# linchaobao/EPPM

Hardware: AMD Instinct MI355X
Metric: Mflow-vectors/sec (higher is better)
Workload: dtype f32; 1 GPU; single 1024x436 Sintel-shape synthetic pair per step, full 3-level pyramid, patch_r=9, default defs.h parameters; 1 rank(s), independent pairs; inputs: RGBA planes resident in HBM before the timed region; outputs: interleaved float2 flow left in HBM (the PCIe-inclusive window of the reference API -- host RGB in, host u/v out -- is `host_boundary`, with --full); inputs=device-resident RGBA, outputs=device-resident float2 flow, pairs_in_flight_per_gpu=24, pairs_per_launch=8, contexts_in_flight=3, width=1024, height=436

## Files before the change

### eppm_amd/_lib.py

```python
import ctypes as C
import os

from .build import lib_path


class EppmError(RuntimeError):
    pass


class CParams(C.Structure):
    _fields_ = [("patch_r", C.c_int), ("num_iter", C.c_int), ("search_range", C.c_int), ("num_guess", C.c_int),
                ("seg_len", C.c_int), ("wmf_iters", C.c_int), ("seed", C.c_ulonglong), ("propagation", C.c_int),
                ("levels", C.c_int)]


class CTrackParams(C.Structure):
    _fields_ = [("spacing", C.c_int), ("min_eig", C.c_int64), ("fb_alpha", C.c_float), ("fb_beta", C.c_float), ("mb_alpha", C.c_float),
                ("mb_beta", C.c_float), ("capacity", C.c_int)]


class CTFilterParams(C.Structure):
    _fields_ = [("thresh", C.c_float), ("n_max", C.c_int)]


class CStabParams(C.Structure):
    _fields_ = [("tau", C.c_float), ("iters", C.c_int), ("smooth", C.c_float)]


class CGMotionModel(C.Structure):
    _fields_ = [("p", C.c_double * 6), ("n_valid", C.c_int64), ("n_inliers", C.c_int64), ("valid", C.c_int), ("passes", C.c_int)]

    def as_dict(self):
        import numpy as np
        return dict(p=np.array(self.p[:], np.float64), n_valid=int(self.n_valid), n_inliers=int(self.n_inliers), valid=int(self.valid),
                    passes=int(self.passes))


class CCutParams(C.Structure):
    _fields_ = [("lost_permille", C.c_int), ("residual_max", C.c_float)]


class CCutStats(C.Structure):
    _fields_ = [("n", C.c_int64), ("c1", C.c_int64 * 4), ("c2", C.c_int64 * 4), ("n_tracked", C.c_int64), ("sad", C.c_int64), ("cut", C.c_int32),
                ("stepped", C.c_int32)]

    def as_dict(self):
        return dict(n=int(self.n), c1=[int(x) for x in self.c1], c2=[int(x) for x in self.c2], n_tracked=int(self.n_tracked), sad=int(self.sad),
                    cut=int(self.cut), stepped=int(self.stepped))


class CTrackCounts(C.Structure):
    _fields_ = [("live", C.c_int), ("ended", C.c_int), ("seeded", C.c_int), ("dropped", C.c_int), ("frame", C.c_int), ("next_id", C.c_int)]

    def as_dict(self):
        return {k: int(getattr(self, k)) for k, _ in self._fields_}


_lib = None

SYMBOLS = [
    "eppm_default_params", "eppm_create", "eppm_create_batch", "eppm_batch_size", "eppm_batch_set_images", "eppm_batch_set_images_device",
    "eppm_batch_compute", "eppm_batch_compute_device", "eppm_batch_compute_end", "eppm_batch_get_plane", "eppm_destroy", "eppm_set_stream", "eppm_set_images", "eppm_set_images_device",
    "eppm_compute", "eppm_compute_begin", "eppm_compute_end", "eppm_compute_device", "eppm_synchronize", "eppm_num_levels", "eppm_level_dims", "eppm_get_plane",
    "eppm_stage_times", "eppm_clear_stage_times", "eppm_enable_stage_timing", "eppm_last_error", "eppm_version",
    "eppm_device_count", "eppm_set_device", "eppm_malloc_device", "eppm_malloc_pitched", "eppm_free_device",
    "eppm_memcpy_h2d", "eppm_memcpy_d2h", "eppm_memcpy2d_h2d", "eppm_memcpy2d_d2h", "eppm_memset_device",
    "eppm_device_synchronize", "eppm_device_mem_info", "eppm_device_pci_bus_id", "eppm_bind_thread_to_device", "eppm_release_cached_memory", "eppm_set_launcher_stream", "eppm_set_launcher_params", "eppm_launcher_status",
    "baoCudaPatchMatchMultiscalePrepare", "baoCudaCensusTransform", "baoCudaPatchMatch", "baoCudaLeftRightCheck",
    "baoCudaOutlierRemoval", "baoCudaWeightedMedianFilter", "baoCudaFillHole", "baoCudaNNF2Flow", "baoCudaBLF_C2F",
    "baoCudaBLFCostFilterRefine", "baoCudaFlowSmoothing", "eppm_flow_to_color", "eppm_compute_color",
    "eppm_pm_rng_create", "eppm_pm_rng_reset", "eppm_pm_rng_destroy", "eppm_pm_rng_block_states", "eppm_pm_gen_rand_field",
    "eppm_pm_cost_field", "eppm_pm_seg_propagate", "eppm_pm_jump_propagate", "eppm_pm_parallel_propagate", "eppm_pm_random_search", "eppm_gauss_filter_rgba", "eppm_resize_rgba",
    "eppm_resize_flow",
    "eppm_host_register", "eppm_host_unregister", "eppm_host_is_registered", "eppm_host_alloc", "eppm_host_free",
    "eppm_compute_begin_into", "eppm_batch_compute_begin_into",
    "eppm_load_ppm", "eppm_ppm_size", "eppm_save_flo", "eppm_load_flo", "eppm_flo_size", "eppm_flow_error",
    "eppm_flow_error_border", "eppm_flow_error_percentage", "eppm_flow_cutoff", "eppm_flow_to_color_host",
    "eppm_compute_bidirectional", "eppm_compute_bidirectional_device", "eppm_batch_compute_bidirectional", "eppm_set_occlusion_params",
    "eppm_fb_occlusion", "eppm_fb_occlusion_host",
    "eppm_interpolate", "eppm_interpolate_device", "eppm_batch_interpolate", "eppm_interpolate_frames", "eppm_interpolate_host",
    "eppm_track_default_params", "eppm_track_capacity", "eppm_tracker_create", "eppm_tracker_destroy", "eppm_track_step",
    "eppm_track_step_frames", "eppm_tracker_get", "eppm_tracker_get_ended", "eppm_tracker_set", "eppm_track_step_host", "eppm_track_seeds_host",
    "eppm_push_image", "eppm_push_image_device", "eppm_set_temporal", "eppm_temporal_reset", "eppm_temporal_valid", "eppm_temporal_prior_host",
    "eppm_temporal_prior",
    "eppm_batch_set_temporal", "eppm_batch_push_images", "eppm_batch_push_images_device", "eppm_batch_temporal_valid", "eppm_batch_temporal_reset",
    "eppm_temporal_prior_batch",
    "eppm_set_stop_level", "eppm_stop_level", "eppm_flow_upsample",
    "eppm_tfilter_default_params", "eppm_tfilter_create", "eppm_tfilter_create_size", "eppm_tfilter_destroy", "eppm_tfilter_reset", "eppm_tfilter_step",
    "eppm_tfilter_step_frames", "eppm_tfilter_get", "eppm_tfilter_get_device", "eppm_tfilter_get_state", "eppm_tfilter_set_state",
    "eppm_tfilter_seed_host", "eppm_tfilter_step_host",
    "eppm_stab_default_params", "eppm_stab_create", "eppm_stab_create_size", "eppm_stab_destroy", "eppm_stab_reset", "eppm_stab_step",
    "eppm_stab_step_frames", "eppm_stab_get", "eppm_stab_get_device", "eppm_stab_get_mask", "eppm_stab_get_model", "eppm_stab_get_path",
    "eppm_stab_set_path", "eppm_gmotion_fit_host", "eppm_stab_update_host", "eppm_stab_warp_host",
    "eppm_cutdet_default_params", "eppm_cutdet_create", "eppm_cutdet_create_size", "eppm_cutdet_destroy", "eppm_cutdet_step",
    "eppm_cutdet_step_frames", "eppm_cutdet_get", "eppm_cutdet_cuts", "eppm_cutdet_host",
]


TEST_SYMBOLS = ["eppm_test_set_option", "eppm_test_c2f_refine_batch", "eppm_probe_c2f_window", "eppm_probe_dispatch", "eppm_probe_fast_exp", "eppm_probe_div_const", "eppm_probe_delta_table",
                "eppm_probe_unpack_texel", "eppm_probe_pm_parity", "eppm_probe_ctx_rng_states"]

_variant = None


def select_library(variant):
    global _variant
    if _lib is not None and variant != _variant:
        raise EppmError("select_library: a library is loaded already")
    _variant = variant


def lib():
    global _lib
    if _lib is None:
        path = lib_path(_variant)
        if not os.path.exists(path):
            raise EppmError(f"{path} is missing: run eppm_amd.build() (hipcc --offload-arch=gfx950); there is no CPU fallback")
        L = C.CDLL(path)
        L.eppm_last_error.restype = C.c_char_p
        L.eppm_version.restype = C.c_char_p
        _lib = L
    return _lib


def check(status, what=""):
    if status != 0:
        raise EppmError(f"{what}: status {status}: {lib().eppm_last_error().decode()}")


def check_launcher(what=""):
    check(lib().eppm_launcher_status(), what)


def probe_dispatch(stage, *args, nout=1):
    a = (C.c_int * len(args))(*[int(v) for v in args])
    out = (C.c_int * nout)()
    check(lib().eppm_probe_dispatch(stage.encode(), a, len(args), out, nout), f"eppm_probe_dispatch {stage}")
    return tuple(out)
```

### eppm_amd/csrc/api_internal.h

```cpp
#pragma once

#include <ctype.h>
#include <math.h>
#include <sched.h>
#include <stdarg.h>
#include <stdio.h>
#include <stdlib.h>
#include <string.h>

#include <atomic>
#include <chrono>
#include <condition_variable>
#include <map>
#include <mutex>
#include <string>
#include <tuple>
#include <vector>

#include "eppm_internal.h"
#include "host_registry.h"

#define EPPM_HIDDEN __attribute__((visibility("hidden")))

EPPM_HIDDEN int set_err(int code, const char* fmt, ...) __attribute__((format(printf, 2, 3)));
#define HIPCHK(expr)                                                                                         \
    do {                                                                                                     \
        hipError_t e_ = (expr);                                                                              \
        if (e_ != hipSuccess) {                                                                              \
            (void)hipGetLastError();                                                                         \
            return set_err(EPPM_ERR_HIP, "%s failed: %s (%s:%d)", #expr, hipGetErrorString(e_), __FILE__, __LINE__); \
        }                                                                                                    \
    } while (0)
#define CHK(expr)                     \
    do {                              \
        int r_ = (expr);              \
        if (r_ != EPPM_OK) return r_; \
    } while (0)

EPPM_HIDDEN int check_params(const eppm_params& p);
EPPM_HIDDEN void host_pm_lut(int R, std::vector<float>& v);
EPPM_HIDDEN void host_wmf_lut(std::vector<float>& v);
EPPM_HIDDEN void host_blf_lut(std::vector<float>& v);
EPPM_HIDDEN int pyr_init_dim(int* arrH, int* arrW, int h, int w, int maxDepth, double ratio);
EPPM_HIDDEN int upload_lut(float** dst, const std::vector<float>& v);
struct DeltaIndex { int32_t t1[256]; std::vector<float> dval; };
EPPM_HIDDEN const DeltaIndex& delta_index();
EPPM_HIDDEN int upload_lut_delta(float** dst, const std::vector<float>& head, int which);
EPPM_HIDDEN int upload_pm_lut(float** dst, int R);
EPPM_HIDDEN int upload_wmf_lut(float** dst);
EPPM_HIDDEN int upload_blf_lut(float** dst);

#ifdef EPPM_TEST_HOOKS
EPPM_HIDDEN extern std::atomic<int> g_opt_rand_table;
EPPM_HIDDEN extern std::atomic<int> g_opt_sweep_spec;
EPPM_HIDDEN extern std::atomic<int> g_opt_no_split;
EPPM_HIDDEN extern std::atomic<int> g_opt_force_split;
static inline int opt_rand_table() { return g_opt_rand_table.load(); }
static inline int opt_sweep_spec() { return g_opt_sweep_spec.load(); }
static inline int opt_no_split() { return g_opt_no_split.load(); }
static inline int opt_force_split() { return g_opt_force_split.load(); }
#else
static constexpr int opt_rand_table() { return 1; }
static constexpr int opt_sweep_spec() { return -1; }
static constexpr int opt_no_split() { return 0; }
static constexpr int opt_force_split() { return 0; }
#endif


namespace eppm { struct RngTables; }
struct eppm_pm_rng {
    eppm::RngTables* tables = nullptr;
    const int16_t* rand_tab = nullptr;
    size_t rand_stride = 0;
    int device = 0, w = 0, h = 0, gx = 0, gy = 0, G = 0, per_lane = 0;
    unsigned long long seed = 0;
    uint32_t* init_tab = nullptr;
    uint32_t* iter_tab = nullptr;
    uint32_t* work[2][2] = {{nullptr, nullptr}, {nullptr, nullptr}};
    bool own_work = true;
    int cur[2] = {0, 0};
    uint32_t* skip_mat = nullptr;
    uint32_t skip_weyl = 0;
    eppm::PmRngDev dev() const
    {
        eppm::PmRngDev d;
        d.init_tab = init_tab; d.iter_tab = iter_tab; d.skip_mat = skip_mat;
        d.skip_weyl = skip_weyl; d.per_lane = per_lane; d.gx = gx; d.gy = gy;
        return d;
    }
};
EPPM_HIDDEN int rng_create(eppm_pm_rng** out, int w, int h, const eppm_params& p, bool alloc_work = true);
EPPM_HIDDEN void rng_free(eppm_pm_rng* r);
EPPM_HIDDEN void rngtab_release_idle();

EPPM_HIDDEN hipError_t cache_alloc(void** p, size_t bytes, bool pinned, int device);
EPPM_HIDDEN void cache_free(void* p, size_t bytes, bool pinned, int device);
EPPM_HIDDEN hipError_t pooled_stream_create(hipStream_t* out, int device);
EPPM_HIDDEN void pooled_stream_destroy(hipStream_t s, int device);

EPPM_HIDDEN eppm::PmProblem mk_problem(const eppm::PlanesH& P, float* cost, int16_t* nnf, int16_t* nnf_alt, eppm_pm_rng* rng, int k, float* spec = nullptr,
                                       int32_t* scand = nullptr, uint32_t* wl = nullptr, int16_t* seed = nullptr);
EPPM_HIDDEN void search(eppm::PmBatch& b, eppm_pm_rng* rng, const float* lut, const eppm_params& prm, hipStream_t s, int launch_no = -1);
EPPM_HIDDEN bool sweep_list_on(int mode);
EPPM_HIDDEN void sweep(eppm::PmBatch& b, const float* lut, const eppm_params& prm, int dir, hipStream_t s, bool speculative = false);
EPPM_HIDDEN void jump(eppm::PmBatch& b, const float* lut, const eppm_params& prm, hipStream_t s);
EPPM_HIDDEN void neighbor(eppm::PmBatch& b, const float* lut, const eppm_params& prm, int launches, hipStream_t s);
EPPM_HIDDEN void run_patchmatch(eppm::PmBatch& b, eppm_pm_rng* rng, const float* lut, const eppm_params& prm, hipStream_t s, int spec_mode);
EPPM_HIDDEN void pm_start(eppm::PmBatch& b, eppm_pm_rng* rng, const float* lut, const eppm_params& prm, hipStream_t s);
EPPM_HIDDEN void pm_iterate(eppm::PmBatch& b, eppm_pm_rng* rng, const float* lut, const eppm_params& prm, hipStream_t s, int spec_mode);
#ifndef EPPM_SWEEP_CACHE
#define EPPM_SWEEP_CACHE 1
#endif

EPPM_HIDDEN int launcher_finish();

EPPM_HIDDEN int ctx_track_inputs(eppm_ctx* c, int pair, int h, int w, int device, const char* what, eppm::TrackIn* in, hipStream_t* s);
EPPM_HIDDEN int ctx_device(const eppm_ctx* c, int* h, int* w);
EPPM_HIDDEN void ctx_stage_begin(eppm_ctx* c, const char* name);
EPPM_HIDDEN void ctx_stage_end(eppm_ctx* c);
EPPM_HIDDEN int tracker_step_on(eppm_tracker* t, const eppm::TrackIn& in, hipStream_t s, eppm_ctx* timing);
EPPM_HIDDEN int tracker_device(const eppm_tracker* t, int* h, int* w);

EPPM_HIDDEN int ctx_tfilter_inputs(eppm_ctx* c, int h, int w, int device, int nslots, const char* what, eppm::TFilterArgs* in, hipStream_t* s);
EPPM_HIDDEN int tfilter_step_on(eppm_tfilter* f, eppm::TFilterArgs& in, int slot0, const uint8_t* cut, hipStream_t s, eppm_ctx* timing);
EPPM_HIDDEN int tfilter_device(const eppm_tfilter* f, int* h, int* w, int* nslots);

EPPM_HIDDEN int ctx_stab_inputs(eppm_ctx* c, int h, int w, int device, int nslots, const char* what, eppm::StabArgs* in, hipStream_t* s);
EPPM_HIDDEN int stab_step_on(eppm_stab* f, eppm::StabArgs& in, int slot0, const uint8_t* cut, hipStream_t s, eppm_ctx* timing);
EPPM_HIDDEN int stab_device(const eppm_stab* f, int* h, int* w, int* nslots);

EPPM_HIDDEN int ctx_cutdet_inputs(eppm_ctx* c, int h, int w, int device, int nslots, const char* what, eppm::CutArgs* in, hipStream_t* s);
EPPM_HIDDEN int cutdet_step_on(eppm_cutdet* f, eppm::CutArgs& in, int slot0, hipStream_t s, eppm_ctx* timing);
EPPM_HIDDEN int cutdet_device(const eppm_cutdet* f, int* h, int* w, int* nslots);
```

### eppm_amd/csrc/context.cpp

```cpp
#include "context.h"

using namespace eppm;

extern "C" int eppm_destroy(eppm_ctx* c)
{
    if (!c) return EPPM_OK;
    (void)hipSetDevice(c->device);
    if (c->stream) (void)hipStreamSynchronize(c->stream);
    c->out_hold.release();
    clear_events(c, c->ev);
    clear_events(c, c->ev_prep);
    for (hipEvent_t e : c->ev_pool) (void)hipEventDestroy(e);
    cache_free(c->slab, c->slab_bytes, false, c->device);
    if (c->h_color) (void)hipHostFree(c->h_color);
    for (int q = 0; q < 2; q++) {
        cache_free(c->h_rgb[q], c->h_rgb_bytes, true, c->device);
        if (c->ev_rgb[q]) (void)hipEventDestroy(c->ev_rgb[q]);
    }
    if (c->ev_h2d) (void)hipEventDestroy(c->ev_h2d);
    cache_free(c->h_flow, c->h_flow_bytes, true, c->device);
    cache_free(c->bwd, c->bwd_bytes, false, c->device);
    cache_free(c->h_bwd, c->h_bwd_bytes, true, c->device);
    cache_free(c->itp, c->itp_bytes, false, c->device);
    cache_free(c->h_itp, c->h_itp_bytes, true, c->device);
    cache_free(c->tmp, c->tmp_bytes, false, c->device);
    rng_free(c->rng);
    if (c->own_stream && c->stream) pooled_stream_destroy(c->stream, c->device);
    delete c;
    return EPPM_OK;
}

static int shared_luts(int device, int R, float** pm, float** wmf, float** blf)
{
    struct Entry { int device, R; float *pm, *wmf, *blf; };
    static std::mutex mu;
    static std::vector<Entry> tab;
    std::lock_guard<std::mutex> lk(mu);
    for (const Entry& e : tab)
        if (e.device == device && e.R == R) { *pm = e.pm; *wmf = e.wmf; *blf = e.blf; return EPPM_OK; }
    Entry e{device, R, nullptr, nullptr, nullptr};
    CHK(upload_pm_lut(&e.pm, R));
    CHK(upload_wmf_lut(&e.wmf));
    CHK(upload_blf_lut(&e.blf));
    tab.push_back(e);
    *pm = e.pm; *wmf = e.wmf; *blf = e.blf;
    return EPPM_OK;
}

static int ctx_alloc(eppm_ctx* c)
{
    const int h = c->h, w = c->w;
    Carve cv;
    auto pitch_of = [](size_t row_bytes) { return (row_bytes + 255) & ~(size_t)255; };
    c->raw_pitch = pitch_of((size_t)w * 4);
    for (uint32_t** p : {&c->raw1, &c->raw2}) cv.plane(p, c->raw_pitch * h);
    for (int i = 0; i < c->nl; i++) {
        c->ipitch[i] = pitch_of((size_t)c->W[i] * 4);
        c->cpitch[i] = pitch_of((size_t)c->W[i]);
        const size_t n = (size_t)c->W[i] * c->H[i];
        for (uint32_t** p : {&c->img1[i], &c->img2[i], &c->tmpu[i]}) cv.plane(p, c->ipitch[i] * c->H[i]);
        for (void** p : {&c->pk1[i], &c->pk2[i]}) cv.plane(p, n * 16);
        for (uint32_t** p : {&c->pc1[i], &c->pc2[i]}) cv.plane(p, n * 4);
        for (uint8_t** p : {&c->cen1[i], &c->cen2[i]}) cv.plane(p, c->cpitch[i] * c->H[i]);
        for (float** p : {&c->flow[i], &c->flow_tmp[i]}) cv.plane(p, n * 8);
        if (i < c->nl - 1 && c2f_refine_wants_split(c->W[i], c->H[i], c->prm.patch_r, 1, c->opt_no_split != 0)) cv.plane(&c->c2f_cost9[i], n * 36 * 4);
    }
    const int L = c->nl - 1;
    const size_t n2 = (size_t)c->W[L] * c->H[L];
#ifndef EPPM_TOL
    if (c->prm.patch_r == 9)
#endif
    {
        c->pp_pad = (c->prm.patch_r + 2) & ~1;
        c->pp_pitch = parity_pitch(c->W[L], c->pp_pad);
        for (uint32_t** p : {&c->pp1, &c->pp2}) cv.plane(p, (size_t)2 * c->H[L] * c->pp_pitch * 4);
    }
    for (int16_t** p : {&c->nnf1, &c->nnf2, &c->nnf_tmp, &c->nnf_tmp2}) cv.plane(p, n2 * 4);
    for (float** p : {&c->cost1, &c->cost2}) cv.plane(p, n2 * 4);
    for (float** p : {&c->spec1, &c->spec2}) cv.plane(p, n2 * 4 * 4);
    for (int32_t** p : {&c->scand1, &c->scand2}) cv.plane(p, n2 * 4 * 4);
    for (uint32_t** p : {&c->wl1, &c->wl2}) cv.plane(p, pm_worklist_words(c->W[L], c->H[L], c->prm.seg_len) * 4);
    for (int16_t** p : {&c->seed1, &c->seed2}) cv.plane(p, n2 * 4 * 4);
    cv.plane(&c->wmf_ws, wmf_workspace_words(c->W[L], c->H[L], c->prm.wmf_iters) * 4);
    cv.plane(&c->d_rgb, (size_t)h * w * 3 * 2);
    cv.plane(&c->d_color, (size_t)h * w * 4);
    cv.plane(&c->d_uv, (size_t)h * w * 8);
    CHK(rng_create(&c->rng, c->W[L], c->H[L], c->prm, false));
    const size_t rng_bytes = (size_t)c->rng->gx * c->rng->gy * 64 * 6 * 4;
    for (int k = 0; k < 2; k++)
        for (int q = 0; q < 2; q++) cv.plane(&c->rng->work[k][q], rng_bytes);
    c->stride = (cv.off + 4095) & ~(size_t)4095;
    CHK(cv.alloc(&c->slab, &c->slab_bytes, c->stride * c->npairs, c->device, (std::to_string(c->npairs) + " slab(s)").c_str()));
    CHK(shared_luts(c->device, c->prm.patch_r, &c->lut_pm, &c->lut_wmf, &c->lut_blf));
    c->out_u.assign(c->npairs, nullptr);
    c->out_v.assign(c->npairs, nullptr);
    for (auto* v : {&c->tmp_snap, &c->tmp_valid, &c->tmp_seeded, &c->tmp_cut}) v->assign(c->npairs, 0);
    return EPPM_OK;
}

extern "C" int eppm_create_batch(eppm_ctx** out, int h, int w, int device, const eppm_params* params, int npairs)
{
    if (!out) return set_err(EPPM_ERR_ARG, "eppm_create: NULL out");
    *out = nullptr;
    if (npairs < 1 || npairs > 4096) return set_err(EPPM_ERR_ARG, "eppm_create_batch: npairs %d out of range [1,4096]", npairs);
    if (h < 4 || w < 4 || h > 32767 || w > 32767) return set_err(EPPM_ERR_ARG, "eppm_create: size %dx%d out of range (NNF coordinates are int16)", w, h);
    if ((unsigned long long)h * (unsigned long long)w * 16ULL >= (1ULL << 32))
        return set_err(EPPM_ERR_ARG, "eppm_create: size %dx%d out of range (texel planes are addressed with 32-bit byte offsets)", w, h);
    eppm_params p;
    eppm_default_params(&p);
    if (params) p = *params;
    CHK(check_params(p));
    HIPCHK(hipSetDevice(device));
    eppm_ctx* c = new eppm_ctx();
    c->device = device; c->prm = p; c->h = h; c->w = w; c->npairs = npairs; c->n_active = 1;
    c->opt_sweep_spec = opt_sweep_spec(); c->opt_no_split = opt_no_split();
    c->nl = pyr_init_dim(c->H, c->W, h, w, p.levels, 0.5f);
    const int L = c->nl - 1;
    if (c->H[L] < 1 || c->W[L] < 1 || (c->W[L] + p.seg_len - 1) / p.seg_len > 1024 || (c->H[L] + p.seg_len - 1) / p.seg_len > 1024) {
        delete c;
        return set_err(EPPM_ERR_ARG, "eppm_create: unsupported size %dx%d", w, h);
    }
    const hipError_t e = pooled_stream_create(&c->stream, c->device);
    if (e != hipSuccess) { delete c; return set_err(EPPM_ERR_HIP, "hipStreamCreate: %s", hipGetErrorString(e)); }
    c->own_stream = true;
    int r = ctx_alloc(c);
    if (r != EPPM_OK) { eppm_destroy(c); return r; }
    *out = c;
    return EPPM_OK;
}

extern "C" int eppm_create(eppm_ctx** out, int h, int w, int device, const eppm_params* params)
{
    return eppm_create_batch(out, h, w, device, params, 1);
}

extern "C" int eppm_batch_size(const eppm_ctx* c) { return c ? c->npairs : 0; }

extern "C" int eppm_set_stream(eppm_ctx* c, void* s)
{
    if (!c) return set_err(EPPM_ERR_ARG, "NULL ctx");
    if (c->own_stream && c->stream) { (void)hipStreamSynchronize(c->stream); pooled_stream_destroy(c->stream, c->device); }
    c->stream = (hipStream_t)s;
    c->own_stream = false;
    return EPPM_OK;
}

extern "C" int eppm_num_levels(const eppm_ctx* c) { return c ? c->nl : 0; }
extern "C" int eppm_level_dims(const eppm_ctx* c, int level, int* h, int* w)
{
    if (!c || level < 0 || level >= c->nl) return set_err(EPPM_ERR_ARG, "bad level");
    if (h) *h = c->H[level];
    if (w) *w = c->W[level];
    return EPPM_OK;
}
extern "C" int eppm_enable_stage_timing(eppm_ctx* c, int on)
{
    if (!c) return set_err(EPPM_ERR_ARG, "NULL ctx");
    c->timing = (on == 2) ? 2 : (on != 0);
    return EPPM_OK;
}

int ctx_device(const eppm_ctx* c, int* h, int* w)
{
    *h = c->h;
    *w = c->w;
    return c->device;
}

void ctx_stage_begin(eppm_ctx* c, const char* name) { stage_begin(c, c->ev, name); }
void ctx_stage_end(eppm_ctx* c) { stage_end(c, c->ev); }

extern "C" int eppm_synchronize(eppm_ctx* c)
{
    if (!c) return set_err(EPPM_ERR_ARG, "NULL ctx");
    HIPCHK(hipStreamSynchronize(c->stream));
    return EPPM_OK;
}

extern "C" int eppm_stage_times(eppm_ctx* c, const char** names, float* ms, int max)
{
    if (!c) return 0;
    (void)hipStreamSynchronize(c->stream);
    int n = 0;
    for (auto* v : {&c->ev_prep, &c->ev})
        for (auto& e : *v) {
            if (n >= max) return n;
            float t = 0;
            if (hipEventElapsedTime(&t, e.a, e.b) != hipSuccess) t = -1;
            names[n] = e.name; ms[n] = t; n++;
        }
    return n;
}

extern "C" int eppm_clear_stage_times(eppm_ctx* c)
{
    if (!c) return set_err(EPPM_ERR_ARG, "NULL ctx");
    (void)hipStreamSynchronize(c->stream);
    clear_events(c, c->ev);
    clear_events(c, c->ev_prep);
    return EPPM_OK;
}

extern "C" int eppm_batch_get_plane(eppm_ctx* c, int pair, const char* name, int level, void* dst, size_t dst_bytes)
{
    if (!c || !name || !dst) return set_err(EPPM_ERR_ARG, "eppm_get_plane: NULL argument");
    if (level < 0 || level >= c->nl) return set_err(EPPM_ERR_ARG, "eppm_get_plane: bad level %d", level);
    if (pair < 0 || pair >= c->npairs) return set_err(EPPM_ERR_ARG, "eppm_get_plane: bad pair %d", pair);
    HIPCHK(hipSetDevice(c->device));
    HIPCHK(hipStreamSynchronize(c->stream));
    const int w = c->W[level], h = c->H[level], L = c->nl - 1;
    const void* src = nullptr;
    size_t esz = 0, pitch = 0, pstride = c->stride;
    std::string n(name);
    if (n == "img1" || n == "img2") { src = (n == "img1") ? c->img1[level] : c->img2[level]; esz = 4; pitch = c->ipitch[level]; }
    else if (n == "census1" || n == "census2") { src = (n == "census1") ? c->cen1[level] : c->cen2[level]; esz = 1; pitch = c->cpitch[level]; }
    else if (n == "flow") { src = c->flow[level]; esz = 8; pitch = (size_t)w * 8; }
    else if (level == L && (n == "nnf1" || n == "nnf2")) { src = (n == "nnf1") ? c->nnf1 : c->nnf2; esz = 4; pitch = (size_t)w * 4; }
    else if (level == L && (n == "cost1" || n == "cost2")) { src = (n == "cost1") ? c->cost1 : c->cost2; esz = 4; pitch = (size_t)w * 4; }
    else if (n == "flow_bwd" || (level == 0 && (n == "occ1" || n == "occ2"))) {
        if (!c->have_bwd) return set_err(EPPM_ERR_STATE, "eppm_get_plane: '%s' needs a bidirectional call first", name);
        if (n == "flow_bwd") { src = c->bflow[level]; esz = 8; }
        else { src = (n == "occ1") ? c->occ1 : c->occ2; esz = 1; }
        pitch = (size_t)w * esz;
        pstride = c->bwd_stride;
    }
    else if (level == L && (n == "prior1" || n == "prior2" || n == "nnf_init1" || n == "nnf_init2" || n == "cost_init1" || n == "cost_init2")) {
        if (!c->tmp_seeded[pair]) return set_err(EPPM_ERR_STATE, "eppm_get_plane: '%s' needs a compute that started from a temporal prior", name);
        src = n == "prior1" ? (void*)c->prior1 : n == "prior2" ? (void*)c->prior2 : n == "nnf_init1" ? (void*)c->nnf_init1 : n == "nnf_init2" ? (void*)c->nnf_init2
            : n == "cost_init1" ? (void*)c->cost_init1 : (void*)c->cost_init2;
        esz = 4; pitch = (size_t)w * 4;
        pstride = c->tmp_stride;
    }
    else return set_err(EPPM_ERR_ARG, "eppm_get_plane: unknown plane '%s' at level %d", name, level);
    if (dst_bytes < (size_t)w * h * esz) return set_err(EPPM_ERR_ARG, "eppm_get_plane: dst too small");
    HIPCHK(hipMemcpy2D(dst, (size_t)w * esz, (const char*)src + (size_t)pair * pstride, pitch, (size_t)w * esz, h, hipMemcpyDeviceToHost));
    return EPPM_OK;
}

extern "C" int eppm_get_plane(eppm_ctx* c, const char* name, int level, void* dst, size_t dst_bytes)
{
    return eppm_batch_get_plane(c, 0, name, level, dst, dst_bytes);
}

extern "C" int eppm_compute_color(eppm_ctx* c, uint8_t* rgb, size_t row_stride, float max_disp_x, float max_disp_y)
{
    if (!c || !rgb) return set_err(EPPM_ERR_ARG, "eppm_compute_color: NULL argument");
    if (!c->have_flow) return set_err(EPPM_ERR_STATE, "eppm_compute_color: no flow computed yet");
    if (row_stride < (size_t)c->w * 3) return set_err(EPPM_ERR_ARG, "eppm_compute_color: row_stride %zu < 3*w", row_stride);
    HIPCHK(hipSetDevice(c->device));
    const size_t n = (size_t)c->h * c->w;
    if (!c->h_color) HIPCHK(hipHostMalloc((void**)&c->h_color, n * 4, hipHostMallocDefault));
    launch_flow_to_color(c->d_color, c->flow[0], c->h, c->w, max_disp_x, max_disp_y, c->stream);
    HIPCHK(hipMemcpyAsync(c->h_color, c->d_color, n * 4, hipMemcpyDeviceToHost, c->stream));
    HIPCHK(hipStreamSynchronize(c->stream));
    for (int y = 0; y < c->h; y++)
        for (int x = 0; x < c->w; x++) {
            const uint32_t p = c->h_color[(size_t)y * c->w + x];
            uint8_t* o = rgb + (size_t)y * row_stride + (size_t)x * 3;
            o[0] = (uint8_t)(p & 0xff); o[1] = (uint8_t)((p >> 8) & 0xff); o[2] = (uint8_t)((p >> 16) & 0xff);
        }
    return EPPM_OK;
}

#ifdef EPPM_TEST_HOOKS
extern "C" int eppm_probe_pm_parity(const eppm_ctx* c, int* pitch, int* pad, int* kernels)
{
    if (!c || !pitch || !pad || !kernels) return set_err(EPPM_ERR_ARG, "eppm_probe_pm_parity: NULL argument");
    *pitch = c->pp1 ? c->pp_pitch : 0;
    *pad = c->pp1 ? c->pp_pad : 0;
    *kernels = c->pp1 ? pm_parity_kernels(c->prm.patch_r) : 0;
    return EPPM_OK;
}
extern "C" int eppm_probe_ctx_rng_states(eppm_ctx* c, uint32_t* dst, size_t dst_words)
{
    if (!c || !dst) return set_err(EPPM_ERR_ARG, "eppm_probe_ctx_rng_states: NULL argument");
    const int nb = c->rng->gx * c->rng->gy;
    if (dst_words < (size_t)nb * 6) return set_err(EPPM_ERR_ARG, "eppm_probe_ctx_rng_states: dst too small");
    HIPCHK(hipSetDevice(c->device));
    HIPCHK(hipStreamSynchronize(c->stream));
    HIPCHK(hipMemcpy2D(dst, 24, c->rng->work[0][c->rng->cur[0]], 64 * 24, 24, nb, hipMemcpyDeviceToHost));
    return EPPM_OK;
}
#endif
```

### eppm_amd/csrc/context.h

```cpp
#pragma once

#include <algorithm>

#include "api_internal.h"

struct StageEv { const char* name; hipEvent_t a, b; };

struct eppm_ctx {
    int device = 0;
    hipStream_t stream = nullptr;
    bool own_stream = false;
    int opt_sweep_spec = -1, opt_no_split = 0;
    eppm_params prm;
    int h = 0, w = 0, nl = 0;
    int stop_level = 0;
    int npairs = 1, n_active = 1;
    char* slab = nullptr;
    size_t stride = 0;
    int H[eppm::kMaxLevels], W[eppm::kMaxLevels];
    size_t ipitch[eppm::kMaxLevels], cpitch[eppm::kMaxLevels];
    uint32_t *raw1 = nullptr, *raw2 = nullptr;
    size_t raw_pitch = 0;
    uint32_t *img1[eppm::kMaxLevels] = {}, *img2[eppm::kMaxLevels] = {}, *tmpu[eppm::kMaxLevels] = {};
    uint8_t *cen1[eppm::kMaxLevels] = {}, *cen2[eppm::kMaxLevels] = {};
    void *pk1[eppm::kMaxLevels] = {}, *pk2[eppm::kMaxLevels] = {};
    uint32_t *pc1[eppm::kMaxLevels] = {}, *pc2[eppm::kMaxLevels] = {};
    uint32_t *pp1 = nullptr, *pp2 = nullptr;
    int pp_pitch = 0, pp_pad = 0;
    int16_t *nnf1 = nullptr, *nnf2 = nullptr, *nnf_tmp = nullptr, *nnf_tmp2 = nullptr;
    float *cost1 = nullptr, *cost2 = nullptr;
    float *spec1 = nullptr, *spec2 = nullptr;
    int32_t *scand1 = nullptr, *scand2 = nullptr;
    uint32_t *wl1 = nullptr, *wl2 = nullptr;
    int16_t *seed1 = nullptr, *seed2 = nullptr;
    uint32_t* wmf_ws = nullptr;
    bool flow_pending = false;
    float *flow[eppm::kMaxLevels] = {}, *flow_tmp[eppm::kMaxLevels] = {};
    float* c2f_cost9[eppm::kMaxLevels] = {};
    float *lut_pm = nullptr, *lut_wmf = nullptr, *lut_blf = nullptr;
    eppm_pm_rng* rng = nullptr;
    float* d_uv = nullptr;
    uint32_t* d_color = nullptr;
    uint32_t* h_color = nullptr;
    uint8_t* d_rgb = nullptr;
    size_t slab_bytes = 0, h_rgb_bytes = 0, h_flow_bytes = 0;
    uint8_t* h_rgb[2] = {nullptr, nullptr};
    hipEvent_t ev_rgb[2] = {nullptr, nullptr};
    hipEvent_t ev_h2d = nullptr;
    int rgb_cur = 0;
    float* h_flow = nullptr;
    std::vector<float*> out_u, out_v;
    eppm::HostHold out_hold;
    bool have_images = false, have_flow = false;
    char* bwd = nullptr;
    size_t bwd_stride = 0, bwd_bytes = 0, h_bwd_bytes = 0;
    float* bflow[eppm::kMaxLevels] = {};
    float* d_buv = nullptr;
    uint8_t *occ1 = nullptr, *occ2 = nullptr;
    uint8_t* h_bwd = nullptr;
    float occ_alpha = 0.01f, occ_beta = 0.5f;
    bool have_bwd = false;
    bool bwd_images = false;
    char* itp = nullptr;
    size_t itp_bytes = 0, itp_plane = 0, h_itp_bytes = 0;
    uint64_t* itp_keys = nullptr;
    int32_t *itp_fill1 = nullptr, *itp_fill2 = nullptr;
    uint8_t* itp_rgb = nullptr;
    uint8_t* h_itp = nullptr;
    bool temporal = false;
    std::vector<uint8_t> tmp_snap;
    std::vector<uint8_t> tmp_valid;
    std::vector<uint8_t> tmp_seeded;
    std::vector<uint8_t> tmp_cut;
    char* tmp = nullptr;
    size_t tmp_bytes = 0, tmp_stride = 0;
    int16_t *prev_fwd = nullptr, *prev_bwd = nullptr, *prior1 = nullptr, *prior2 = nullptr, *nnf_init1 = nullptr, *nnf_init2 = nullptr;
    float *cost_init1 = nullptr, *cost_init2 = nullptr;
    int32_t* tmp_keys = nullptr;
    void tmp_drop() { std::fill(tmp_valid.begin(), tmp_valid.end(), 0); std::fill(tmp_snap.begin(), tmp_snap.end(), 0); std::fill(tmp_cut.begin(), tmp_cut.end(), 0); }
    int timing = 0;
    std::vector<StageEv> ev;
    std::vector<StageEv> ev_prep;
    std::vector<hipEvent_t> ev_pool;
    eppm::Batch bt() const { return eppm::Batch{n_active, stride}; }
    template <class T> T* of_pair(T* p, int k) const { return (T*)((char*)p + (size_t)k * stride); }
    template <class T> T* of_bwd_pair(T* p, int k) const { return (T*)((char*)p + (size_t)k * bwd_stride); }
};

static inline eppm::PlanesH planes(const eppm_ctx* c, int l, bool swap)
{
    eppm::PlanesH p;
    p.pk1 = swap ? c->pk2[l] : c->pk1[l];
    p.pk2 = swap ? c->pk1[l] : c->pk2[l];
    p.w = c->W[l]; p.h = c->H[l];
    p.pitch = c->W[l];
    p.pc1 = swap ? c->pc2[l] : c->pc1[l];
    p.pc2 = swap ? c->pc1[l] : c->pc2[l];
    if (l == c->nl - 1 && c->pp1) {
        p.pp1 = swap ? c->pp2 : c->pp1;
        p.pp2 = swap ? c->pp1 : c->pp2;
        p.pp_pitch = c->pp_pitch; p.pp_pad = c->pp_pad;
    }
    return p;
}

static inline hipEvent_t pool_event(eppm_ctx* c)
{
    hipEvent_t e = nullptr;
    if (!c->ev_pool.empty()) { e = c->ev_pool.back(); c->ev_pool.pop_back(); }
    else (void)hipEventCreate(&e);
    return e;
}
static inline bool stage_on(const eppm_ctx* c, bool dominant) { return c->timing == 1 || (c->timing == 2 && dominant); }
static inline void stage_begin(eppm_ctx* c, std::vector<StageEv>& v, const char* name, bool dominant = false)
{
    if (!stage_on(c, dominant)) return;
    StageEv e;
    e.name = name;
    e.a = pool_event(c);
    e.b = pool_event(c);
    (void)hipEventRecord(e.a, c->stream);
    v.push_back(e);
}
static inline void stage_end(eppm_ctx* c, std::vector<StageEv>& v, bool dominant = false)
{
    if (!stage_on(c, dominant)) return;
    (void)hipEventRecord(v.back().b, c->stream);
}
static inline void stage_end_at(eppm_ctx* c, std::vector<StageEv>& v, size_t idx)
{
    if (!stage_on(c, false)) return;
    (void)hipEventRecord(v[idx].b, c->stream);
}
static inline void clear_events(eppm_ctx* c, std::vector<StageEv>& v)
{
    for (auto& e : v) { c->ev_pool.push_back(e.a); c->ev_pool.push_back(e.b); }
    v.clear();
}

struct EPPM_HIDDEN Carve {
    struct Fix { void** dst; size_t off; };
    std::vector<Fix> fix;
    size_t off = 0;
    template <class T> void plane(T** dst, size_t bytes) { fix.push_back(Fix{(void**)dst, off}); off = (off + bytes + 255) & ~(size_t)255; }
    int alloc(char** base, size_t* held, size_t bytes, int device, const char* what) const
    {
        const hipError_t e = cache_alloc((void**)base, bytes, false, device);
        if (e != hipSuccess) {
            (void)hipGetLastError();
            *base = nullptr;
            return set_err(EPPM_ERR_HIP, "hipMalloc of %zu bytes (%s) failed: %s", bytes, what, hipGetErrorString(e));
        }
        *held = bytes;
        for (const Fix& f : fix) *f.dst = *base + f.off;
        return EPPM_OK;
    }
};

template <class T> static inline hipError_t pinned_lazy(T** p, size_t* held, size_t bytes, int device)
{
    if (*p) return hipSuccess;
    *held = bytes;
    return cache_alloc((void**)p, bytes, true, device);
}

static inline void copy_rows(uint8_t* dst, size_t dst_stride, const uint8_t* src, size_t src_stride, size_t row, int h)
{
    if (dst_stride == row && src_stride == row) { memcpy(dst, src, row * h); return; }
    for (int y = 0; y < h; y++) memcpy(dst + (size_t)y * dst_stride, src + (size_t)y * src_stride, row);
}
```

### eppm_amd/csrc/ctx_compute.cpp

```cpp
#include "context.h"
#include "temporal.h"

using namespace eppm;

static int tmp_alloc(eppm_ctx* c)
{
    if (c->tmp) return EPPM_OK;
    const int L = c->nl - 1;
    const size_t n2 = (size_t)c->W[L] * c->H[L];
    Carve cv;
    for (int16_t** p : {&c->prev_fwd, &c->prev_bwd, &c->prior1, &c->prior2, &c->nnf_init1, &c->nnf_init2}) cv.plane(p, n2 * 4);
    for (float** p : {&c->cost_init1, &c->cost_init2}) cv.plane(p, n2 * 4);
    cv.plane(&c->tmp_keys, n2 * 4 * 2);
    c->tmp_stride = cv.off;
    CHK(cv.alloc(&c->tmp, &c->tmp_bytes, c->tmp_stride * c->npairs, c->device, "temporal planes"));
    for (int k = 0; k < c->npairs; k++) launch_temporal_keys_init((int32_t*)((char*)c->tmp_keys + (size_t)k * c->tmp_stride), (int)(2 * n2), c->stream);
    HIPCHK(hipGetLastError());
    return EPPM_OK;
}

static int set_temporal(eppm_ctx* c, int on)
{
    c->temporal = on != 0;
    if (!on) c->tmp_drop();
    return EPPM_OK;
}
extern "C" int eppm_set_temporal(eppm_ctx* c, int on)
{
    if (!c) return set_err(EPPM_ERR_ARG, "eppm_set_temporal: NULL ctx");
    if (on && c->npairs != 1) return set_err(EPPM_ERR_ARG, "eppm_set_temporal: a batch context streams through eppm_batch_set_temporal (one clip per slot)");
    return set_temporal(c, on);
}
extern "C" int eppm_temporal_reset(eppm_ctx* c)
{
    if (!c) return set_err(EPPM_ERR_ARG, "eppm_temporal_reset: NULL ctx");
    return eppm_batch_temporal_reset(c, 0);
}
extern "C" int eppm_temporal_valid(const eppm_ctx* c) { return eppm_batch_temporal_valid(c, 0); }

extern "C" int eppm_batch_set_temporal(eppm_ctx* c, int on)
{
    if (!c) return set_err(EPPM_ERR_ARG, "eppm_batch_set_temporal: NULL ctx");
    return set_temporal(c, on);
}
extern "C" int eppm_batch_temporal_reset(eppm_ctx* c, int pair)
{
    if (!c) return set_err(EPPM_ERR_ARG, "eppm_batch_temporal_reset: NULL ctx");
    if (pair >= c->npairs) return set_err(EPPM_ERR_ARG, "eppm_batch_temporal_reset: pair %d, context holds %d", pair, c->npairs);
    for (int k = pair < 0 ? 0 : pair; k < (pair < 0 ? c->npairs : pair + 1); k++) c->tmp_valid[k] = c->tmp_snap[k] = 0;
    return EPPM_OK;
}
extern "C" int eppm_batch_temporal_valid(const eppm_ctx* c, int pair)
{
    return c && pair >= 0 && pair < c->npairs && c->temporal && c->tmp_valid[pair] ? 1 : 0;
}

struct Branch {
    int16_t *&nnf, *&nnf_alt;
    float* cost;
    uint32_t* const* guide;
    bool swap, bwd, dominant;
    int16_t* snapshot;
    float *a[kMaxLevels], *b[kMaxLevels];
};

enum { kStageUp, kStageRefine, kStageBlf, kStageJbu };
static const struct EPPM_HIDDEN LevelStageNames {
    char s[4][2][kMaxLevels][24];
    LevelStageNames()
    {
        const char* base[4] = {"upsample", "c2f_refine", "flow_blf", "flow_jbu"};
        for (int k = 0; k < 4; k++)
            for (int b = 0; b < 2; b++)
                for (int l = 0; l < kMaxLevels; l++) snprintf(s[k][b][l], sizeof s[k][b][l], "%s%s_L%d", base[k], b ? "_bwd" : "", l);
    }
} level_stage;

static void branch_nnf2flow(eppm_ctx* c, Branch& d)
{
    hipStream_t s = c->stream;
    const Batch bt = c->bt();
    const int L = c->nl - 1, lw = c->W[L], lh = c->H[L], gp = (int)(c->ipitch[L] / 4);
    launch_outlier(d.nnf_alt, d.cost, d.nnf, lw, lh, lw, lw, s, bt);
    std::swap(d.nnf, d.nnf_alt);
    if (launch_wmf(d.nnf, d.nnf_alt, d.guide[L], gp, lw, lh, lw, c->lut_wmf, c->prm.wmf_iters, 1, c->wmf_ws, s, bt) != d.nnf)
        std::swap(d.nnf, d.nnf_alt);
    launch_fill_holes(d.nnf_alt, d.nnf, d.guide[L], gp, lw, lh, lw, s, bt);
    std::swap(d.nnf, d.nnf_alt);
    if (d.snapshot) launch_nnf2flow_snapshot(d.a[L], lw, d.snapshot, c->tmp_stride, d.nnf, lw, lw, lh, s, bt);
    else launch_nnf2flow(d.a[L], lw, d.nnf, lw, lw, lh, s, bt);
}

static int branch_c2f(eppm_ctx* c, Branch& d, int (*keep)(eppm_ctx*, int, float*))
{
    hipStream_t s = c->stream;
    const Batch bt = c->bt();
    const int L = c->nl - 1;
    auto blf = [&](float* dst, const float* src, int l) { launch_flow_blf(dst, src, d.guide[l], (int)(c->ipitch[l] / 4), c->W[l], c->H[l], c->W[l], c->lut_blf, s, bt); };
    const int stop = c->stop_level;
    float* r = d.a[L];
    for (int l = L - 1; l >= 0; l--) {
        if (l < stop) {
            stage_begin(c, c->ev, level_stage.s[kStageJbu][d.bwd][l]);
            float* out = (r == d.b[l]) ? d.a[l] : d.b[l];
            launch_flow_jbu(out, r, d.guide[l], (int)(c->ipitch[l] / 4), c->W[l], c->H[l], c->W[l + 1], c->H[l + 1], c->lut_blf, s, bt);
            r = out;
            CHK(keep(c, l, r));
            stage_end(c, c->ev);
            continue;
        }
        stage_begin(c, c->ev, level_stage.s[kStageUp][d.bwd][l]);
        launch_resize_flow(d.a[l], c->H[l], c->W[l], r, c->H[l + 1], c->W[l + 1], 2.0f, 2.0f, s, bt);
        stage_end(c, c->ev);
        stage_begin(c, c->ev, level_stage.s[kStageRefine][d.bwd][l], d.dominant);
        launch_c2f_refine(planes(c, l, d.swap), d.a[l], c->lut_pm, c->prm.patch_r, c->c2f_cost9[l], s, bt, c->opt_no_split != 0);
        stage_end(c, c->ev, d.dominant);
        stage_begin(c, c->ev, level_stage.s[kStageBlf][d.bwd][l]);
        blf(d.b[l], d.a[l], l);
        r = d.b[l];
        if (l > 0) CHK(keep(c, l, r));
        stage_end(c, c->ev);
    }
    if (stop > 0) return EPPM_OK;
    stage_begin(c, c->ev, d.bwd ? "flow_blf_bwd_final" : "flow_blf_final");
    float* out = (r == d.b[0]) ? d.a[0] : d.b[0];
    blf(out, r, 0);
    CHK(keep(c, 0, out));
    stage_end(c, c->ev);
    return EPPM_OK;
}

static int keep_fwd(eppm_ctx* c, int l, float* r)
{
    if (r != c->flow[l]) std::swap(c->flow[l], c->flow_tmp[l]);
    return EPPM_OK;
}

static int compute_all(eppm_ctx* c)
{
    if (!c->have_images) return set_err(EPPM_ERR_STATE, "eppm_compute: no images set");
    HIPCHK(hipSetDevice(c->device));
    c->have_bwd = false;
    hipStream_t s = c->stream;
    const Batch bt = c->bt();
    const int L = c->nl - 1, lw = c->W[L], lh = c->H[L];

    const bool tmode = c->temporal;
    bool seeded = false;
    std::fill(c->tmp_seeded.begin(), c->tmp_seeded.end(), 0);
    if (tmode) {
        CHK(tmp_alloc(c));
        TemporalArgs a{};
        for (int k = 0; k < bt.n; k++)
            if (c->tmp_valid[k]) { a.armed[k >> 5] |= 1u << (k & 31); seeded = true; }
        if (seeded) {
            a.prev[0] = c->prev_fwd; a.prior[0] = c->prior1; a.keys[0] = c->tmp_keys; a.step[0] = 1;
            a.prev[1] = c->prev_bwd; a.prior[1] = c->prior2; a.keys[1] = c->tmp_keys + (size_t)lw * lh; a.step[1] = -1;
            a.w = lw; a.h = lh; a.ndir = 2; a.nslots = bt.n; a.stride = c->tmp_stride;
            stage_begin(c, c->ev, "temporal_advect");
            launch_temporal_splat(a, s);
            launch_temporal_gather(a, s);
            stage_end(c, c->ev);
        }
    }
    std::fill(c->tmp_snap.begin(), c->tmp_snap.end(), 0);

    const size_t pm_entry = c->ev.size();
    stage_begin(c, c->ev, "patchmatch");
    {
        PmBatch b;
        b.n = 2; b.cpitch = lw; b.npitch = lw; b.npairs = bt.n; b.stride = bt.stride;
        b.cache_plane = (size_t)lw * lh;
        b.seed_plane = (size_t)lw * lh * 2;
        b.wl_units = pm_worklist_units(lw, lh, c->prm.seg_len);
        b.p[0] = mk_problem(planes(c, L, false), c->cost1, c->nnf1, c->nnf_tmp, c->rng, 0, c->spec1, EPPM_SWEEP_CACHE ? c->scand1 : nullptr, sweep_list_on(c->opt_sweep_spec) ? c->wl1 : nullptr, c->seed1);
        b.p[1] = mk_problem(planes(c, L, true), c->cost2, c->nnf2, c->nnf_tmp2, c->rng, 1, c->spec2, EPPM_SWEEP_CACHE ? c->scand2 : nullptr, sweep_list_on(c->opt_sweep_spec) ? c->wl2 : nullptr, c->seed2);
        if (!seeded) run_patchmatch(b, c->rng, c->lut_pm, c->prm, s, c->opt_sweep_spec);
        else {
            pm_start(b, c->rng, c->lut_pm, c->prm, s);
            PmSeed sd;
            sd.prior[0] = c->prior1; sd.nnf_init[0] = c->nnf_init1; sd.cost_init[0] = c->cost_init1;
            sd.prior[1] = c->prior2; sd.nnf_init[1] = c->nnf_init2; sd.cost_init[1] = c->cost_init2;
            sd.stride = c->tmp_stride;
            stage_begin(c, c->ev, "temporal_select");
            launch_pm_cost_select(b, sd, c->lut_pm, c->prm.patch_r, s);
            stage_end(c, c->ev);
            pm_iterate(b, c->rng, c->lut_pm, c->prm, s, c->opt_sweep_spec);
        }
    }
    stage_end_at(c, c->ev, pm_entry);
    if (tmode) launch_temporal_snapshot(c->prev_bwd, c->tmp_stride, c->nnf2, lw, lw, lh, s, bt);

    stage_begin(c, c->ev, "l2_post");
    launch_lr_check(c->nnf1, c->cost1, c->nnf2, lw, lh, lw, lw, s, bt);
    launch_lr_check(c->nnf2, c->cost2, c->nnf1, lw, lh, lw, lw, s, bt);
    Branch d{c->nnf1, c->nnf_tmp, c->cost1, c->img1, false, false, true, tmode ? c->prev_fwd : nullptr};
    for (int l = 0; l <= L; l++) { d.a[l] = c->flow[l]; d.b[l] = c->flow_tmp[l]; }
    branch_nnf2flow(c, d);
    stage_end(c, c->ev);
    CHK(branch_c2f(c, d, keep_fwd));
    HIPCHK(hipGetLastError());
    c->have_flow = true;
    for (int k = 0; k < bt.n; k++) {
        c->tmp_snap[k] = tmode && !c->tmp_cut[k];
        c->tmp_seeded[k] = tmode && c->tmp_valid[k];
    }
    std::fill(c->tmp_valid.begin(), c->tmp_valid.end(), 0);
    return EPPM_OK;
}


static int bwd_alloc(eppm_ctx* c)
{
    if (c->bwd) return EPPM_OK;
    Carve cv;
    for (int l = 0; l < c->nl; l++) cv.plane(&c->bflow[l], (size_t)c->W[l] * c->H[l] * 8);
    const size_t n = (size_t)c->h * c->w;
    cv.plane(&c->d_buv, n * 10);
    c->bwd_stride = (cv.off + 4095) & ~(size_t)4095;
    CHK(cv.alloc(&c->bwd, &c->bwd_bytes, c->bwd_stride * c->npairs, c->device, "backward planes"));
    c->occ1 = (uint8_t*)c->d_buv + n * 8;
    c->occ2 = c->occ1 + n;
    return EPPM_OK;
}

static int keep_bwd(eppm_ctx* c, int l, float* src)
{
    const size_t bytes = (size_t)c->W[l] * c->H[l] * 8;
    for (int k = 0; k < c->n_active; k++)
        HIPCHK(hipMemcpyAsync(c->of_bwd_pair(c->bflow[l], k), c->of_pair(src, k), bytes, hipMemcpyDeviceToDevice, c->stream));
    return EPPM_OK;
}

static int backward_all(eppm_ctx* c)
{
    const int L = c->nl - 1;
    Branch d{c->nnf2, c->nnf_tmp2, c->cost2, c->img2, true, true, false, nullptr};
    for (int l = 0; l <= L; l++) { d.a[l] = c->flow_tmp[l]; d.b[l] = c->d_uv; }
    stage_begin(c, c->ev, "l2_post_bwd");
    branch_nnf2flow(c, d);
    if (L > 0) CHK(keep_bwd(c, L, d.a[L]));
    stage_end(c, c->ev);
    CHK(branch_c2f(c, d, keep_bwd));

    stage_begin(c, c->ev, "fb_occlusion");
    launch_fb_occlusion(c->occ1, c->occ2, c->flow[0], c->stride, c->bflow[0], c->bwd_stride, c->h, c->w, c->occ_alpha, c->occ_beta, c->n_active, 2, c->stream);
    stage_end(c, c->ev);
    HIPCHK(hipGetLastError());
    c->have_bwd = true;
    c->bwd_images = true;
    return EPPM_OK;
}

static int compute_bidir_all(eppm_ctx* c)
{
    if (!c->have_images) return set_err(EPPM_ERR_STATE, "eppm_compute_bidirectional: no images set");
    HIPCHK(hipSetDevice(c->device));
    CHK(bwd_alloc(c));
    CHK(compute_all(c));
    return backward_all(c);
}

extern "C" int eppm_compute_device(eppm_ctx* c, void* d_flow)
{
    if (!c) return set_err(EPPM_ERR_ARG, "NULL ctx");
    CHK(compute_all(c));
    if (d_flow) HIPCHK(hipMemcpyAsync(d_flow, c->flow[0], (size_t)c->h * c->w * 8, hipMemcpyDeviceToDevice, c->stream));
    return EPPM_OK;
}

extern "C" int eppm_batch_compute_device(eppm_ctx* c, void* const* d_flows)
{
    if (!c) return set_err(EPPM_ERR_ARG, "NULL ctx");
    CHK(compute_all(c));
    if (d_flows)
        for (int k = 0; k < c->n_active; k++)
            if (d_flows[k]) HIPCHK(hipMemcpyAsync(d_flows[k], c->of_pair(c->flow[0], k), (size_t)c->h * c->w * 8, hipMemcpyDeviceToDevice, c->stream));
    return EPPM_OK;
}

static int compute_begin_impl(eppm_ctx* c, int n_out, float* const* u, float* const* v, bool bidir)
{
    CHK(bidir ? compute_bidir_all(c) : compute_all(c));
    const size_t n = (size_t)c->h * c->w;
    launch_split_flow(c->d_uv, c->flow[0], (int)n, c->stream, c->bt());
    if (bidir) {
        launch_split_flow(c->d_buv, c->bflow[0], (int)n, c->stream, Batch{c->n_active, c->bwd_stride});
        HIPCHK(pinned_lazy(&c->h_bwd, &c->h_bwd_bytes, n * 10 * c->npairs, c->device));
        for (int k = 0; k < c->n_active; k++)
            HIPCHK(hipMemcpyAsync(c->h_bwd + (size_t)k * n * 10, c->of_bwd_pair(c->d_buv, k), n * 10, hipMemcpyDeviceToHost, c->stream));
    }
    for (int k = 0; k < c->n_active; k++) {
        float* du = (u && k < n_out) ? u[k] : nullptr;
        float* dv = (v && k < n_out) ? v[k] : nullptr;
        const float* src = c->of_pair(c->d_uv, k);
        if (du && dv && c->out_hold.add2(du, dv, n * 4)) {
            HIPCHK(hipMemcpyAsync(du, src, n * 4, hipMemcpyDeviceToHost, c->stream));
            HIPCHK(hipMemcpyAsync(dv, src + n, n * 4, hipMemcpyDeviceToHost, c->stream));
            c->out_u[k] = du; c->out_v[k] = dv;
            continue;
        }
        HIPCHK(pinned_lazy(&c->h_flow, &c->h_flow_bytes, n * 8 * c->npairs, c->device));
        HIPCHK(hipMemcpyAsync(c->h_flow + (size_t)k * n * 2, src, n * 8, hipMemcpyDeviceToHost, c->stream));
        c->out_u[k] = c->out_v[k] = nullptr;
    }
    c->flow_pending = true;
    return EPPM_OK;
}
static int compute_begin(eppm_ctx* c, int n_out, float* const* u, float* const* v, bool bidir = false)
{
    const int r = compute_begin_impl(c, n_out, u, v, bidir);
    if (r != EPPM_OK && !c->out_hold.v.empty()) {
        (void)hipStreamSynchronize(c->stream);
        c->out_hold.release();
    }
    return r;
}

extern "C" int eppm_compute_begin(eppm_ctx* c)
{
    if (!c) return set_err(EPPM_ERR_ARG, "eppm_compute_begin: NULL ctx");
    return compute_begin(c, 0, nullptr, nullptr);
}

extern "C" int eppm_compute_begin_into(eppm_ctx* c, float* u, float* v)
{
    if (!c || !u || !v) return set_err(EPPM_ERR_ARG, "eppm_compute_begin_into: NULL argument");
    return compute_begin(c, 1, &u, &v);
}

extern "C" int eppm_batch_compute_begin_into(eppm_ctx* c, float* const* u, float* const* v)
{
    if (!c || !u || !v) return set_err(EPPM_ERR_ARG, "eppm_batch_compute_begin_into: NULL argument");
    return compute_begin(c, c->n_active, u, v);
}

static int compute_end(eppm_ctx* c, int n_out, float* const* u, float* const* v)
{
    if (!c->flow_pending) return set_err(EPPM_ERR_STATE, "eppm_compute_end without eppm_compute_begin");
    HIPCHK(hipSetDevice(c->device));
    const hipError_t es = hipStreamSynchronize(c->stream);
    c->out_hold.release();
    HIPCHK(es);
    c->flow_pending = false;
    const size_t n = (size_t)c->h * c->w;
    for (int k = 0; k < n_out && k < c->n_active; k++) {
        if (!u[k] || !v[k]) continue;
        const float* fu = c->out_u[k] ? c->out_u[k] : c->h_flow + (size_t)k * n * 2;
        const float* fv = c->out_v[k] ? c->out_v[k] : c->h_flow + (size_t)k * n * 2 + n;
        if (u[k] != fu) memcpy(u[k], fu, n * sizeof(float));
        if (v[k] != fv) memcpy(v[k], fv, n * sizeof(float));
    }
    return EPPM_OK;
}

extern "C" int eppm_compute_end(eppm_ctx* c, float* u, float* v)
{
    if (!c || !u || !v) return set_err(EPPM_ERR_ARG, "eppm_compute_end: NULL argument");
    return compute_end(c, 1, &u, &v);
}

extern "C" int eppm_batch_compute_end(eppm_ctx* c, float* const* u, float* const* v)
{
    if (!c || !u || !v) return set_err(EPPM_ERR_ARG, "eppm_batch_compute_end: NULL argument");
    return compute_end(c, c->n_active, u, v);
}

extern "C" int eppm_compute(eppm_ctx* c, float* u, float* v)
{
    if (!c || !u || !v) return set_err(EPPM_ERR_ARG, "eppm_compute: NULL argument");
    CHK(compute_begin(c, 1, &u, &v));
    return compute_end(c, 1, &u, &v);
}

extern "C" int eppm_batch_compute(eppm_ctx* c, float* const* u, float* const* v)
{
    if (!c || !u || !v) return set_err(EPPM_ERR_ARG, "eppm_batch_compute: NULL argument");
    CHK(compute_begin(c, c->n_active, u, v));
    return compute_end(c, c->n_active, u, v);
}

static void bwd_copy_out(eppm_ctx* c, int n_out, float* const* bu, float* const* bv, uint8_t* const* o1, uint8_t* const* o2)
{
    const size_t n = (size_t)c->h * c->w;
    for (int k = 0; k < n_out && k < c->n_active; k++) {
        const uint8_t* src = c->h_bwd + (size_t)k * n * 10;
        if (bu && bu[k]) memcpy(bu[k], src, n * 4);
        if (bv && bv[k]) memcpy(bv[k], src + n * 4, n * 4);
        if (o1 && o1[k]) memcpy(o1[k], src + n * 8, n);
        if (o2 && o2[k]) memcpy(o2[k], src + n * 9, n);
    }
}

static int compute_bidir(eppm_ctx* c, int n_out, float* const* u, float* const* v, float* const* bu, float* const* bv, uint8_t* const* o1,
                         uint8_t* const* o2)
{
    if (c->flow_pending) return set_err(EPPM_ERR_STATE, "eppm_compute_bidirectional: an eppm_compute_begin is pending");
    CHK(compute_begin(c, n_out, u, v, true));
    CHK(compute_end(c, n_out, u, v));
    bwd_copy_out(c, n_out, bu, bv, o1, o2);
    return EPPM_OK;
}

extern "C" int eppm_compute_bidirectional(eppm_ctx* c, float* u, float* v, float* bu, float* bv, uint8_t* occ1, uint8_t* occ2)
{
    if (!c || !u || !v) return set_err(EPPM_ERR_ARG, "eppm_compute_bidirectional: NULL argument");
    return compute_bidir(c, 1, &u, &v, &bu, &bv, &occ1, &occ2);
}

extern "C" int eppm_batch_compute_bidirectional(eppm_ctx* c, float* const* u, float* const* v, float* const* bu, float* const* bv,
                                                uint8_t* const* occ1, uint8_t* const* occ2)
{
    if (!c || !u || !v) return set_err(EPPM_ERR_ARG, "eppm_batch_compute_bidirectional: NULL argument");
    return compute_bidir(c, c->n_active, u, v, bu, bv, occ1, occ2);
}

extern "C" int eppm_compute_bidirectional_device(eppm_ctx* c, void* d_flow, void* d_flow_bwd, void* d_occ1, void* d_occ2)
{
    if (!c) return set_err(EPPM_ERR_ARG, "eppm_compute_bidirectional_device: NULL ctx");
    CHK(compute_bidir_all(c));
    const size_t n = (size_t)c->h * c->w;
    if (d_flow) HIPCHK(hipMemcpyAsync(d_flow, c->flow[0], n * 8, hipMemcpyDeviceToDevice, c->stream));
    if (d_flow_bwd) HIPCHK(hipMemcpyAsync(d_flow_bwd, c->bflow[0], n * 8, hipMemcpyDeviceToDevice, c->stream));
    if (d_occ1) HIPCHK(hipMemcpyAsync(d_occ1, c->occ1, n, hipMemcpyDeviceToDevice, c->stream));
    if (d_occ2) HIPCHK(hipMemcpyAsync(d_occ2, c->occ2, n, hipMemcpyDeviceToDevice, c->stream));
    return EPPM_OK;
}

extern "C" int eppm_set_stop_level(eppm_ctx* c, int level)
{
    if (!c) return set_err(EPPM_ERR_ARG, "eppm_set_stop_level: NULL ctx");
    if (level < 0 || level > c->nl - 1) return set_err(EPPM_ERR_ARG, "eppm_set_stop_level: level %d outside 0 .. %d", level, c->nl - 1);
    if (c->flow_pending) return set_err(EPPM_ERR_STATE, "eppm_set_stop_level: an eppm_compute_begin is pending");
    c->stop_level = level;
    c->have_flow = c->have_bwd = false;
    return EPPM_OK;
}
extern "C" int eppm_stop_level(const eppm_ctx* c) { return c ? c->stop_level : -1; }

extern "C" int eppm_set_occlusion_params(eppm_ctx* c, float alpha, float beta)
{
    if (!c) return set_err(EPPM_ERR_ARG, "eppm_set_occlusion_params: NULL ctx");
    if (!(alpha >= 0 && isfinite(alpha)) || !(beta >= 0 && isfinite(beta)))
        return set_err(EPPM_ERR_ARG, "eppm_set_occlusion_params: alpha %g, beta %g must be finite and >= 0", alpha, beta);
    c->occ_alpha = alpha;
    c->occ_beta = beta;
    return EPPM_OK;
}
```

### eppm_amd/csrc/eppm_internal.h

```cpp
#pragma once

#include <hip/hip_runtime.h>
#include <stddef.h>
#include <stdint.h>

#include "../../include/eppm.h"

namespace eppm {

constexpr int kMaxLevels = 8;
constexpr int kNumLevels = 3;
constexpr int kBlock = 16;
constexpr int kMaxS = 32;
constexpr int kWmfRadius = 4;
constexpr int kBlfRadius = 10;
constexpr int kDeltaSlots = 800;

struct Batch {
    int n;
    size_t stride;
};
constexpr Batch kOnePair = {1, 0};

#define EPPM_DECISION __attribute__((visibility("hidden")))

struct PlanesH {
    const void* pk1;
    const void* pk2;
    int w, h, pitch;
    const uint32_t* pc1 = nullptr;
    const uint32_t* pc2 = nullptr;
    const uint32_t* pp1 = nullptr;
    const uint32_t* pp2 = nullptr;
    int pp_pitch = 0, pp_pad = 0;
};
inline int parity_pitch(int w, int pad) { return (w + 2 * pad + 1) / 2 + 1; }
void launch_parity_planes(uint32_t* pp, int pp_pitch, int pad, const uint32_t* pc, int pc_pitch, int w, int h, hipStream_t s, Batch bt = kOnePair);

void launch_gauss_rgba(uint32_t* out, const uint32_t* in, int pitch_px, int h, int w, float sigma, int radius, hipStream_t s, Batch bt = kOnePair);
bool gauss_decimate2_ok(int outH, int outW, int h, int w, float ratio, int radius);
void launch_gauss_decimate2(uint32_t* out0, const uint32_t* in0, uint32_t* out1, const uint32_t* in1, int nimg, int out_pitch_px, int outH,
                            int outW, int pitch_px, int h, int w, float sigma, int radius, hipStream_t s, Batch bt = kOnePair);
void launch_gauss_rgba2(uint32_t* out0, const uint32_t* in0, uint32_t* out1, const uint32_t* in1, int pitch_px, int h, int w, float sigma,
                        int radius, hipStream_t s, Batch bt = kOnePair);
struct CensusJob { uint8_t* census; int cpitch; void* texels; int tpitch; const uint32_t* img; int ipitch; int w, h; int first_block;
                   uint32_t* packed = nullptr; };
struct CensusBatch { int n; CensusJob job[2 * kMaxLevels]; };
void launch_census_batch(CensusBatch& B, hipStream_t s, Batch bt = kOnePair);
void launch_resize_rgba(uint32_t* out, int out_pitch_px, int outH, int outW, const uint32_t* in, int in_pitch_px, int h, int w,
                        float ratio, hipStream_t s, Batch bt = kOnePair);
void launch_census(uint8_t* census, int cpitch, void* texels, int tpitch, const uint32_t* img, int ipitch, int w, int h, hipStream_t s);
void launch_pack(void* texels, int tpitch, const uint32_t* img, int ipitch, const uint8_t* census, int cpitch, int w, int h, hipStream_t s);
void launch_delta_values(float* t2, int n, int which, hipStream_t s);
void launch_rgb_to_rgba(uint32_t* out, int pitch_px, const uint8_t* rgb, int h, int w, hipStream_t s, Batch bt = kOnePair);

struct PmProblem {
    PlanesH P;
    float* cost;
    int16_t* nnf;
    int16_t* nnf_alt;
    float* spec = nullptr;
    int32_t* scand = nullptr;
    uint32_t* wl = nullptr;
    int16_t* seed = nullptr;
    uint32_t* rng_work;
    uint32_t* rng_work_next;
};
struct PmBatch {
    PmProblem p[2];
    int n;
    int cpitch, npitch;
    int npairs = 1;
    size_t stride = 0;
    size_t cache_plane = 0;
    int wl_units = 0;
    int sweep_seq = 0;
    size_t seed_plane = 0;
    int merged_it = 0;
    int seg_len = 0, nseg_row = 0, nseg_col = 0;
};
int pm_worklist_units(int w, int h, int seg_len);
inline size_t pm_worklist_words(int w, int h, int seg_len) { return 16 + 10 * (size_t)pm_worklist_units(w, h, seg_len); }
struct PmRngDev {
    const uint32_t* init_tab;
    const uint32_t* iter_tab;
    const uint32_t* skip_mat;
    uint32_t skip_weyl;
    int per_lane;
    int gx, gy;
    const int16_t* rand_tab = nullptr;
};
void launch_pm_rand_table(const PmRngDev& rng, uint32_t* work, int16_t* tab, int G, hipStream_t s);
void launch_pm_init_field(const PmBatch& b, const PmRngDev& rng, hipStream_t s);
void launch_pm_cost_field(const PmBatch& b, const float* lut, int R, hipStream_t s);
int pm_parity_kernels(int R);
bool launch_pm_sweep(PmBatch& b, const float* lut, int R, int seg_len, int dir, hipStream_t s, bool speculative = false);
bool launch_pm_sweeps_merged(PmBatch& b, const float* lut, int R, int seg_len, int iteration, hipStream_t s);
void launch_pm_jump(const PmBatch& b, const float* lut, int R, int step, hipStream_t s);
void launch_pm_neighbor(const PmBatch& b, const float* lut, int R, hipStream_t s);
void launch_pm_random_search(const PmBatch& b, const PmRngDev& rng, const float* lut, int R, int search_range, int num_guess,
                             hipStream_t s);
EPPM_DECISION int pm_search_rows(int w, int h, int R, int problems, int npairs, bool table);
struct SweepForm { int lpc; bool small, pre, tile; };
EPPM_DECISION SweepForm pm_sweep_form(int w, int h, int R, int seg_len, int dir, int problems, int npairs);

struct PmSeed {
    const int16_t* prior[2];
    int16_t* nnf_init[2];
    float* cost_init[2];
    size_t stride = 0;
};
void launch_pm_cost_select(const PmBatch& b, const PmSeed& seed, const float* lut, int R, hipStream_t s);

constexpr int kTemporalMaxSlots = 4096;
struct TemporalArgs {
    const int16_t* prev[2];
    int16_t* prior[2];
    int32_t* keys[2];
    int step[2];
    int w, h, ndir;
    int nslots;
    size_t stride;
    uint32_t armed[kTemporalMaxSlots / 32];
};
void launch_temporal_keys_init(int32_t* keys, int n, hipStream_t s);
void launch_temporal_splat(const TemporalArgs& a, hipStream_t s);
void launch_temporal_gather(const TemporalArgs& a, hipStream_t s);
void launch_temporal_snapshot(int16_t* prev, size_t prev_stride, const int16_t* nnf, int nnf_pitch, int w, int h, hipStream_t s, Batch bt = kOnePair);
void launch_nnf2flow_snapshot(float* flow, int flow_pitch, int16_t* prev, size_t prev_stride, const int16_t* nnf, int nnf_pitch, int w, int h,
                              hipStream_t s, Batch bt = kOnePair);

void launch_lr_check(int16_t* nnf1, float* cost1, const int16_t* nnf2, int w, int h, int cost_pitch, int nnf_pitch, hipStream_t s, Batch bt = kOnePair);
void launch_outlier(int16_t* nnf_out, float* cost, const int16_t* nnf_in, int w, int h, int cost_pitch, int nnf_pitch, hipStream_t s, Batch bt = kOnePair);
size_t wmf_workspace_words(int w, int h, int num_iter);
int16_t* launch_wmf(int16_t* buf_a, int16_t* buf_b, const uint32_t* img, int ipitch, int w, int h, int nnf_pitch,
                    const float* wmf_lut, int num_iter, int only_occlusion, uint32_t* ws, hipStream_t s, Batch bt = kOnePair);
void launch_fill_holes(int16_t* nnf_out, const int16_t* nnf_in, const uint32_t* img, int ipitch, int w, int h, int nnf_pitch,
                       hipStream_t s, Batch bt = kOnePair);
void launch_nnf2flow(float* flow, int flow_pitch, const int16_t* nnf, int nnf_pitch, int w, int h, hipStream_t s, Batch bt = kOnePair);

void launch_resize_flow(float* out, int outH, int outW, const float* in, int h, int w, float ratio, float post_scale, hipStream_t s, Batch bt = kOnePair);
void launch_mul_scalar(float* flow, float scale, int h, int w, hipStream_t s);
EPPM_DECISION int c2f_refine_split_factor(int w, int h, int R, int npairs = 1, bool no_split = false);
bool c2f_refine_wants_split(int w, int h, int R, int npairs = 1, bool no_split = false);
bool c2f_window_span(int R, int* span_x, int* span_y);
void launch_c2f_refine(const PlanesH& P, float* flow, const float* lut, int R, float* cost9, hipStream_t s, Batch bt = kOnePair, bool no_split = false);
void launch_flow_blf(float* out, const float* in, const uint32_t* img, int ipitch, int w, int h, int flow_pitch,
                     const float* blf_lut, hipStream_t s, Batch bt = kOnePair);
EPPM_DECISION int flow_blf_pixels_per_lane(int w, int h, int npairs = 1);
void launch_flow_jbu(float* out, const float* in_coarse, const uint32_t* img, int ipitch, int w, int h, int wc, int hc, const float* blf_lut,
                     hipStream_t s, Batch bt = kOnePair);

void launch_split_flow(float* uv, const float* flow, int n, hipStream_t s, Batch bt = kOnePair);

void launch_fb_occlusion(uint8_t* occ1, uint8_t* occ2, const float* fwd, size_t fwd_stride, const float* bwd, size_t bwd_stride, int h, int w,
                         float alpha, float beta, int npairs, int ndir, hipStream_t s);

constexpr int kInterpChunk = 4;
struct InterpArgs {
    const uint8_t* img1;
    const uint8_t* img2;
    size_t img_pitch, img_stride;
    const float* flow;
    size_t flow_stride;
    const uint8_t* occ1;
    const uint8_t* occ2;
    size_t occ_stride;
    uint64_t* keys;
    int32_t* fill1;
    int32_t* fill2;
    size_t plane;
    uint8_t* rgb;
    uint8_t* rgba[kInterpChunk];
    size_t rgba_pitch;
    int h, w, nt;
    float t[kInterpChunk];
};
void launch_interp_splat(const InterpArgs& a, int npairs, hipStream_t s);
void launch_interp_fill(const InterpArgs& a, int npairs, hipStream_t s);
void launch_interp_blend(const InterpArgs& a, int npairs, hipStream_t s);

enum {
    kTrackCntLive, kTrackCntNextId, kTrackCntFrame, kTrackCntDropped, kTrackCntEnded, kTrackCntSeeded,
    kTrackCntIdBase, kTrackCntSurv, kTrackCntPrevLive, kTrackCntSeeded0, kTrackCntDropped0, kTrackCntN = 16
};
struct TrackRec;
struct TrackDev {
    struct {
        int spacing;
        long long min_eig;
        float fb_alpha, fb_beta, mb_alpha, mb_beta;
    } p;
    int cap, ncells, ncx;
    float* npos;
    uint8_t* stat;
    TrackRec* ended;
    int32_t* ended_reason;
    uint8_t* cov;
    uint8_t* flags;
    int32_t *blk_s, *blk_e;
    int32_t* blk_c;
    int32_t* cnt;
};
struct TrackIn {
    const uint8_t* img1;
    const uint8_t* img2;
    size_t pitch;
    const float* fwd;
    const float* bwd;
    int h, w;
};
void launch_track_seed0(const TrackDev& d, const TrackIn& in, TrackRec* cur, hipStream_t s);
void launch_track_advance(const TrackDev& d, const TrackIn& in, const TrackRec* cur, hipStream_t s);
void launch_track_seed(const TrackDev& d, const TrackIn& in, hipStream_t s);
void launch_track_compact(const TrackDev& d, const TrackIn& in, const TrackRec* cur, TrackRec* next, hipStream_t s);

struct TFilterArgs {
    const uint8_t* img1;
    const uint8_t* img2;
    size_t img_pitch, img_stride;
    const float* bwd;
    size_t bwd_stride;
    const uint8_t* occ2;
    size_t occ_stride;
    float* st0;
    float* st1;
    uint32_t* out;
    size_t slot_stride;
    int h, w, n, slot0;
    float thresh;
    int n_max;
    uint32_t cur[kTemporalMaxSlots / 32], empty[kTemporalMaxSlots / 32], cut[kTemporalMaxSlots / 32];
};
void launch_tfilter_step(const TFilterArgs& a, hipStream_t s);

constexpr int kGmTileW = 64, kGmTileH = 16, kGmSlabBytes = 128;
struct StabArgs {
    const uint8_t* img2;
    size_t img_pitch, img_stride;
    const float* fwd;
    size_t fwd_stride;
    const uint8_t* occ1;
    size_t occ_stride;
    char* mem;
    size_t slot_stride, off_model, off_out, off_mask;
    int h, w, n, slot0, tiles_x, tiles_y, iters, pass;
    float tau2, smooth;
    uint32_t empty[kTemporalMaxSlots / 32], cut[kTemporalMaxSlots / 32];
};
void launch_gmotion_accumulate(const StabArgs& a, hipStream_t s);
void launch_gmotion_solve(const StabArgs& a, hipStream_t s);
void launch_stab_warp(const StabArgs& a, hipStream_t s);

constexpr int kCutTileW = 64, kCutTileH = 16, kCutSlabBytes = 64;
struct CutArgs {
    const uint8_t* img1;
    const uint8_t* img2;
    size_t img_pitch, img_stride;
    const float* bwd;
    size_t bwd_stride;
    const uint8_t* occ1;
    const uint8_t* occ2;
    size_t occ_stride;
    char* mem;
    size_t off_slabs, slab_stride;
    int h, w, n, slot0, tiles_x, tiles_y;
    int lost_permille;
    long long r16;
};
void launch_cutdet_accumulate(const CutArgs& a, hipStream_t s);
void launch_cutdet_finish(const CutArgs& a, hipStream_t s);

void launch_flow_to_color(uint32_t* rgba, const float* flow, int h, int w, float max_disp_x, float max_disp_y, hipStream_t s, Batch bt = kOnePair);

void launch_probe_delta(const float* x, float* y, int n, const float* delta_tab, hipStream_t s);
void launch_probe(const float* x, float* y, int n, int which, hipStream_t s);
void launch_probe_unpack(const uint32_t* w, float* y, int n, hipStream_t s);

struct XorwowState { uint32_t v[5]; uint32_t d; };
void xorwow_init(XorwowState* s, unsigned long long seed, unsigned long long subsequence);
uint32_t xorwow_next(XorwowState* s);
void xorwow_skip_matrix(unsigned long long n, uint32_t* out);

}
```

### eppm_amd/csrc/k_pm_search.hip

```cpp
#include "pm_device.cuh"

namespace eppm {

__device__ __forceinline__ void xorwow_skip(Xorwow& st, const uint32_t* __restrict__ skip_mat, uint32_t skip_weyl)
{
    const uint32_t v[5] = {st.v0, st.v1, st.v2, st.v3, st.v4};
    uint32_t a0 = 0, a1 = 0, a2 = 0, a3 = 0, a4 = 0;
#pragma unroll
    for (int wd = 0; wd < 5; wd++) {
        const uint32_t vw = v[wd];
#pragma unroll 8
        for (int b = 0; b < 32; b++) {
            const uint32_t* row = skip_mat + (wd * 32 + b) * 5;
            const uint32_t m = 0u - ((vw >> b) & 1u);
            a0 ^= m & row[0]; a1 ^= m & row[1]; a2 ^= m & row[2]; a3 ^= m & row[3]; a4 ^= m & row[4];
        }
    }
    st.v0 = a0; st.v1 = a1; st.v2 = a2; st.v3 = a3; st.v4 = a4;
    st.d += skip_weyl;
}

__global__ __launch_bounds__(64) void k_pm_rand_table(PmRngDev rng, uint32_t* __restrict__ work, int16_t* __restrict__ tab, int G)
{
    const int block_id = blockIdx.x, lane = threadIdx.x;
    const size_t so = ((size_t)block_id * 64 + lane) * 6;
    Xorwow st = load_state(work + so);
    int16_t* __restrict__ out = tab + (size_t)block_id * 512 * G + rng.per_lane * lane;
    for (int q = 0; q < rng.per_lane; q++) out[q] = (int16_t)xorwow_next(st);
    xorwow_skip(st, rng.skip_mat, rng.skip_weyl);
    store_state(work + so, st);
}
void launch_pm_rand_table(const PmRngDev& rng, uint32_t* work, int16_t* tab, int G, hipStream_t s)
{
    hipLaunchKernelGGL(k_pm_rand_table, dim3(rng.gx * rng.gy), dim3(64), 0, s, rng, work, tab, G);
}

template <int RT, int PK = 0, bool TAB = false, int ROWS = 4>
__global__ __launch_bounds__(576) EPPM_SEARCH_OCC void k_pm_random_search(PmBatch B, PmRngDev rng, const float* __restrict__ lut, int R,
                                                          int search_range, int G)
{
    static_assert(ROWS == 4 || (ROWS == 2 && TAB && RT != 0), "eighth-block workgroups read their numbers from the table");
    using LUT = typename SearchLut<RT>::type;
    constexpr int PIXW = 16 * ROWS, NSUB = kBlock / ROWS;
    constexpr int TW = (RT == 0) ? 1 : kBlock + 2 * RT, TH = (RT == 0) ? 1 : ROWS + 2 * RT;
    __shared__ float4 s_src[TW * TH];
    __shared__ EPPM_LUT_ALIGN LUT L;
    __shared__ int16_t s_rand[TAB ? 2 : 8 * 512];
    __shared__ float s_cost[8][64];
    __shared__ int s_guess[8][64];
    __shared__ uint32_t s_state[TAB ? 2 : 64 * 6];
    const unsigned nprob = B.n * B.npairs, bq = blockIdx.x % nprob, brest = blockIdx.x / nprob;
    const int bxx = brest % rng.gx, byy = brest / rng.gx;
    const PmProblem pr = pm_problem(B, bq);
    const int tid = threadIdx.x;
    const int tile_y = byy / NSUB, quarter = byy % NSUB;
    const int block_id = tile_y * rng.gx + bxx;
    load_patch_lut(L, lut, R, tid, blockDim.x);
    if (!TAB && tid < 64) {
        const size_t so = ((size_t)block_id * 64 + tid) * 6;
        Xorwow st = load_state(pr.rng_work + so);
        const int base = rng.per_lane * tid;
        for (int q = 0; q < rng.per_lane; q++) s_rand[base + q] = (int16_t)xorwow_next(st);
        if (quarter == 0) store_state(s_state + tid * 6, st);
    }
    const Planes P = to_dev(pr.P);
    if (RT != 0) {
        const int x0 = bxx * kBlock - RT, y0 = tile_y * kBlock + quarter * ROWS - RT;
        for (int t = tid; t < TW * TH; t += blockDim.x) {
            const int sy = iclamp(y0 + t / TW, 0, P.h - 1), sx = iclamp(x0 + t % TW, 0, P.w - 1);
            s_src[t] = P.pk1[(unsigned)(sy * P.pitch + sx)];
        }
    }
    __syncthreads();
    const int lane = tid % PIXW, k = tid / PIXW;
    if (!TAB && k == G) {
        if (quarter == 0) {
            const size_t so = ((size_t)block_id * 64 + lane) * 6;
            Xorwow st = load_state(s_state + lane * 6);
            xorwow_skip(st, rng.skip_mat, rng.skip_weyl);
            store_state(pr.rng_work_next + so, st);
        }
    }
    const int pix = quarter * PIXW + lane;
    const int x = bxx * kBlock + (pix & 15), y = tile_y * kBlock + (pix >> 4);
    const bool inimg = (k < G) && (x < P.w && y < P.h);
    const int nidx = y * B.npitch + x, cidx = y * B.cpitch + x;
    int bx = 0, by = 0;
    int mag = search_range;
    for (int q = 0; q < k; q++) if (mag / 2 >= 1) mag /= 2;
    if (inimg) { bx = pr.nnf[nidx * 2]; by = pr.nnf[nidx * 2 + 1]; }
    int gx = 0, gy = 0;
    bool evaluate = false;
    if (inimg) {
        uint32_t rdn1, rdn2;
        if (TAB) {
            const uint32_t two = *reinterpret_cast<const uint32_t*>(rng.rand_tab + ((size_t)block_id * G + k) * 512 + 2 * pix);
            rdn1 = (uint32_t)(int32_t)(int16_t)(two & 0xffffu);
            rdn2 = (uint32_t)(int32_t)(int16_t)(two >> 16);
        } else {
            rdn1 = (uint32_t)(int32_t)s_rand[512 * k + 2 * pix];
            rdn2 = (uint32_t)(int32_t)s_rand[512 * k + 2 * pix + 1];
        }
        const int xmin = max(bx - mag, 0), xmax = min(bx + mag + 1, P.w + 1);
        const int ymin = max(by - mag, 0), ymax = min(by + mag + 1, P.h + 1);
        gx = (int)(int16_t)((uint32_t)xmin + rdn1 % (uint32_t)(xmax - xmin));
        gy = (int)(int16_t)((uint32_t)ymin + rdn2 % (uint32_t)(ymax - ymin));
        evaluate = !(EPPM_SEARCH_SKIP_SAME && gx == bx && gy == by);
        s_guess[k][lane] = (gx & 0xffff) | (gy << 16);
    }
    if (inimg) {
        float cv = INFINITY;
        if (evaluate) {
            cv = search_patch_dist<RT, PK>(P, L, R, s_src, TW, lane & 15, lane >> 4, x, y, gx, gy, pr.P);
        }
        s_cost[k][lane] = cv;
    }
    __syncthreads();
    if (k == 0 && inimg) {
        float best_cost = pr.cost[cidx];
        for (int g = 0; g < G; g++) {
            const float cv = s_cost[g][lane];
            if (cv < best_cost) {
                const int e = s_guess[g][lane];
                bx = (int)(int16_t)(e & 0xffff); by = e >> 16; best_cost = cv;
            }
        }
        pr.nnf[nidx * 2] = (int16_t)bx;
        pr.nnf[nidx * 2 + 1] = (int16_t)by;
        pr.cost[cidx] = best_cost;
    }
}

int pm_search_rows(int w, int h, int R, int problems, int npairs, bool table)
{
    const int quarter_wgs = ((w + kBlock - 1) / kBlock) * ((h + kBlock - 1) / kBlock) * 4 * problems * npairs;
    return (table && R == 9 && quarter_wgs < EPPM_SEARCH_HALF_BELOW_WGS) ? 2 : 4;
}

void launch_pm_random_search(const PmBatch& b, const PmRngDev& rng, const float* lut, int R, int search_range, int num_guess,
                             hipStream_t s)
{
    dim3 grid(rng.gx * rng.gy * 4 * b.n * b.npairs), block(64 * (num_guess + 1));
    const bool have_pc = b.p[0].P.pc2 && (b.n < 2 || b.p[1].P.pc2);
    if (rng.rand_tab && (R == 9 || R == 17)) {
        dim3 blockt(64 * num_guess);
        const bool half = pm_search_rows(b.p[0].P.w, b.p[0].P.h, R, b.n, b.npairs, true) == 2;
        if (pm_has_parity(b, R, EPPM_PARITY_SEARCH)) {
            if (half)
                hipLaunchKernelGGL((k_pm_random_search<9, 2, true, 2>), dim3(grid.x * 2), dim3(32 * num_guess), 0, s, b, rng, lut, R, search_range, num_guess);
            else if (R == 9) hipLaunchKernelGGL((k_pm_random_search<9, 2, true>), grid, blockt, 0, s, b, rng, lut, R, search_range, num_guess);
            else hipLaunchKernelGGL((k_pm_random_search<17, 2, true>), grid, blockt, 0, s, b, rng, lut, R, search_range, num_guess);
            return;
        }
        if (half) {
            hipLaunchKernelGGL((k_pm_random_search<9, 0, true, 2>), dim3(grid.x * 2), dim3(32 * num_guess), 0, s, b, rng, lut, R, search_range, num_guess);
            return;
        }
        if (R == 9) hipLaunchKernelGGL((k_pm_random_search<9, 0, true>), grid, blockt, 0, s, b, rng, lut, R, search_range, num_guess);
        else if (have_pc) hipLaunchKernelGGL((k_pm_random_search<17, 1, true>), grid, blockt, 0, s, b, rng, lut, R, search_range, num_guess);
        else hipLaunchKernelGGL((k_pm_random_search<17, 0, true>), grid, blockt, 0, s, b, rng, lut, R, search_range, num_guess);
        return;
    }
    if (R == 17 && have_pc && EPPM_SEARCH_PK17) hipLaunchKernelGGL((k_pm_random_search<17, 1>), grid, block, 0, s, b, rng, lut, R, search_range, num_guess);
    else if (R == 9) hipLaunchKernelGGL(k_pm_random_search<9>, grid, block, 0, s, b, rng, lut, R, search_range, num_guess);
    else if (R == 17) hipLaunchKernelGGL(k_pm_random_search<17>, grid, block, 0, s, b, rng, lut, R, search_range, num_guess);
    else hipLaunchKernelGGL(k_pm_random_search<0>, grid, block, 0, s, b, rng, lut, R, search_range, num_guess);
}

}
```

### eppm_amd/csrc/launchers_ref_abi.cpp

```cpp
#include "api_internal.h"

using namespace eppm;

namespace {
struct DevState {
    float *lut_pm = nullptr, *lut_wmf = nullptr, *lut_blf = nullptr;
    int lut_R = -1;
    void* scratch[9] = {nullptr, nullptr, nullptr, nullptr, nullptr, nullptr, nullptr, nullptr, nullptr};
    size_t scratch_bytes[9] = {0, 0, 0, 0, 0, 0, 0, 0, 0};
    std::map<std::tuple<int, int, int, unsigned long long>, eppm_pm_rng*> rngs;
};
std::mutex g_mu;
std::map<int, DevState> g_dev;
hipStream_t g_stream = nullptr;
eppm_params g_prm = {9, 10, 30, 6, 10, 20, 1234ULL, 0, kNumLevels};
int g_launch_status = EPPM_OK;

int dev_state(DevState** out)
{
    int d = 0;
    HIPCHK(hipGetDevice(&d));
    DevState& s = g_dev[d];
    if (s.lut_R != g_prm.patch_r) {
        (void)hipFree(s.lut_pm); s.lut_pm = nullptr;
        CHK(upload_pm_lut(&s.lut_pm, g_prm.patch_r));
        s.lut_R = g_prm.patch_r;
    }
    if (!s.lut_wmf) CHK(upload_wmf_lut(&s.lut_wmf));
    if (!s.lut_blf) CHK(upload_blf_lut(&s.lut_blf));
    *out = &s;
    return EPPM_OK;
}
int get_scratch(DevState* s, size_t bytes, void** out, int slot = 0)
{
    if (s->scratch_bytes[slot] < bytes) {
        (void)hipStreamSynchronize(g_stream);
        (void)hipFree(s->scratch[slot]);
        s->scratch[slot] = nullptr; s->scratch_bytes[slot] = 0;
        HIPCHK(hipMalloc(&s->scratch[slot], bytes));
        s->scratch_bytes[slot] = bytes;
    }
    *out = s->scratch[slot];
    return EPPM_OK;
}
int get_rng(DevState* s, int w, int h, eppm_pm_rng** out)
{
    auto key = std::make_tuple(w, h, g_prm.num_guess, g_prm.seed);
    auto it = s->rngs.find(key);
    if (it == s->rngs.end()) {
        eppm_pm_rng* r = nullptr;
        CHK(rng_create(&r, w, h, g_prm));
        it = s->rngs.emplace(key, r).first;
    }
    *out = it->second;
    return EPPM_OK;
}
int mk_planes(DevState* ds, PlanesH* out, const void* i1, const void* i2, const void* c1, const void* c2, int w, int h, size_t ip, size_t cp)
{
    void *a = nullptr, *b = nullptr;
    CHK(get_scratch(ds, (size_t)w * h * 16, &a, 2));
    CHK(get_scratch(ds, (size_t)w * h * 16, &b, 3));
    launch_pack(a, w, (const uint32_t*)i1, (int)(ip / 4), (const uint8_t*)c1, (int)cp, w, h, g_stream);
    launch_pack(b, w, (const uint32_t*)i2, (int)(ip / 4), (const uint8_t*)c2, (int)cp, w, h, g_stream);
    out->pk1 = a; out->pk2 = b; out->w = w; out->h = h; out->pitch = w;
    return EPPM_OK;
}
int finish() { HIPCHK(hipGetLastError()); return EPPM_OK; }
int split_scratch(DevState* ds, int w, int h, float** out)
{
    *out = nullptr;
    if (!opt_force_split()) return EPPM_OK;
    void* p = nullptr;
    CHK(get_scratch(ds, (size_t)w * h * 36 * 4, &p, 8));
    *out = (float*)p;
    return EPPM_OK;
}
int copy_d2d(void* dst, const void* src, size_t bytes)
{
    HIPCHK(hipMemcpyAsync(dst, src, bytes, hipMemcpyDeviceToDevice, g_stream));
    return EPPM_OK;
}
}

#define LAUNCHER_BEGIN std::lock_guard<std::mutex> lk_(g_mu); DevState* ds = nullptr; g_launch_status = dev_state(&ds); if (g_launch_status != EPPM_OK) return
#define LAUNCHER_BEGIN_INT std::lock_guard<std::mutex> lk_(g_mu); DevState* ds = nullptr; CHK(dev_state(&ds))

extern "C" int eppm_set_launcher_stream(void* s) { std::lock_guard<std::mutex> lk(g_mu); g_stream = (hipStream_t)s; return EPPM_OK; }
extern "C" int eppm_set_launcher_params(const eppm_params* p)
{
    std::lock_guard<std::mutex> lk(g_mu);
    if (!p) return eppm_default_params(&g_prm);
    CHK(check_params(*p));
    g_prm = *p;
    return EPPM_OK;
}

extern "C" int eppm_pm_rng_create(eppm_pm_rng** out, int w, int h, const eppm_params* p)
{
    if (!out || w < 1 || h < 1) return set_err(EPPM_ERR_ARG, "eppm_pm_rng_create: bad argument");
    eppm_params q;
    eppm_default_params(&q);
    if (p) q = *p;
    CHK(check_params(q));
    return rng_create(out, w, h, q);
}
extern "C" int eppm_pm_rng_reset(eppm_pm_rng* r)
{
    if (!r) return set_err(EPPM_ERR_ARG, "NULL rng");
    const size_t bytes = (size_t)r->gx * r->gy * 64 * 6 * 4;
    HIPCHK(hipMemcpy(r->work[0][r->cur[0]], r->iter_tab, bytes, hipMemcpyDeviceToDevice));
    return EPPM_OK;
}
extern "C" int eppm_pm_rng_destroy(eppm_pm_rng* r) { rng_free(r); return EPPM_OK; }
extern "C" int eppm_pm_rng_block_states(eppm_pm_rng* r, uint32_t* dst, size_t dst_words)
{
    if (!r || !dst) return set_err(EPPM_ERR_ARG, "NULL argument");
    const int nb = r->gx * r->gy;
    if (dst_words < (size_t)nb * 6) return set_err(EPPM_ERR_ARG, "dst too small");
    HIPCHK(hipDeviceSynchronize());
    HIPCHK(hipMemcpy2D(dst, 24, r->work[0][r->cur[0]], 64 * 24, 24, nb, hipMemcpyDeviceToHost));
    return EPPM_OK;
}
extern "C" int eppm_pm_gen_rand_field(eppm_pm_rng* r, eppm_short2* d_nnf, int w, int h, size_t disp_pitch)
{
    if (!r || !d_nnf || w != r->w || h != r->h) return set_err(EPPM_ERR_ARG, "eppm_pm_gen_rand_field: bad argument");
    std::lock_guard<std::mutex> lk(g_mu);
    PmBatch b;
    b.n = 1; b.cpitch = w; b.npitch = (int)(disp_pitch / 4);
    PlanesH P0;
    P0.pk1 = P0.pk2 = nullptr; P0.w = w; P0.h = h; P0.pitch = w;
    b.p[0] = mk_problem(P0, nullptr, (int16_t*)d_nnf, nullptr, r, 0);
    launch_pm_init_field(b, r->dev(), g_stream);
    return finish();
}
extern "C" int eppm_pm_cost_field(float* d_cost, const eppm_short2* d_nnf, const eppm_uchar4* i1, const eppm_uchar4* i2,
                                  const unsigned char* c1, const unsigned char* c2, int w, int h, size_t img_pitch,
                                  size_t cost_pitch, size_t disp_pitch, size_t census_pitch)
{
    LAUNCHER_BEGIN_INT;
    PmBatch b;
    b.n = 1; b.cpitch = (int)(cost_pitch / 4); b.npitch = (int)(disp_pitch / 4);
    PlanesH P;
    CHK(mk_planes(ds, &P, i1, i2, c1, c2, w, h, img_pitch, census_pitch));
    b.p[0] = mk_problem(P, d_cost, (int16_t*)d_nnf, nullptr, nullptr, 0);
    launch_pm_cost_field(b, ds->lut_pm, g_prm.patch_r, g_stream);
    return finish();
}
extern "C" int eppm_pm_seg_propagate(float* d_cost, eppm_short2* d_nnf, const eppm_uchar4* i1, const eppm_uchar4* i2,
                                     const unsigned char* c1, const unsigned char* c2, int w, int h, size_t img_pitch,
                                     size_t cost_pitch, size_t disp_pitch, size_t census_pitch, int dir)
{
    LAUNCHER_BEGIN_INT;
    void* tmp = nullptr;
    CHK(get_scratch(ds, disp_pitch * h, &tmp));
    PmBatch b;
    b.n = 1; b.cpitch = (int)(cost_pitch / 4); b.npitch = (int)(disp_pitch / 4);
    PlanesH P;
    CHK(mk_planes(ds, &P, i1, i2, c1, c2, w, h, img_pitch, census_pitch));
    void* spec = nullptr;
    const bool speculative = opt_sweep_spec() >= 1;
    const size_t plane_bytes = cost_pitch * h;
    CHK(get_scratch(ds, plane_bytes * 8, &spec, 4));
    HIPCHK(hipMemsetAsync((char*)spec + plane_bytes * 4, 0xff, plane_bytes * 4, g_stream));
    b.cache_plane = plane_bytes / 4;
    void* wl = nullptr;
    if (speculative && sweep_list_on(opt_sweep_spec())) {
        b.wl_units = pm_worklist_units(w, h, g_prm.seg_len);
        const size_t wl_bytes = pm_worklist_words(w, h, g_prm.seg_len) * 4;
        CHK(get_scratch(ds, wl_bytes, &wl, 5));
        HIPCHK(hipMemsetAsync(wl, 0, wl_bytes, g_stream));
    }
    b.p[0] = mk_problem(P, d_cost, (int16_t*)d_nnf, (int16_t*)tmp, nullptr, 0, (float*)spec, (int32_t*)((char*)spec + plane_bytes * 4), (uint32_t*)wl);
    for (int d = 0; d < 4; d++)
        if (dir < 0 || dir == d) sweep(b, ds->lut_pm, g_prm, d, g_stream, speculative);
    if (b.p[0].nnf != (int16_t*)d_nnf) HIPCHK(hipMemcpyAsync(d_nnf, b.p[0].nnf, disp_pitch * h, hipMemcpyDeviceToDevice, g_stream));
    return finish();
}
extern "C" int eppm_pm_jump_propagate(float* d_cost, eppm_short2* d_nnf, const eppm_uchar4* i1, const eppm_uchar4* i2,
                                      const unsigned char* c1, const unsigned char* c2, int w, int h, size_t img_pitch,
                                      size_t cost_pitch, size_t disp_pitch, size_t census_pitch)
{
    LAUNCHER_BEGIN_INT;
    void* tmp = nullptr;
    CHK(get_scratch(ds, disp_pitch * h, &tmp));
    PmBatch b;
    b.n = 1; b.cpitch = (int)(cost_pitch / 4); b.npitch = (int)(disp_pitch / 4);
    PlanesH P;
    CHK(mk_planes(ds, &P, i1, i2, c1, c2, w, h, img_pitch, census_pitch));
    b.p[0] = mk_problem(P, d_cost, (int16_t*)d_nnf, (int16_t*)tmp, nullptr, 0);
    jump(b, ds->lut_pm, g_prm, g_stream);
    if (b.p[0].nnf != (int16_t*)d_nnf) HIPCHK(hipMemcpyAsync(d_nnf, b.p[0].nnf, disp_pitch * h, hipMemcpyDeviceToDevice, g_stream));
    return finish();
}
extern "C" int eppm_pm_parallel_propagate(float* d_cost, eppm_short2* d_nnf, const eppm_uchar4* i1, const eppm_uchar4* i2,
                                          const unsigned char* c1, const unsigned char* c2, int w, int h, size_t img_pitch,
                                          size_t cost_pitch, size_t disp_pitch, size_t census_pitch)
{
    LAUNCHER_BEGIN_INT;
    void* tmp = nullptr;
    CHK(get_scratch(ds, disp_pitch * h, &tmp));
    PmBatch b;
    b.n = 1; b.cpitch = (int)(cost_pitch / 4); b.npitch = (int)(disp_pitch / 4);
    PlanesH P;
    CHK(mk_planes(ds, &P, i1, i2, c1, c2, w, h, img_pitch, census_pitch));
    b.p[0] = mk_problem(P, d_cost, (int16_t*)d_nnf, (int16_t*)tmp, nullptr, 0);
    neighbor(b, ds->lut_pm, g_prm, 1, g_stream);
    if (b.p[0].nnf != (int16_t*)d_nnf) HIPCHK(hipMemcpyAsync(d_nnf, b.p[0].nnf, disp_pitch * h, hipMemcpyDeviceToDevice, g_stream));
    return finish();
}
extern "C" int eppm_pm_random_search(eppm_pm_rng* r, float* d_cost, eppm_short2* d_nnf, const eppm_uchar4* i1, const eppm_uchar4* i2,
                                     const unsigned char* c1, const unsigned char* c2, int w, int h, size_t img_pitch,
                                     size_t cost_pitch, size_t disp_pitch, size_t census_pitch)
{
    if (!r || w != r->w || h != r->h) return set_err(EPPM_ERR_ARG, "eppm_pm_random_search: bad rng");
    LAUNCHER_BEGIN_INT;
    if (r->G != g_prm.num_guess) return set_err(EPPM_ERR_ARG, "rng was created for num_guess=%d", r->G);
    PmBatch b;
    b.n = 1; b.cpitch = (int)(cost_pitch / 4); b.npitch = (int)(disp_pitch / 4);
    PlanesH P;
    CHK(mk_planes(ds, &P, i1, i2, c1, c2, w, h, img_pitch, census_pitch));
    b.p[0] = mk_problem(P, d_cost, (int16_t*)d_nnf, nullptr, r, 0);
    if (opt_rand_table() == 2 && (g_prm.patch_r == 9 || g_prm.patch_r == 17)) {
        void* tab = nullptr;
        CHK(get_scratch(ds, (size_t)r->gx * r->gy * 512 * r->G * sizeof(int16_t), &tab, 7));
        PmRngDev d = r->dev();
        launch_pm_rand_table(d, r->work[0][r->cur[0]], (int16_t*)tab, r->G, g_stream);
        d.rand_tab = (const int16_t*)tab;
        launch_pm_random_search(b, d, ds->lut_pm, g_prm.patch_r, g_prm.search_range, g_prm.num_guess, g_stream);
        return finish();
    }
    search(b, r, ds->lut_pm, g_prm, g_stream);
    return finish();
}
extern "C" int eppm_gauss_filter_rgba(eppm_uchar4* d_out, const eppm_uchar4* d_in, size_t pitch, int h, int w, float sigma, int radius)
{
    if (radius < 0 || radius > 6) return set_err(EPPM_ERR_ARG, "radius %d out of range [0,6]", radius);
    std::lock_guard<std::mutex> lk(g_mu);
    launch_gauss_rgba((uint32_t*)d_out, (const uint32_t*)d_in, (int)(pitch / 4), h, w, sigma, radius, g_stream);
    return finish();
}
extern "C" int eppm_resize_rgba(eppm_uchar4* d_out, size_t out_pitch, int outH, int outW, const eppm_uchar4* d_in, size_t in_pitch,
                                int h, int w, float ratio)
{
    std::lock_guard<std::mutex> lk(g_mu);
    launch_resize_rgba((uint32_t*)d_out, (int)(out_pitch / 4), outH, outW, (const uint32_t*)d_in, (int)(in_pitch / 4), h, w, ratio, g_stream);
    return finish();
}
extern "C" int eppm_resize_flow(eppm_float2* d_out, int outH, int outW, const eppm_float2* d_in, int h, int w, float ratio)
{
    std::lock_guard<std::mutex> lk(g_mu);
    launch_resize_flow((float*)d_out, outH, outW, (const float*)d_in, h, w, ratio, 1.0f, g_stream);
    return finish();
}
extern "C" int eppm_flow_upsample(eppm_float2* d_out, int h, int w, const eppm_float2* d_coarse, int hc, int wc, const eppm_uchar4* d_guide,
                                  size_t guide_pitch)
{
    if (!d_out || !d_coarse || !d_guide || h < 1 || w < 1 || hc < 1 || wc < 1) return set_err(EPPM_ERR_ARG, "eppm_flow_upsample: bad argument");
    if (guide_pitch < (size_t)w * 4 || (guide_pitch & 3)) return set_err(EPPM_ERR_ARG, "eppm_flow_upsample: bad pitch %zu", guide_pitch);
    if ((unsigned long long)h * (unsigned long long)guide_pitch >= (1ULL << 32) || (unsigned long long)h * (unsigned long long)w >= (1ULL << 30))
        return set_err(EPPM_ERR_ARG, "eppm_flow_upsample: size %dx%d out of range", w, h);
    LAUNCHER_BEGIN_INT;
    launch_flow_jbu((float*)d_out, (const float*)d_coarse, (const uint32_t*)d_guide, (int)(guide_pitch / 4), w, h, wc, hc, ds->lut_blf, g_stream);
    HIPCHK(hipStreamSynchronize(g_stream));
    return finish();
}

extern "C" void baoCudaCensusTransform(unsigned char* d_census1, unsigned char* d_census2, eppm_uchar4* d_img1, eppm_uchar4* d_img2,
                                       int w, int h, size_t img_pitch, size_t census_pitch)
{
    std::lock_guard<std::mutex> lk(g_mu);
    launch_census(d_census1, (int)census_pitch, nullptr, 0, (const uint32_t*)d_img1, (int)(img_pitch / 4), w, h, g_stream);
    launch_census(d_census2, (int)census_pitch, nullptr, 0, (const uint32_t*)d_img2, (int)(img_pitch / 4), w, h, g_stream);
    g_launch_status = finish();
}

extern "C" void baoCudaPatchMatchMultiscalePrepare(eppm_uchar4** pImgPyr1, eppm_uchar4** pImgPyr2, unsigned char** pCensusPyr1,
        unsigned char** pCensusPyr2, eppm_uchar4** pTempPyr1, eppm_uchar4** pTempPyr2, int* arrH, int* arrW,
        size_t* arrPitchUchar4, size_t* arrPitchUchar1, int nLevels, eppm_uchar4* d_img1, eppm_uchar4* d_img2, int h, int w)
{
    std::lock_guard<std::mutex> lk(g_mu);
    hipStream_t s = g_stream;
    const float ratio = 0.5f;
    const float baseSigma = (1 / ratio - 1);
    const int n = (int)(log(0.25) / (double)logf(ratio));
    const float nSigma = baseSigma * n;
    for (int k = 0; k < 2; k++) {
        uint32_t** pyr = (uint32_t**)(k ? pImgPyr2 : pImgPyr1);
        uint32_t** tmp = (uint32_t**)(k ? pTempPyr2 : pTempPyr1);
        const uint32_t* raw = (const uint32_t*)(k ? d_img2 : d_img1);
        launch_gauss_rgba(pyr[0], raw, (int)(arrPitchUchar4[0] / 4), h, w, .5f, 2, s);
        for (int i = 1; i < nLevels; i++) {
            if (i <= n) {
                const float sigma = baseSigma * i;
                launch_gauss_rgba(tmp[0], pyr[0], (int)(arrPitchUchar4[0] / 4), arrH[0], arrW[0], sigma, (int)(sigma * 3), s);
                launch_resize_rgba(pyr[i], (int)(arrPitchUchar4[i] / 4), arrH[i], arrW[i], tmp[0], (int)(arrPitchUchar4[0] / 4), arrH[0], arrW[0], (float)pow(ratio, i), s);
            } else {
                const int j = i - n;
                launch_gauss_rgba(tmp[j], pyr[j], (int)(arrPitchUchar4[j] / 4), arrH[j], arrW[j], nSigma, (int)(nSigma * 3), s);
                launch_resize_rgba(pyr[i], (int)(arrPitchUchar4[i] / 4), arrH[i], arrW[i], tmp[j], (int)(arrPitchUchar4[j] / 4), arrH[j], arrW[j],
                                   (float)pow(ratio, i) * arrW[0] / arrW[j], s);
            }
        }
    }
    for (int i = 0; i < nLevels; i++) {
        launch_census(pCensusPyr1[i], (int)arrPitchUchar1[i], nullptr, 0, (const uint32_t*)pImgPyr1[i], (int)(arrPitchUchar4[i] / 4), arrW[i], arrH[i], s);
        launch_census(pCensusPyr2[i], (int)arrPitchUchar1[i], nullptr, 0, (const uint32_t*)pImgPyr2[i], (int)(arrPitchUchar4[i] / 4), arrW[i], arrH[i], s);
    }
    g_launch_status = finish();
}

extern "C" void baoCudaPatchMatch(eppm_short2* d_disp_vec, float* d_cost, eppm_uchar4* d_img1, eppm_uchar4* d_img2,
        unsigned char* d_census1, unsigned char* d_census2, int w, int h, size_t img_pitch, size_t cost_pitch,
        size_t disp_pitch, size_t census_pitch)
{
    LAUNCHER_BEGIN;
    eppm_pm_rng* r = nullptr;
    g_launch_status = get_rng(ds, w, h, &r);
    if (g_launch_status != EPPM_OK) return;
    void* tmp = nullptr;
    g_launch_status = get_scratch(ds, disp_pitch * h, &tmp);
    if (g_launch_status != EPPM_OK) return;
    PmBatch b;
    b.n = 1; b.cpitch = (int)(cost_pitch / 4); b.npitch = (int)(disp_pitch / 4);
    PlanesH P;
    g_launch_status = mk_planes(ds, &P, d_img1, d_img2, d_census1, d_census2, w, h, img_pitch, census_pitch);
    if (g_launch_status != EPPM_OK) return;
    void* spec = nullptr;
    const size_t plane_bytes = cost_pitch * h;
    g_launch_status = get_scratch(ds, plane_bytes * 8, &spec, 4);
    if (g_launch_status != EPPM_OK) return;
    b.cache_plane = plane_bytes / 4;
    void* wl = nullptr;
    b.wl_units = pm_worklist_units(w, h, g_prm.seg_len);
    g_launch_status = get_scratch(ds, pm_worklist_words(w, h, g_prm.seg_len) * 4, &wl, 5);
    if (g_launch_status != EPPM_OK) return;
    b.p[0] = mk_problem(P, d_cost, (int16_t*)d_disp_vec, (int16_t*)tmp, r, 0, (float*)spec, (int32_t*)((char*)spec + plane_bytes * 4), sweep_list_on(opt_sweep_spec()) ? (uint32_t*)wl : nullptr);
    run_patchmatch(b, r, ds->lut_pm, g_prm, g_stream, opt_sweep_spec());
    if (b.p[0].nnf != (int16_t*)d_disp_vec && (g_launch_status = copy_d2d(d_disp_vec, b.p[0].nnf, disp_pitch * h)) != EPPM_OK) return;
    g_launch_status = finish();
}

extern "C" void baoCudaLeftRightCheck(eppm_short2* d_disp_vec, float* d_cost, eppm_short2* d_disp_vec2, float* d_cost2,
        int w, int h, size_t cost_pitch, size_t disp_pitch)
{
    std::lock_guard<std::mutex> lk(g_mu);
    launch_lr_check((int16_t*)d_disp_vec, d_cost, (const int16_t*)d_disp_vec2, w, h, (int)(cost_pitch / 4), (int)(disp_pitch / 4), g_stream);
    launch_lr_check((int16_t*)d_disp_vec2, d_cost2, (const int16_t*)d_disp_vec, w, h, (int)(cost_pitch / 4), (int)(disp_pitch / 4), g_stream);
    g_launch_status = finish();
}

extern "C" void baoCudaOutlierRemoval(eppm_short2* d_disp_vec, float* d_cost, int w, int h, size_t cost_pitch, size_t disp_pitch)
{
    LAUNCHER_BEGIN;
    void* tmp = nullptr;
    g_launch_status = get_scratch(ds, disp_pitch * h, &tmp);
    if (g_launch_status != EPPM_OK) return;
    if ((g_launch_status = copy_d2d(tmp, d_disp_vec, disp_pitch * h)) != EPPM_OK) return;
    launch_outlier((int16_t*)d_disp_vec, d_cost, (const int16_t*)tmp, w, h, (int)(cost_pitch / 4), (int)(disp_pitch / 4), g_stream);
    g_launch_status = finish();
}

extern "C" void baoCudaWeightedMedianFilter(eppm_short2* d_disp_vec, float* d_cost, eppm_uchar4* d_img, int w, int h,
        size_t img_pitch, size_t cost_pitch, size_t disp_pitch, int num_iter, bool is_only_occlusion)
{
    (void)d_cost; (void)cost_pitch;
    LAUNCHER_BEGIN;
    void* tmp = nullptr;
    g_launch_status = get_scratch(ds, disp_pitch * h, &tmp);
    if (g_launch_status != EPPM_OK) return;
    void* ws = nullptr;
    g_launch_status = get_scratch(ds, wmf_workspace_words(w, h, num_iter) * 4, &ws, 1);
    if (g_launch_status != EPPM_OK) return;
    int16_t* res = launch_wmf((int16_t*)d_disp_vec, (int16_t*)tmp, (const uint32_t*)d_img, (int)(img_pitch / 4), w, h, (int)(disp_pitch / 4),
                              ds->lut_wmf, num_iter, is_only_occlusion ? 1 : 0, (uint32_t*)ws, g_stream);
    if (res != (int16_t*)d_disp_vec && (g_launch_status = copy_d2d(d_disp_vec, res, disp_pitch * h)) != EPPM_OK) return;
    g_launch_status = finish();
}

extern "C" void baoCudaFillHole(eppm_short2* d_disp_vec, float* d_cost, eppm_uchar4* d_img, int w, int h,
        size_t img_pitch, size_t cost_pitch, size_t disp_pitch)
{
    (void)d_cost; (void)cost_pitch;
    LAUNCHER_BEGIN;
    void* tmp = nullptr;
    g_launch_status = get_scratch(ds, disp_pitch * h, &tmp);
    if (g_launch_status != EPPM_OK) return;
    if ((g_launch_status = copy_d2d(tmp, d_disp_vec, disp_pitch * h)) != EPPM_OK) return;
    launch_fill_holes((int16_t*)d_disp_vec, (const int16_t*)tmp, (const uint32_t*)d_img, (int)(img_pitch / 4), w, h, (int)(disp_pitch / 4), g_stream);
    g_launch_status = finish();
}

extern "C" void baoCudaNNF2Flow(eppm_float2* d_flow, eppm_short2* d_disp_vec, int w, int h, size_t disp_pitch, size_t flow_pitch)
{
    std::lock_guard<std::mutex> lk(g_mu);
    launch_nnf2flow((float*)d_flow, (int)(flow_pitch / 8), (const int16_t*)d_disp_vec, (int)(disp_pitch / 4), w, h, g_stream);
    g_launch_status = finish();
}

extern "C" void baoCudaBLFCostFilterRefine(eppm_float2* d_flow_vec, eppm_uchar4* d_img1, eppm_uchar4* d_img2, unsigned char* d_census1,
        unsigned char* d_census2, int w, int h, size_t img_pitch, size_t census_pitch)
{
    LAUNCHER_BEGIN;
    PlanesH P;
    g_launch_status = mk_planes(ds, &P, d_img1, d_img2, d_census1, d_census2, w, h, img_pitch, census_pitch);
    if (g_launch_status != EPPM_OK) return;
    float* cost9 = nullptr;
    if ((g_launch_status = split_scratch(ds, w, h, &cost9)) != EPPM_OK) return;
    launch_c2f_refine(P, (float*)d_flow_vec, ds->lut_pm, g_prm.patch_r, cost9, g_stream, kOnePair, opt_no_split() != 0);
    g_launch_status = finish();
}

extern "C" void baoCudaBLF_C2F(eppm_float2** pFlowPyr, eppm_uchar4** pImgPyr1, eppm_uchar4** pImgPyr2, unsigned char** pCensusPyr1,
        unsigned char** pCensusPyr2, eppm_float2** pTempPyr1, eppm_float2** pTempPyr2, int* arrH, int* arrW,
        size_t* arrPitchUchar4, size_t* arrPitchUchar1, int nLayerIdx)
{
    (void)pTempPyr1; (void)pTempPyr2;
    LAUNCHER_BEGIN;
    const int l = nLayerIdx;
    launch_resize_flow((float*)pFlowPyr[l], arrH[l], arrW[l], (const float*)pFlowPyr[l + 1], arrH[l + 1], arrW[l + 1], 2.0f, 1.0f, g_stream);
    launch_mul_scalar((float*)pFlowPyr[l], 2.0f, arrH[l], arrW[l], g_stream);
    PlanesH P;
    g_launch_status = mk_planes(ds, &P, pImgPyr1[l], pImgPyr2[l], pCensusPyr1[l], pCensusPyr2[l], arrW[l], arrH[l], arrPitchUchar4[l], arrPitchUchar1[l]);
    if (g_launch_status != EPPM_OK) return;
    float* cost9 = nullptr;
    if ((g_launch_status = split_scratch(ds, arrW[l], arrH[l], &cost9)) != EPPM_OK) return;
    launch_c2f_refine(P, (float*)pFlowPyr[l], ds->lut_pm, g_prm.patch_r, cost9, g_stream, kOnePair, opt_no_split() != 0);
    g_launch_status = finish();
}

#ifdef EPPM_TEST_HOOKS
extern "C" int eppm_test_c2f_refine_batch(float* d_flow, const uint32_t* d_img1, const uint32_t* d_img2, const uint8_t* d_census1,
        const uint8_t* d_census2, int w, int h, int npairs)
{
    if (!d_flow || !d_img1 || !d_img2 || !d_census1 || !d_census2 || w < 1 || h < 1 || npairs < 1)
        return set_err(EPPM_ERR_ARG, "eppm_test_c2f_refine_batch: bad argument");
    LAUNCHER_BEGIN_INT;
    const size_t n = (size_t)w * h, stride = n * 16;
    void *a = nullptr, *b = nullptr, *f = nullptr;
    CHK(get_scratch(ds, stride * npairs, &a, 2));
    CHK(get_scratch(ds, stride * npairs, &b, 3));
    CHK(get_scratch(ds, stride * npairs, &f, 0));
    for (int p = 0; p < npairs; p++) {
        launch_pack((char*)a + p * stride, w, d_img1 + p * n, w, d_census1 + p * n, w, w, h, g_stream);
        launch_pack((char*)b + p * stride, w, d_img2 + p * n, w, d_census2 + p * n, w, w, h, g_stream);
        CHK(copy_d2d((char*)f + p * stride, d_flow + p * n * 2, n * 8));
    }
    PlanesH P;
    P.pk1 = a; P.pk2 = b; P.w = w; P.h = h; P.pitch = w;
    launch_c2f_refine(P, (float*)f, ds->lut_pm, g_prm.patch_r, nullptr, g_stream, Batch{npairs, stride}, opt_no_split() != 0);
    for (int p = 0; p < npairs; p++) CHK(copy_d2d(d_flow + p * n * 2, (char*)f + p * stride, n * 8));
    return finish();
}
#endif

extern "C" void baoCudaFlowSmoothing(eppm_float2* d_flow, eppm_uchar4* d_img, int w, int h, size_t img_pitch, size_t flow_pitch)
{
    LAUNCHER_BEGIN;
    void* tmp = nullptr;
    g_launch_status = get_scratch(ds, flow_pitch * h, &tmp);
    if (g_launch_status != EPPM_OK) return;
    if ((g_launch_status = copy_d2d(tmp, d_flow, flow_pitch * h)) != EPPM_OK) return;
    launch_flow_blf((float*)d_flow, (const float*)tmp, (const uint32_t*)d_img, (int)(img_pitch / 4), w, h, (int)(flow_pitch / 8), ds->lut_blf, g_stream);
    g_launch_status = finish();
}

extern "C" int eppm_flow_to_color(eppm_uchar4* d_rgba, const eppm_float2* d_flow, int h, int w, float max_disp_x, float max_disp_y)
{
    if (!d_rgba || !d_flow || h < 1 || w < 1) return set_err(EPPM_ERR_ARG, "eppm_flow_to_color: bad argument");
    LAUNCHER_BEGIN_INT;
    (void)ds;
    launch_flow_to_color((uint32_t*)d_rgba, (const float*)d_flow, h, w, max_disp_x, max_disp_y, g_stream);
    return finish();
}
extern "C" int eppm_fb_occlusion(uint8_t* d_occ, const eppm_float2* d_flow, const eppm_float2* d_other, int h, int w, float alpha, float beta)
{
    if (!d_occ || !d_flow || !d_other || h < 1 || w < 1) return set_err(EPPM_ERR_ARG, "eppm_fb_occlusion: bad argument");
    if (!(alpha >= 0 && isfinite(alpha)) || !(beta >= 0 && isfinite(beta)))
        return set_err(EPPM_ERR_ARG, "eppm_fb_occlusion: alpha %g, beta %g must be finite and >= 0", alpha, beta);
    LAUNCHER_BEGIN_INT;
    (void)ds;
    launch_fb_occlusion(d_occ, nullptr, (const float*)d_flow, 0, (const float*)d_other, 0, h, w, alpha, beta, 1, 1, g_stream);
    return finish();
}
extern "C" int eppm_temporal_prior(eppm_short2* d_prior, const eppm_short2* d_prev, int h, int w, int backward)
{
    if (!d_prior || !d_prev || h < 1 || w < 1 || h > 32767 || w > 32767) return set_err(EPPM_ERR_ARG, "eppm_temporal_prior: bad argument");
    if ((unsigned long long)h * (unsigned long long)w >= (1ULL << 30)) return set_err(EPPM_ERR_ARG, "eppm_temporal_prior: size %dx%d out of range", w, h);
    LAUNCHER_BEGIN_INT;
    void* keys = nullptr;
    CHK(get_scratch(ds, (size_t)w * h * 4, &keys, 6));
    TemporalArgs a{};
    a.prev[0] = (const int16_t*)d_prev; a.prior[0] = (int16_t*)d_prior; a.keys[0] = (int32_t*)keys; a.step[0] = backward ? -1 : 1;
    a.w = w; a.h = h; a.ndir = 1; a.nslots = 1; a.armed[0] = 1u;
    launch_temporal_keys_init(a.keys[0], w * h, g_stream);
    launch_temporal_splat(a, g_stream);
    launch_temporal_gather(a, g_stream);
    return finish();
}
extern "C" int eppm_temporal_prior_batch(eppm_short2* d_prior, const eppm_short2* d_prev, int h, int w, int backward, int npairs, const uint8_t* armed)
{
    if (!d_prior || !d_prev || h < 1 || w < 1 || h > 32767 || w > 32767 || npairs < 1 || npairs > kTemporalMaxSlots)
        return set_err(EPPM_ERR_ARG, "eppm_temporal_prior_batch: bad argument");
    if ((unsigned long long)h * (unsigned long long)w * (unsigned long long)npairs >= (1ULL << 30))
        return set_err(EPPM_ERR_ARG, "eppm_temporal_prior_batch: %d slots of %dx%d out of range", npairs, w, h);
    LAUNCHER_BEGIN_INT;
    void* keys = nullptr;
    CHK(get_scratch(ds, (size_t)w * h * 4 * npairs, &keys, 6));
    TemporalArgs a{};
    a.prev[0] = (const int16_t*)d_prev; a.prior[0] = (int16_t*)d_prior; a.keys[0] = (int32_t*)keys; a.step[0] = backward ? -1 : 1;
    a.w = w; a.h = h; a.ndir = 1; a.nslots = npairs; a.stride = (size_t)w * h * 4;
    for (int k = 0; k < npairs; k++)
        if (!armed || armed[k]) a.armed[k >> 5] |= 1u << (k & 31);
    launch_temporal_keys_init(a.keys[0], w * h * npairs, g_stream);
    launch_temporal_splat(a, g_stream);
    launch_temporal_gather(a, g_stream);
    return finish();
}
extern "C" int eppm_interpolate_frames(void* d_rgba_out, size_t out_pitch, const void* d_rgba1, const void* d_rgba2, size_t in_pitch,
                                       const eppm_float2* d_flow, const uint8_t* d_occ1, const uint8_t* d_occ2, int h, int w, float t)
{
    if (!d_rgba_out || !d_rgba1 || !d_rgba2 || !d_flow || !d_occ1 || !d_occ2 || h < 1 || w < 1) return set_err(EPPM_ERR_ARG, "eppm_interpolate_frames: bad argument");
    if (!(t >= 0.0f && t <= 1.0f)) return set_err(EPPM_ERR_ARG, "eppm_interpolate_frames: t = %g outside [0, 1]", t);
    if (in_pitch < (size_t)w * 4 || out_pitch < (size_t)w * 4 || (in_pitch & 3) || (out_pitch & 3))
        return set_err(EPPM_ERR_ARG, "eppm_interpolate_frames: bad pitch %zu / %zu", in_pitch, out_pitch);
    if ((unsigned long long)h * (unsigned long long)w >= (1ULL << 31)) return set_err(EPPM_ERR_ARG, "eppm_interpolate_frames: size %dx%d out of range", w, h);
    LAUNCHER_BEGIN_INT;
    const size_t plane = ((size_t)h * w + 63) & ~(size_t)63;
    void* scr = nullptr;
    CHK(get_scratch(ds, plane * 16, &scr, 6));
    InterpArgs a{};
    a.img1 = (const uint8_t*)d_rgba1; a.img2 = (const uint8_t*)d_rgba2; a.img_pitch = in_pitch;
    a.flow = (const float*)d_flow;
    a.occ1 = d_occ1; a.occ2 = d_occ2;
    a.keys = (uint64_t*)scr; a.fill1 = (int32_t*)((char*)scr + plane * 8); a.fill2 = (int32_t*)((char*)scr + plane * 12); a.plane = plane;
    a.rgba[0] = (uint8_t*)d_rgba_out; a.rgba_pitch = out_pitch;
    a.h = h; a.w = w; a.nt = 1; a.t[0] = t;
    launch_interp_splat(a, 1, g_stream);
    launch_interp_fill(a, 1, g_stream);
    launch_interp_blend(a, 1, g_stream);
    return finish();
}
extern "C" int eppm_track_step_frames(eppm_tracker* t, const void* d_rgba1, const void* d_rgba2, size_t pitch, const eppm_float2* d_flow,
                                      const eppm_float2* d_flow_bwd, int h, int w)
{
    if (!t || !d_rgba1 || !d_rgba2 || !d_flow || !d_flow_bwd) return set_err(EPPM_ERR_ARG, "eppm_track_step_frames: NULL argument");
    int th, tw;
    const int device = tracker_device(t, &th, &tw);
    if (h != th || w != tw) return set_err(EPPM_ERR_ARG, "eppm_track_step_frames: %dx%d planes, the tracker is %dx%d", w, h, tw, th);
    if (pitch < (size_t)w * 4 || (pitch & 3)) return set_err(EPPM_ERR_ARG, "eppm_track_step_frames: bad pitch %zu", pitch);
    std::lock_guard<std::mutex> lk(g_mu);
    int d = 0;
    HIPCHK(hipGetDevice(&d));
    if (d != device) return set_err(EPPM_ERR_ARG, "eppm_track_step_frames: the tracker lives on device %d, the current device is %d", device, d);
    TrackIn in{(const uint8_t*)d_rgba1, (const uint8_t*)d_rgba2, pitch, (const float*)d_flow, (const float*)d_flow_bwd, h, w};
    CHK(tracker_step_on(t, in, g_stream, nullptr));
    HIPCHK(hipStreamSynchronize(g_stream));
    return finish();
}
extern "C" int eppm_tfilter_step_frames(eppm_tfilter* f, int slot, const void* d_rgba1, const void* d_rgba2, size_t pitch,
                                        const eppm_float2* d_flow_bwd, const uint8_t* d_occ2, int cut)
{
    if (!f || !d_rgba1 || !d_rgba2 || !d_flow_bwd || !d_occ2) return set_err(EPPM_ERR_ARG, "eppm_tfilter_step_frames: NULL argument");
    int h, w, nslots;
    const int device = tfilter_device(f, &h, &w, &nslots);
    if (slot < 0 || slot >= nslots) return set_err(EPPM_ERR_ARG, "eppm_tfilter_step_frames: slot %d, the filter has %d", slot, nslots);
    if (pitch < (size_t)w * 4 || (pitch & 3)) return set_err(EPPM_ERR_ARG, "eppm_tfilter_step_frames: bad pitch %zu", pitch);
    std::lock_guard<std::mutex> lk(g_mu);
    int d = 0;
    HIPCHK(hipGetDevice(&d));
    if (d != device) return set_err(EPPM_ERR_ARG, "eppm_tfilter_step_frames: the filter lives on device %d, the current device is %d", device, d);
    TFilterArgs in{};
    in.img1 = (const uint8_t*)d_rgba1; in.img2 = (const uint8_t*)d_rgba2; in.img_pitch = pitch;
    in.bwd = (const float*)d_flow_bwd; in.occ2 = d_occ2;
    in.n = 1;
    const uint8_t c = cut != 0;
    CHK(tfilter_step_on(f, in, slot, &c, g_stream, nullptr));
    HIPCHK(hipStreamSynchronize(g_stream));
    return finish();
}
extern "C" int eppm_stab_step_frames(eppm_stab* f, int slot, const void* d_rgba2, size_t pitch, const eppm_float2* d_flow, const uint8_t* d_occ1, int cut)
{
    if (!f || !d_rgba2 || !d_flow || !d_occ1) return set_err(EPPM_ERR_ARG, "eppm_stab_step_frames: NULL argument");
    int h, w, nslots;
    const int device = stab_device(f, &h, &w, &nslots);
    if (slot < 0 || slot >= nslots) return set_err(EPPM_ERR_ARG, "eppm_stab_step_frames: slot %d, the stabiliser has %d", slot, nslots);
    if (pitch < (size_t)w * 4 || (pitch & 3)) return set_err(EPPM_ERR_ARG, "eppm_stab_step_frames: bad pitch %zu", pitch);
    std::lock_guard<std::mutex> lk(g_mu);
    int d = 0;
    HIPCHK(hipGetDevice(&d));
    if (d != device) return set_err(EPPM_ERR_ARG, "eppm_stab_step_frames: the stabiliser lives on device %d, the current device is %d", device, d);
    StabArgs in{};
    in.img2 = (const uint8_t*)d_rgba2; in.img_pitch = pitch;
    in.fwd = (const float*)d_flow; in.occ1 = d_occ1;
    in.n = 1;
    const uint8_t c = cut != 0;
    CHK(stab_step_on(f, in, slot, &c, g_stream, nullptr));
    HIPCHK(hipStreamSynchronize(g_stream));
    return finish();
}
extern "C" int eppm_cutdet_step_frames(eppm_cutdet* f, int slot, const void* d_rgba1, const void* d_rgba2, size_t pitch, const eppm_float2* d_flow_bwd,
                                       const uint8_t* d_occ1, const uint8_t* d_occ2)
{
    if (!f || !d_rgba1 || !d_rgba2 || !d_flow_bwd || !d_occ1 || !d_occ2) return set_err(EPPM_ERR_ARG, "eppm_cutdet_step_frames: NULL argument");
    int h, w, nslots;
    const int device = cutdet_device(f, &h, &w, &nslots);
    if (slot < 0 || slot >= nslots) return set_err(EPPM_ERR_ARG, "eppm_cutdet_step_frames: slot %d, the detector has %d", slot, nslots);
    if (pitch < (size_t)w * 4 || (pitch & 3)) return set_err(EPPM_ERR_ARG, "eppm_cutdet_step_frames: bad pitch %zu", pitch);
    std::lock_guard<std::mutex> lk(g_mu);
    int d = 0;
    HIPCHK(hipGetDevice(&d));
    if (d != device) return set_err(EPPM_ERR_ARG, "eppm_cutdet_step_frames: the detector lives on device %d, the current device is %d", device, d);
    CutArgs in{};
    in.img1 = (const uint8_t*)d_rgba1; in.img2 = (const uint8_t*)d_rgba2; in.img_pitch = pitch;
    in.bwd = (const float*)d_flow_bwd; in.occ1 = d_occ1; in.occ2 = d_occ2;
    in.n = 1;
    CHK(cutdet_step_on(f, in, slot, g_stream, nullptr));
    HIPCHK(hipStreamSynchronize(g_stream));
    return finish();
}
void bao_cuda_convert_flow_to_colorshow(uchar4* rgbflow, float2* flow_vec, int h, int w, float max_disp_x, float max_disp_y)
{
    g_launch_status = eppm_flow_to_color((eppm_uchar4*)rgbflow, (const eppm_float2*)flow_vec, h, w, max_disp_x, max_disp_y);
}

extern "C" int eppm_launcher_status(void) { return g_launch_status; }

int launcher_finish() { return finish(); }
```

### eppm_amd/csrc/pm_device.cuh

```cuda
#pragma once
#include "eppm_device.cuh"

#ifndef EPPM_PARITY_SEARCH
#define EPPM_PARITY_SEARCH 1
#endif
#ifndef EPPM_PARITY_SPEC
#define EPPM_PARITY_SPEC 0
#endif
#ifndef EPPM_PARITY_COST
#define EPPM_PARITY_COST 1
#endif
#ifndef EPPM_COST_FIELD_TILE
#define EPPM_COST_FIELD_TILE 1
#endif
#ifndef EPPM_LPC9
#ifdef EPPM_TOL
#define EPPM_LPC9 32
#else
#define EPPM_LPC9 16
#endif
#endif
#ifndef EPPM_LPC17
#define EPPM_LPC17 64
#endif
#ifndef EPPM_LPC9_SPEC
#ifdef EPPM_TOL
#define EPPM_LPC9_SPEC 32
#else
#define EPPM_LPC9_SPEC 16
#endif
#endif
#ifndef EPPM_LPC17_SPEC
#define EPPM_LPC17_SPEC 64
#endif
#ifndef EPPM_LPC_SWITCH_WAVES
#define EPPM_LPC_SWITCH_WAVES (2 * 1024)
#endif
#ifndef EPPM_SWEEP_PRE
#define EPPM_SWEEP_PRE 1
#endif
#ifndef EPPM_SWEEP_GB
#define EPPM_SWEEP_GB 7
#endif
#ifndef EPPM_SWEEP_GB_SPEC
#define EPPM_SWEEP_GB_SPEC 3
#endif
#ifndef EPPM_SWEEP_TILE
#define EPPM_SWEEP_TILE 1
#endif
#ifdef EPPM_SWEEP_WAVES
#define EPPM_SWEEP_OCC __attribute__((amdgpu_waves_per_eu(EPPM_SWEEP_WAVES, EPPM_SWEEP_WAVES)))
#else
#define EPPM_SWEEP_OCC
#endif
#ifndef EPPM_SPEC_COOP17_MAX
#define EPPM_SPEC_COOP17_MAX 32
#endif
#ifndef EPPM_MERGED_COOP9_MAX
#define EPPM_MERGED_COOP9_MAX 16
#endif
#ifdef EPPM_SEARCH_WAVES
#define EPPM_SEARCH_OCC __attribute__((amdgpu_waves_per_eu(EPPM_SEARCH_WAVES, EPPM_SEARCH_WAVES)))
#else
#define EPPM_SEARCH_OCC
#endif
#ifndef EPPM_SEARCH_SKIP_SAME
#define EPPM_SEARCH_SKIP_SAME 1
#endif
#ifndef EPPM_SEARCH_HALF_BELOW_WGS
#define EPPM_SEARCH_HALF_BELOW_WGS 1024
#endif
#ifndef EPPM_SEARCH_PK17
#define EPPM_SEARCH_PK17 1
#endif

namespace eppm {

__device__ __forceinline__ Planes to_dev(const PlanesH& h)
{
    Planes p;
    p.pk1 = (const float4*)h.pk1; p.pk2 = (const float4*)h.pk2;
    p.w = h.w; p.h = h.h; p.pitch = h.pitch;
    return p;
}

__device__ __forceinline__ PmProblem pm_problem(const PmBatch& B, unsigned q)
{
    PmProblem p = B.p[q % (unsigned)B.n];
    const unsigned pair = q / (unsigned)B.n;
    p.P.pk1 = pair_ptr_opt(p.P.pk1, B.stride, pair);
    p.P.pk2 = pair_ptr_opt(p.P.pk2, B.stride, pair);
    p.P.pc1 = pair_ptr_opt(p.P.pc1, B.stride, pair);
    p.P.pc2 = pair_ptr_opt(p.P.pc2, B.stride, pair);
    p.P.pp1 = pair_ptr_opt(p.P.pp1, B.stride, pair);
    p.P.pp2 = pair_ptr_opt(p.P.pp2, B.stride, pair);
    p.cost = pair_ptr_opt(p.cost, B.stride, pair);
    p.nnf = pair_ptr_opt(p.nnf, B.stride, pair);
    p.nnf_alt = pair_ptr_opt(p.nnf_alt, B.stride, pair);
    p.spec = pair_ptr_opt(p.spec, B.stride, pair);
    p.scand = pair_ptr_opt(p.scand, B.stride, pair);
    p.wl = pair_ptr_opt(p.wl, B.stride, pair);
    p.seed = pair_ptr_opt(p.seed, B.stride, pair);
    p.rng_work = pair_ptr_opt(p.rng_work, B.stride, pair);
    p.rng_work_next = pair_ptr_opt(p.rng_work_next, B.stride, pair);
    return p;
}

__device__ __forceinline__ Xorwow load_state(const uint32_t* p)
{
    Xorwow s;
    s.v0 = p[0]; s.v1 = p[1]; s.v2 = p[2]; s.v3 = p[3]; s.v4 = p[4]; s.d = p[5];
    return s;
}
__device__ __forceinline__ void store_state(uint32_t* p, const Xorwow& s)
{
    p[0] = s.v0; p[1] = s.v1; p[2] = s.v2; p[3] = s.v3; p[4] = s.v4; p[5] = s.d;
}

template <int RT> struct SearchLut { using type = PatchLutT<RT + 1>; };
template <> struct SearchLut<0> { using type = PatchLut; };

__device__ __forceinline__ float patch_dist_any(const Planes& P, const PatchLut& L, int R, int x1, int y1, int x2, int y2) { return patch_dist(P, L, R, x1, y1, x2, y2); }
template <int M> __device__ __forceinline__ float patch_dist_any(const Planes&, const PatchLutT<M>&, int, int, int, int, int) { return 0.0f; }

#define EPPM_PM_PRAGMA_(x) _Pragma(#x)
#define EPPM_PM_UNROLL(n) EPPM_PM_PRAGMA_(unroll n)
template <int RT, int PK = 0, class LUT>
__device__ __forceinline__ float search_patch_dist(const Planes& P, const LUT& L, int R, const float4* __restrict__ s_src, int TW,
                                                   int tx, int ty, int x1, int y1, int x2, int y2, const PlanesH& PH)
{
    if (RT == 0) return patch_dist_any(P, L, R, x1, y1, x2, y2);
    constexpr int S = RT + 1;
    const int pitch16 = P.pitch << 4;
    const rgbf c1 = texel_rgb(s_src[(ty + RT) * TW + tx + RT]);
    const rgbf c2 = texel_rgb(texel_at(P.pk2, texel_off(pitch16, P.w, P.h, x2, y2)));
    PatchSum sum;
    constexpr int CS = tol_chunk(RT);
    static_assert(S % CS == 0, "whole chunks per row");
    if constexpr (PK == 2) {
        static_assert(S % 4 == 2, "a row = whole dwordx4 gathers + one dwordx2");
        const __amdgpu_buffer_rsrc_t rs = __builtin_amdgcn_make_buffer_rsrc(const_cast<uint32_t*>(PH.pp2), 0, 2 * P.h * PH.pp_pitch * 4, 0x00020000);
        const int xp = x2 - RT + PH.pp_pad;
        const int rb = ((xp & 1) * P.h) * PH.pp_pitch + (xp >> 1);
        uint32_t two = 2u;
        asm volatile("" : "+v"(two));
#pragma unroll 2
        for (int ii = 0; ii < S; ii++) {
            const int ro = (rb + iclamp(y2 + 2 * ii - RT, 0, P.h - 1) * PH.pp_pitch) * 4;
            const float4* __restrict__ srow = s_src + (ty + 2 * ii) * TW + tx;
            uint32_t wq[S];
#pragma unroll
            for (int g = 0; g < S / 4; g++) {
                const u32x4 v = __builtin_amdgcn_raw_buffer_load_b128(rs, ro + 16 * g, 0, 0);
                wq[4 * g] = v.x; wq[4 * g + 1] = v.y; wq[4 * g + 2] = v.z; wq[4 * g + 3] = v.w;
            }
            { const u32x2 v = __builtin_amdgcn_raw_buffer_load_b64(rs, ro + 4 * (S - 2), 0, 0); wq[S - 2] = v.x; wq[S - 1] = v.y; }
#ifdef EPPM_SEARCH_TERM_UNROLL
            constexpr int TU = EPPM_SEARCH_TERM_UNROLL;
#else
            constexpr int TU = (S % 5 == 0) ? 5 : (S % 9 == 0) ? 9 : S;
#endif
EPPM_PM_UNROLL((TU))
            for (int jj = 0; jj < S; jj++) {
                float ct, wt;
                patch_terms(srow[2 * jj], unpack_texel(wq[jj], two), c1, c2, L.gsp[ii * S + jj], L.tab(), ct, wt);
                sum.add(ct, wt);
                if ((jj + 1) % CS == 0) sum.flush();
            }
        }
        return sum.result();
    }
    const uint32_t* __restrict__ pc2 = PH.pc2;
    for (int ii = 0; ii < S; ii++) {
        const int i = 2 * ii - RT;
        const unsigned r2 = __umul24((unsigned)iclamp(y2 + i, 0, P.h - 1), (unsigned)pitch16);
        const float4* __restrict__ srow = s_src + (ty + 2 * ii) * TW + tx;
        for (int j0 = 0; j0 < S; j0 += 5) {
            float4 q1[5], q2[5];
            uint32_t w2[PK == 1 ? 5 : 1];
#pragma unroll
            for (int k = 0; k < 5; k++) {
                const int jj = min(j0 + k, S - 1);
                q1[k] = srow[2 * jj];
                const unsigned o2 = r2 + ((unsigned)iclamp(x2 + 2 * jj - RT, 0, P.w - 1) << 4);
                if (PK == 1) w2[k] = *reinterpret_cast<const uint32_t*>(reinterpret_cast<const char*>(pc2) + (o2 >> 2));
                else q2[k] = texel_at(P.pk2, o2);
            }
#pragma unroll
            for (int k = 0; k < 5; k++) {
                if (j0 + k < S) {
                    float ct, wt;
                    if (PK == 1) q2[k] = make_texel(w2[k], w2[k] >> 24);
                    patch_terms(q1[k], q2[k], c1, c2, L.gsp[ii * S + j0 + k], L.tab(), ct, wt);
                    sum.add(ct, wt);
                    if ((j0 + k + 1) % CS == 0) sum.flush();
                }
            }
        }
    }
    return sum.result();
}

template <int RT>
__device__ __forceinline__ void pm_stage_tile(float4* __restrict__ s_src, const Planes& P, int bx, int by, int tid)
{
    constexpr int TW = kBlock + 2 * RT;
    const int x0 = bx * kBlock - RT, y0 = by * kBlock - RT;
    for (int t = tid; t < TW * TW; t += 256) {
        const int sy = iclamp(y0 + t / TW, 0, P.h - 1), sx = iclamp(x0 + t % TW, 0, P.w - 1);
        s_src[t] = P.pk1[(unsigned)(sy * P.pitch + sx)];
    }
}

static inline bool pm_parity_adopted(int R, bool exact_adopts)
{
#ifdef EPPM_TOL
    (void)exact_adopts;
    return R == 9 || R == 17;
#else
    return exact_adopts && R == 9;
#endif
}
static inline bool pm_has_parity(const PmBatch& b, int R, bool exact_adopts)
{
    return pm_parity_adopted(R, exact_adopts) && b.p[0].P.pp2 && (b.n < 2 || b.p[1].P.pp2);
}

template <int LPC>
__device__ __forceinline__ float dpp_prev_lane(float v)
{
    if (LPC == 4) return __int_as_float(__builtin_amdgcn_update_dpp(0, __float_as_int(v), 0x93 , 0xf, 0xf, false));
    if (LPC == 16) return __int_as_float(__builtin_amdgcn_update_dpp(0, __float_as_int(v), 0x121 , 0xf, 0xf, false));
    return __int_as_float(__builtin_amdgcn_update_dpp(0, __float_as_int(v), 0x138 , 0xf, 0xf, false));
}

template <int R, int LPC>
__host__ __device__ constexpr int coop_chunk()
{
#ifdef EPPM_TOL
    return tol_chunk(R);
#else
    return ((R + 1) * (R + 1) + LPC - 1) / LPC;
#endif
}
template <int LPC, int CH, int NS, int NL>
__device__ __forceinline__ void coop_chain_sum(const float (&tc)[CH], const float (&tw)[CH], float& ac, float& aw)
{
#ifdef EPPM_TOL
    float pc = 0.0f, pw = 0.0f;
#pragma unroll
    for (int q = 0; q < CH; q++) patch_accum(pc, pw, tc[q], tw[q]);
#pragma unroll
    for (int ln = 0; ln < NL; ln++) {
        if (ln > 0) { ac = dpp_prev_lane<LPC>(ac); aw = dpp_prev_lane<LPC>(aw); }
        ac += pc; aw += pw;
    }
#else
#pragma unroll
    for (int ln = 0; ln < NL; ln++) {
        if (ln > 0) { ac = dpp_prev_lane<LPC>(ac); aw = dpp_prev_lane<LPC>(aw); }
#pragma unroll
        for (int q = 0; q < CH; q++) {
            if (ln * CH + q < NS) patch_accum(ac, aw, tc[q], tw[q]);
        }
    }
#endif
}

template <int RT, int LPC, class LUT>
__device__ __forceinline__ float coop_patch_dist(const Planes& P, const LUT& L, const float4* __restrict__ s_src, int TW, int tx, int ty,
                                                 int x2, int y2, int r)
{
    constexpr int S = RT + 1, NS = S * S, CH = coop_chunk<RT, LPC>(), NL = (NS + CH - 1) / CH;
    static_assert(NL <= LPC, "a lane per chunk");
    const int pitch16 = P.pitch << 4, wmax16 = (P.w - 1) << 4;
    const rgbf c1 = texel_rgb(s_src[(ty + RT) * TW + tx + RT]);
    const rgbf c2 = texel_rgb(texel_at(P.pk2, texel_off(pitch16, P.w, P.h, x2, y2)));
    const int t0 = r * CH;
    float tc[CH], tw[CH];
    float4 q2[CH];
    int so[CH];
#pragma unroll
    for (int k = 0; k < CH; k++) {
        const int t = min(t0 + k, NS - 1), ii = t / S, jj = t - ii * S;
        so[k] = (ty + 2 * ii) * TW + tx + 2 * jj;
        q2[k] = texel_at(P.pk2, texel_off16(pitch16, wmax16, P.h - 1, (x2 + 2 * jj - RT) << 4, y2 + 2 * ii - RT));
    }
#pragma unroll
    for (int k = 0; k < CH; k++) {
        tc[k] = 0.0f; tw[k] = 0.0f;
        if (t0 + k < NS) patch_terms(s_src[so[k]], q2[k], c1, c2, L.gsp[t0 + k], L.tab(), tc[k], tw[k]);
    }
    float ac = 0.0f, aw = 0.0f;
    coop_chain_sum<LPC, CH, NS, NL>(tc, tw, ac, aw);
    const int src = ((threadIdx.x & 63) / LPC) * LPC + (NL - 1);
    return __shfl(ac, src, 64) / __shfl(aw, src, 64);
}

__device__ __forceinline__ void merged_list_unit(uint32_t* __restrict__ wl, const PmBatch& B, int d, int px, int py)
{
    const bool row = (d & 1) == 0;
    const int along = row ? px : py, ln = row ? py : px, nseg = row ? B.nseg_row : B.nseg_col;
    const unsigned seg = (d < 2 && along < B.seg_len) ? 0u : (unsigned)(along / B.seg_len);
    const unsigned unit = (unsigned)ln * ((unsigned)(nseg + 1) >> 1) + (seg >> 1), U = (unsigned)B.wl_units, seq1 = (unsigned)B.merged_it + 1u;
    if (atomicMax(&wl[16 + 2 * U + d * U + unit], seq1) < seq1)
        wl[16 + 6 * U + d * U + atomicAdd(&wl[8 + 4 * (B.merged_it & 1) + d], 1u)] = unit;
}

template <int LPC> struct SweepTile { static constexpr int CPB = 256 / LPC, SEGS = (CPB >= 16) ? 4 : 2, LINES = CPB / SEGS; };
constexpr int kSpecMaxSteps = 16;

}
```

### eppm_amd/csrc/pm_driver.cpp

```cpp
#include "api_internal.h"

using namespace eppm;

PmProblem mk_problem(const PlanesH& P, float* cost, int16_t* nnf, int16_t* nnf_alt, eppm_pm_rng* rng, int k, float* spec, int32_t* scand, uint32_t* wl, int16_t* seed)
{
    PmProblem p;
    p.P = P; p.cost = cost; p.nnf = nnf; p.nnf_alt = nnf_alt; p.spec = spec; p.scand = scand; p.wl = wl; p.seed = seed;
    p.rng_work = rng ? rng->work[k][rng->cur[k]] : nullptr;
    p.rng_work_next = rng ? rng->work[k][rng->cur[k] ^ 1] : nullptr;
    return p;
}
void search(PmBatch& b, eppm_pm_rng* rng, const float* lut, const eppm_params& prm, hipStream_t s, int launch_no)
{
    PmRngDev d = rng->dev();
    if (rng->rand_tab && launch_no >= 0) d.rand_tab = rng->rand_tab + (size_t)launch_no * rng->rand_stride;
    launch_pm_random_search(b, d, lut, prm.patch_r, prm.search_range, prm.num_guess, s);
    for (int k = 0; k < b.n; k++) {
        std::swap(b.p[k].rng_work, b.p[k].rng_work_next);
        rng->cur[k] ^= 1;
    }
}
#ifndef EPPM_SPEC_FROM_ITER
#define EPPM_SPEC_FROM_ITER 2
#endif
#ifndef EPPM_SWEEP_LIST
#define EPPM_SWEEP_LIST 1
#endif
bool sweep_list_on(int mode) { return EPPM_SWEEP_LIST && mode != 2; }
#ifndef EPPM_SPEC_MIN_PIXELS
#define EPPM_SPEC_MIN_PIXELS 100000
#endif
static bool sweep_speculative(int iteration, long long pixels, int m)
{
    return m < 0 ? (iteration >= EPPM_SPEC_FROM_ITER && pixels >= EPPM_SPEC_MIN_PIXELS) : m != 0;
}
#ifndef EPPM_MERGED_FROM_ITER
#define EPPM_MERGED_FROM_ITER 5
#endif
#ifndef EPPM_MERGED_FROM_ITER_LARGE
#define EPPM_MERGED_FROM_ITER_LARGE 7
#endif
#ifndef EPPM_MERGED_LARGE_PIXELS
#define EPPM_MERGED_LARGE_PIXELS 65536
#endif
static bool sweeps_merged(int iteration, long long pixels, long long problem_pixels, int m)
{
    const int from = problem_pixels > EPPM_MERGED_LARGE_PIXELS ? EPPM_MERGED_FROM_ITER_LARGE : EPPM_MERGED_FROM_ITER;
    return m == 3 || (m < 0 && from >= 0 && iteration >= from && sweep_speculative(iteration, pixels, m));
}
void sweep(PmBatch& b, const float* lut, const eppm_params& prm, int dir, hipStream_t s, bool speculative)
{
    if (launch_pm_sweep(b, lut, prm.patch_r, prm.seg_len, dir, s, speculative))
        for (int k = 0; k < b.n; k++) std::swap(b.p[k].nnf, b.p[k].nnf_alt);
}
void jump(PmBatch& b, const float* lut, const eppm_params& prm, hipStream_t s)
{
    for (int step = 32; step >= 1; step /= 2) {
        launch_pm_jump(b, lut, prm.patch_r, step, s);
        for (int k = 0; k < b.n; k++) std::swap(b.p[k].nnf, b.p[k].nnf_alt);
    }
}
void neighbor(PmBatch& b, const float* lut, const eppm_params& prm, int launches, hipStream_t s)
{
    for (int q = 0; q < launches; q++) {
        launch_pm_neighbor(b, lut, prm.patch_r, s);
        for (int k = 0; k < b.n; k++) std::swap(b.p[k].nnf, b.p[k].nnf_alt);
    }
}
void run_patchmatch(PmBatch& b, eppm_pm_rng* rng, const float* lut, const eppm_params& prm, hipStream_t s, int spec_mode)
{
    pm_start(b, rng, lut, prm, s);
    pm_iterate(b, rng, lut, prm, s, spec_mode);
}
void pm_start(PmBatch& b, eppm_pm_rng* rng, const float* lut, const eppm_params& prm, hipStream_t s)
{
    b.sweep_seq = 0;
    launch_pm_init_field(b, rng->dev(), s);
    launch_pm_cost_field(b, lut, prm.patch_r, s);
}
void pm_iterate(PmBatch& b, eppm_pm_rng* rng, const float* lut, const eppm_params& prm, hipStream_t s, int spec_mode)
{
    for (int it = 0; it < prm.num_iter; it++) {
        if (prm.propagation == 1) jump(b, lut, prm, s);
        else if (prm.propagation == 2) neighbor(b, lut, prm, 10, s);
        else {
            const long long problem_pixels = (long long)b.p[0].P.w * b.p[0].P.h, pixels = problem_pixels * b.n * b.npairs;
            if (sweeps_merged(it, pixels, problem_pixels, spec_mode) && launch_pm_sweeps_merged(b, lut, prm.patch_r, prm.seg_len, it, s)) {  }
            else for (int dir = 0; dir < 4; dir++) sweep(b, lut, prm, dir, s, sweep_speculative(it, pixels, spec_mode));
        }
        search(b, rng, lut, prm, s, it);
    }
}
```

### eppm_amd/stages.py

```python
import ctypes as C

import numpy as np

from ._lib import CParams, check, check_launcher, lib, probe_dispatch
from .api import float2, short2, uchar4


class Dev:

    def __init__(self, arr=None, shape=None, dtype=None, pitched=False):
        if arr is not None:
            arr = np.ascontiguousarray(arr)
            shape, dtype = arr.shape, arr.dtype
        self.h, self.w = shape
        self.dtype = np.dtype(dtype)
        row = self.w * self.dtype.itemsize
        self.ptr = C.c_void_p()
        if pitched:
            pitch = C.c_size_t()
            check(lib().eppm_malloc_pitched(C.byref(self.ptr), C.byref(pitch), C.c_size_t(row), C.c_size_t(self.h)), "malloc_pitched")
            self.pitch = pitch.value
        else:
            check(lib().eppm_malloc_device(C.byref(self.ptr), C.c_size_t(row * self.h)), "malloc")
            self.pitch = row
        if arr is not None:
            self.put(arr)

    def put(self, arr):
        arr = np.ascontiguousarray(arr, self.dtype)
        row = self.w * self.dtype.itemsize
        check(lib().eppm_memcpy2d_h2d(self.ptr, C.c_size_t(self.pitch), arr.ctypes.data_as(C.c_void_p), C.c_size_t(row),
                                      C.c_size_t(row), C.c_size_t(self.h)), "h2d")

    def get(self):
        out = np.empty((self.h, self.w), self.dtype)
        row = self.w * self.dtype.itemsize
        check(lib().eppm_memcpy2d_d2h(out.ctypes.data_as(C.c_void_p), C.c_size_t(row), self.ptr, C.c_size_t(self.pitch),
                                      C.c_size_t(row), C.c_size_t(self.h)), "d2h")
        return out

    def free(self):
        if self.ptr:
            lib().eppm_free_device(self.ptr)
            self.ptr = C.c_void_p()

    def __del__(self):
        try:
            self.free()
        except Exception:
            pass


def set_params(params=None):
    check(lib().eppm_set_launcher_params(C.byref(params) if params is not None else None), "eppm_set_launcher_params")


def _sz(v):
    return C.c_size_t(v)


def probe_fast_exp(x):
    x = np.ascontiguousarray(x, np.float32)
    y = np.empty_like(x)
    check(lib().eppm_probe_fast_exp(x.ctypes.data_as(C.c_void_p), y.ctypes.data_as(C.c_void_p), x.size), "probe_fast_exp")
    return y


def probe_div_const(x, which):
    x = np.ascontiguousarray(x, np.float32)
    y = np.empty_like(x)
    check(lib().eppm_probe_div_const(x.ctypes.data_as(C.c_void_p), y.ctypes.data_as(C.c_void_p), x.size, which), "probe_div_const")
    return y


def probe_delta_table(d, which):
    x = np.ascontiguousarray(d, np.float32)
    y = np.empty_like(x)
    check(lib().eppm_probe_delta_table(x.ctypes.data_as(C.c_void_p), y.ctypes.data_as(C.c_void_p), x.size, which), "probe_delta_table")
    return y


def gauss_filter_rgba(img, sigma, radius):
    h, w = img.shape
    a, b = Dev(img, pitched=True), Dev(shape=(h, w), dtype=uchar4, pitched=True)
    check(lib().eppm_gauss_filter_rgba(b.ptr, a.ptr, _sz(a.pitch), h, w, C.c_float(sigma), radius), "gauss")
    return b.get()


def resize_rgba(img, out_h, out_w, ratio):
    h, w = img.shape
    a, b = Dev(img, pitched=True), Dev(shape=(out_h, out_w), dtype=uchar4, pitched=True)
    check(lib().eppm_resize_rgba(b.ptr, _sz(b.pitch), out_h, out_w, a.ptr, _sz(a.pitch), h, w, C.c_float(ratio)), "resize_rgba")
    return b.get()


def census_transform(img1, img2):
    h, w = img1.shape
    a, b = Dev(img1, pitched=True), Dev(img2, pitched=True)
    c1, c2 = Dev(shape=(h, w), dtype=np.uint8, pitched=True), Dev(shape=(h, w), dtype=np.uint8, pitched=True)
    lib().baoCudaCensusTransform(c1.ptr, c2.ptr, a.ptr, b.ptr, w, h, _sz(a.pitch), _sz(c1.pitch))
    check_launcher("baoCudaCensusTransform")
    return c1.get(), c2.get()


def prepare(raw1, raw2, dims):
    n = len(dims)
    h, w = dims[0]
    r1, r2 = Dev(raw1, pitched=True), Dev(raw2, pitched=True)
    p1 = [Dev(shape=d, dtype=uchar4, pitched=True) for d in dims]
    p2 = [Dev(shape=d, dtype=uchar4, pitched=True) for d in dims]
    t1 = [Dev(shape=d, dtype=uchar4, pitched=True) for d in dims]
    t2 = [Dev(shape=d, dtype=uchar4, pitched=True) for d in dims]
    c1 = [Dev(shape=d, dtype=np.uint8, pitched=True) for d in dims]
    c2 = [Dev(shape=d, dtype=np.uint8, pitched=True) for d in dims]

    def tab(bufs):
        return (C.c_void_p * n)(*[b.ptr for b in bufs])

    arrH = (C.c_int * n)(*[d[0] for d in dims])
    arrW = (C.c_int * n)(*[d[1] for d in dims])
    p4 = (C.c_size_t * n)(*[b.pitch for b in p1])
    pc = (C.c_size_t * n)(*[b.pitch for b in c1])
    lib().baoCudaPatchMatchMultiscalePrepare(tab(p1), tab(p2), tab(c1), tab(c2), tab(t1), tab(t2), arrH, arrW, p4, pc, n,
                                             r1.ptr, r2.ptr, h, w)
    check_launcher("baoCudaPatchMatchMultiscalePrepare")
    return [b.get() for b in p1], [b.get() for b in p2], [b.get() for b in c1], [b.get() for b in c2]


class PlaneSet:

    def __init__(self, img1, img2, c1, c2):
        self.h, self.w = img1.shape
        self.i1, self.i2 = Dev(img1, pitched=True), Dev(img2, pitched=True)
        self.c1, self.c2 = Dev(c1, pitched=True), Dev(c2, pitched=True)

    def args(self):
        return (self.i1.ptr, self.i2.ptr, self.c1.ptr, self.c2.ptr)


class PmRng:
    def __init__(self, w, h, params=None):
        self.p = C.c_void_p()
        self.w, self.h = w, h
        check(lib().eppm_pm_rng_create(C.byref(self.p), w, h, C.byref(params) if params is not None else None), "rng_create")

    def block_states(self):
        nb = ((self.w + 15) // 16) * ((self.h + 15) // 16)
        out = np.empty((nb, 6), np.uint32)
        check(lib().eppm_pm_rng_block_states(self.p, out.ctypes.data_as(C.c_void_p), _sz(out.size)), "rng_block_states")
        return out

    def __del__(self):
        try:
            if self.p:
                lib().eppm_pm_rng_destroy(self.p)
        except Exception:
            pass


def pm_gen_rand_field(rng):
    nnf = Dev(shape=(rng.h, rng.w), dtype=short2)
    check(lib().eppm_memset_device(nnf.ptr, 0, _sz(nnf.pitch * nnf.h)), "memset")
    check(lib().eppm_pm_gen_rand_field(rng.p, nnf.ptr, rng.w, rng.h, _sz(nnf.pitch)), "pm_gen_rand_field")
    return nnf.get()


def pm_cost_field(nnf, P):
    n, c = Dev(nnf), Dev(shape=(P.h, P.w), dtype=np.float32)
    check(lib().eppm_pm_cost_field(c.ptr, n.ptr, *P.args(), P.w, P.h, _sz(P.i1.pitch), _sz(c.pitch), _sz(n.pitch), _sz(P.c1.pitch)),
          "pm_cost_field")
    return c.get()


def pm_seg_propagate(cost, nnf, P, direction):
    n, c = Dev(nnf), Dev(cost)
    check(lib().eppm_pm_seg_propagate(c.ptr, n.ptr, *P.args(), P.w, P.h, _sz(P.i1.pitch), _sz(c.pitch), _sz(n.pitch), _sz(P.c1.pitch),
                                      direction), "pm_seg_propagate")
    return c.get(), n.get()


def pm_jump_propagate(cost, nnf, P):
    n, c = Dev(nnf), Dev(cost)
    check(lib().eppm_pm_jump_propagate(c.ptr, n.ptr, *P.args(), P.w, P.h, _sz(P.i1.pitch), _sz(c.pitch), _sz(n.pitch), _sz(P.c1.pitch)),
          "pm_jump_propagate")
    return c.get(), n.get()


def pm_parallel_propagate(cost, nnf, P):
    n, c = Dev(nnf), Dev(cost)
    check(lib().eppm_pm_parallel_propagate(c.ptr, n.ptr, *P.args(), P.w, P.h, _sz(P.i1.pitch), _sz(c.pitch), _sz(n.pitch),
                                           _sz(P.c1.pitch)), "pm_parallel_propagate")
    return c.get(), n.get()


def pm_random_search(rng, cost, nnf, P):
    n, c = Dev(nnf), Dev(cost)
    check(lib().eppm_pm_random_search(rng.p, c.ptr, n.ptr, *P.args(), P.w, P.h, _sz(P.i1.pitch), _sz(c.pitch), _sz(n.pitch),
                                      _sz(P.c1.pitch)), "pm_random_search")
    return c.get(), n.get()


def patchmatch(P):
    n, c = Dev(shape=(P.h, P.w), dtype=short2), Dev(shape=(P.h, P.w), dtype=np.float32)
    lib().baoCudaPatchMatch(n.ptr, c.ptr, *P.args(), P.w, P.h, _sz(P.i1.pitch), _sz(c.pitch), _sz(n.pitch), _sz(P.c1.pitch))
    check_launcher("baoCudaPatchMatch")
    return n.get(), c.get()


def left_right_check(nnf1, cost1, nnf2, cost2):
    h, w = nnf1.shape
    a, b, c, d = Dev(nnf1), Dev(cost1), Dev(nnf2), Dev(cost2)
    lib().baoCudaLeftRightCheck(a.ptr, b.ptr, c.ptr, d.ptr, w, h, _sz(b.pitch), _sz(a.pitch))
    check_launcher("baoCudaLeftRightCheck")
    return a.get(), b.get(), c.get(), d.get()


def outlier_removal(nnf, cost):
    h, w = nnf.shape
    a, b = Dev(nnf), Dev(cost)
    lib().baoCudaOutlierRemoval(a.ptr, b.ptr, w, h, _sz(b.pitch), _sz(a.pitch))
    check_launcher("baoCudaOutlierRemoval")
    return a.get(), b.get()


def weighted_median(nnf, img, num_iter=20, only_occlusion=True):
    h, w = nnf.shape
    a, i = Dev(nnf), Dev(img, pitched=True)
    lib().baoCudaWeightedMedianFilter(a.ptr, None, i.ptr, w, h, _sz(i.pitch), _sz(w * 4), _sz(a.pitch), num_iter, C.c_bool(only_occlusion))
    check_launcher("baoCudaWeightedMedianFilter")
    return a.get()


def fill_holes(nnf, img):
    h, w = nnf.shape
    a, i = Dev(nnf), Dev(img, pitched=True)
    lib().baoCudaFillHole(a.ptr, None, i.ptr, w, h, _sz(i.pitch), _sz(w * 4), _sz(a.pitch))
    check_launcher("baoCudaFillHole")
    return a.get()


def nnf2flow(nnf):
    h, w = nnf.shape
    a, f = Dev(nnf), Dev(shape=(h, w), dtype=float2)
    lib().baoCudaNNF2Flow(f.ptr, a.ptr, w, h, _sz(a.pitch), _sz(f.pitch))
    check_launcher("baoCudaNNF2Flow")
    return f.get()


def resize_flow(flow, out_h, out_w, ratio=2.0):
    h, w = flow.shape
    a, b = Dev(flow), Dev(shape=(out_h, out_w), dtype=float2)
    check(lib().eppm_resize_flow(b.ptr, out_h, out_w, a.ptr, h, w, C.c_float(ratio)), "resize_flow")
    return b.get()


def flow_upsample(coarse, img):
    h, w = img.shape
    hc, wc = coarse.shape
    a, i, b = Dev(coarse), Dev(img, pitched=True), Dev(shape=(h, w), dtype=float2)
    check(lib().eppm_flow_upsample(b.ptr, h, w, a.ptr, hc, wc, i.ptr, _sz(i.pitch)), "eppm_flow_upsample")
    return b.get()


def c2f_refine(flow, P):
    f = Dev(flow)
    lib().baoCudaBLFCostFilterRefine(f.ptr, *P.args(), P.w, P.h, _sz(P.i1.pitch), _sz(P.c1.pitch))
    check_launcher("baoCudaBLFCostFilterRefine")
    return f.get()


def c2f_refine_batch(flows, planes):
    n = len(flows)
    h, w = flows[0].shape
    f = Dev(np.concatenate([np.ascontiguousarray(x, float2) for x in flows]))
    i1, i2, c1, c2 = (Dev(np.concatenate([np.ascontiguousarray(p[k]) for p in planes])) for k in range(4))
    check(lib().eppm_test_c2f_refine_batch(f.ptr, i1.ptr, i2.ptr, c1.ptr, c2.ptr, w, h, n), "eppm_test_c2f_refine_batch")
    out = f.get()
    return [out[k * h:(k + 1) * h] for k in range(n)]


def blf_c2f(flow_coarse, P_fine, coarse_dims):
    ch, cw = coarse_dims
    fine = Dev(shape=(P_fine.h, P_fine.w), dtype=float2)
    coarse = Dev(flow_coarse)
    tab = lambda a, b: (C.c_void_p * 2)(a, b)
    arrH = (C.c_int * 2)(P_fine.h, ch)
    arrW = (C.c_int * 2)(P_fine.w, cw)
    p4 = (C.c_size_t * 2)(P_fine.i1.pitch, 0)
    pc = (C.c_size_t * 2)(P_fine.c1.pitch, 0)
    lib().baoCudaBLF_C2F(tab(fine.ptr, coarse.ptr), tab(P_fine.i1.ptr, None), tab(P_fine.i2.ptr, None), tab(P_fine.c1.ptr, None),
                         tab(P_fine.c2.ptr, None), None, None, arrH, arrW, p4, pc, 0)
    check_launcher("baoCudaBLF_C2F")
    return fine.get()


def flow_smoothing(flow, img):
    h, w = flow.shape
    f, i = Dev(flow), Dev(img, pitched=True)
    lib().baoCudaFlowSmoothing(f.ptr, i.ptr, w, h, _sz(i.pitch), _sz(f.pitch))
    check_launcher("baoCudaFlowSmoothing")
    return f.get()


def temporal_prior(prev, backward=False):
    d_prev = Dev(np.ascontiguousarray(prev, short2))
    d_out = Dev(shape=prev.shape, dtype=short2)
    check(lib().eppm_temporal_prior(d_out.ptr, d_prev.ptr, d_prev.h, d_prev.w, int(bool(backward))), "eppm_temporal_prior")
    check(lib().eppm_device_synchronize(), "eppm_device_synchronize")
    return d_out.get()


def temporal_prior_batch(prevs, backward=False, armed=None, calls=1):
    prevs = np.ascontiguousarray(prevs, short2)
    n, h, w = prevs.shape
    d_prev = Dev(prevs.reshape(n * h, w))
    d_out = Dev(shape=(n * h, w), dtype=short2)
    flags = None if armed is None else (C.c_uint8 * n)(*[int(bool(x)) for x in armed])
    out = []
    for _ in range(calls):
        check(lib().eppm_temporal_prior_batch(d_out.ptr, d_prev.ptr, h, w, int(bool(backward)), n, flags), "eppm_temporal_prior_batch")
        check(lib().eppm_device_synchronize(), "eppm_device_synchronize")
        out.append(d_out.get().reshape(n, h, w))
    return out[0] if calls == 1 else out


def flow_to_color(flow, max_disp_x=20.0, max_disp_y=20.0):
    h, w = flow.shape
    f, c = Dev(flow), Dev(shape=(h, w), dtype=uchar4)
    check(lib().eppm_flow_to_color(c.ptr, f.ptr, h, w, C.c_float(max_disp_x), C.c_float(max_disp_y)), "eppm_flow_to_color")
    return c.get()
```

Measured before the change: 237.2 Mflow-vectors/s.

## Pre-test random-search guesses on centre rows and evaluate survivors cooperatively

```diff
diff --git a/eppm_amd/_lib.py b/eppm_amd/_lib.py
--- a/eppm_amd/_lib.py
+++ b/eppm_amd/_lib.py
@@ -98,7 +98,7 @@
 
 
 TEST_SYMBOLS = ["eppm_test_set_option", "eppm_test_c2f_refine_batch", "eppm_probe_c2f_window", "eppm_probe_dispatch", "eppm_probe_fast_exp", "eppm_probe_div_const", "eppm_probe_delta_table",
-                "eppm_probe_unpack_texel", "eppm_probe_pm_parity", "eppm_probe_ctx_rng_states"]
+                "eppm_probe_unpack_texel", "eppm_probe_pm_parity", "eppm_probe_ctx_rng_states", "eppm_test_pm_search", "eppm_probe_search_pretest"]
 
 _variant = None
 
diff --git a/eppm_amd/csrc/api_internal.h b/eppm_amd/csrc/api_internal.h
--- a/eppm_amd/csrc/api_internal.h
+++ b/eppm_amd/csrc/api_internal.h
@@ -55,15 +55,18 @@
 EPPM_HIDDEN extern std::atomic<int> g_opt_sweep_spec;
 EPPM_HIDDEN extern std::atomic<int> g_opt_no_split;
 EPPM_HIDDEN extern std::atomic<int> g_opt_force_split;
+EPPM_HIDDEN extern std::atomic<int> g_opt_search_pre;
 static inline int opt_rand_table() { return g_opt_rand_table.load(); }
 static inline int opt_sweep_spec() { return g_opt_sweep_spec.load(); }
 static inline int opt_no_split() { return g_opt_no_split.load(); }
 static inline int opt_force_split() { return g_opt_force_split.load(); }
+static inline int opt_search_pre() { return g_opt_search_pre.load(); }
 #else
 static constexpr int opt_rand_table() { return 1; }
 static constexpr int opt_sweep_spec() { return -1; }
 static constexpr int opt_no_split() { return 0; }
 static constexpr int opt_force_split() { return 0; }
+static constexpr int opt_search_pre() { return -1; }
 #endif
 
 
@@ -99,15 +102,15 @@
 EPPM_HIDDEN void pooled_stream_destroy(hipStream_t s, int device);
 
 EPPM_HIDDEN eppm::PmProblem mk_problem(const eppm::PlanesH& P, float* cost, int16_t* nnf, int16_t* nnf_alt, eppm_pm_rng* rng, int k, float* spec = nullptr,
-                                       int32_t* scand = nullptr, uint32_t* wl = nullptr, int16_t* seed = nullptr);
-EPPM_HIDDEN void search(eppm::PmBatch& b, eppm_pm_rng* rng, const float* lut, const eppm_params& prm, hipStream_t s, int launch_no = -1);
+                                       int32_t* scand = nullptr, uint32_t* wl = nullptr, int16_t* seed = nullptr, float* restw = nullptr);
+EPPM_HIDDEN void search(eppm::PmBatch& b, eppm_pm_rng* rng, const float* lut, const eppm_params& prm, hipStream_t s, int launch_no = -1, bool pretest = false);
 EPPM_HIDDEN bool sweep_list_on(int mode);
 EPPM_HIDDEN void sweep(eppm::PmBatch& b, const float* lut, const eppm_params& prm, int dir, hipStream_t s, bool speculative = false);
 EPPM_HIDDEN void jump(eppm::PmBatch& b, const float* lut, const eppm_params& prm, hipStream_t s);
 EPPM_HIDDEN void neighbor(eppm::PmBatch& b, const float* lut, const eppm_params& prm, int launches, hipStream_t s);
-EPPM_HIDDEN void run_patchmatch(eppm::PmBatch& b, eppm_pm_rng* rng, const float* lut, const eppm_params& prm, hipStream_t s, int spec_mode);
-EPPM_HIDDEN void pm_start(eppm::PmBatch& b, eppm_pm_rng* rng, const float* lut, const eppm_params& prm, hipStream_t s);
-EPPM_HIDDEN void pm_iterate(eppm::PmBatch& b, eppm_pm_rng* rng, const float* lut, const eppm_params& prm, hipStream_t s, int spec_mode);
+EPPM_HIDDEN void run_patchmatch(eppm::PmBatch& b, eppm_pm_rng* rng, const float* lut, const eppm_params& prm, hipStream_t s, int spec_mode, int pre_from = -1);
+EPPM_HIDDEN void pm_start(eppm::PmBatch& b, eppm_pm_rng* rng, const float* lut, const eppm_params& prm, hipStream_t s, int pre_from = -1);
+EPPM_HIDDEN void pm_iterate(eppm::PmBatch& b, eppm_pm_rng* rng, const float* lut, const eppm_params& prm, hipStream_t s, int spec_mode, int pre_from = -1);
 #ifndef EPPM_SWEEP_CACHE
 #define EPPM_SWEEP_CACHE 1
 #endif
diff --git a/eppm_amd/csrc/context.cpp b/eppm_amd/csrc/context.cpp
--- a/eppm_amd/csrc/context.cpp
+++ b/eppm_amd/csrc/context.cpp
@@ -78,6 +78,8 @@
     for (int16_t** p : {&c->nnf1, &c->nnf2, &c->nnf_tmp, &c->nnf_tmp2}) cv.plane(p, n2 * 4);
     for (float** p : {&c->cost1, &c->cost2}) cv.plane(p, n2 * 4);
     for (float** p : {&c->spec1, &c->spec2}) cv.plane(p, n2 * 4 * 4);
+    if (pm_search_pretest_form(c->W[L], c->H[L], c->prm.patch_r, 2, c->npairs))
+        for (float** p : {&c->restw1, &c->restw2}) cv.plane(p, n2 * 4);
     for (int32_t** p : {&c->scand1, &c->scand2}) cv.plane(p, n2 * 4 * 4);
     for (uint32_t** p : {&c->wl1, &c->wl2}) cv.plane(p, pm_worklist_words(c->W[L], c->H[L], c->prm.seg_len) * 4);
     for (int16_t** p : {&c->seed1, &c->seed2}) cv.plane(p, n2 * 4 * 4);
@@ -113,7 +115,7 @@
     HIPCHK(hipSetDevice(device));
     eppm_ctx* c = new eppm_ctx();
     c->device = device; c->prm = p; c->h = h; c->w = w; c->npairs = npairs; c->n_active = 1;
-    c->opt_sweep_spec = opt_sweep_spec(); c->opt_no_split = opt_no_split();
+    c->opt_sweep_spec = opt_sweep_spec(); c->opt_no_split = opt_no_split(); c->opt_search_pre = opt_search_pre();
     c->nl = pyr_init_dim(c->H, c->W, h, w, p.levels, 0.5f);
     const int L = c->nl - 1;
     if (c->H[L] < 1 || c->W[L] < 1 || (c->W[L] + p.seg_len - 1) / p.seg_len > 1024 || (c->H[L] + p.seg_len - 1) / p.seg_len > 1024) {
diff --git a/eppm_amd/csrc/context.h b/eppm_amd/csrc/context.h
--- a/eppm_amd/csrc/context.h
+++ b/eppm_amd/csrc/context.h
@@ -10,7 +10,7 @@
     int device = 0;
     hipStream_t stream = nullptr;
     bool own_stream = false;
-    int opt_sweep_spec = -1, opt_no_split = 0;
+    int opt_sweep_spec = -1, opt_no_split = 0, opt_search_pre = -1;
     eppm_params prm;
     int h = 0, w = 0, nl = 0;
     int stop_level = 0;
@@ -32,6 +32,7 @@
     float *spec1 = nullptr, *spec2 = nullptr;
     int32_t *scand1 = nullptr, *scand2 = nullptr;
     uint32_t *wl1 = nullptr, *wl2 = nullptr;
+    float *restw1 = nullptr, *restw2 = nullptr;
     int16_t *seed1 = nullptr, *seed2 = nullptr;
     uint32_t* wmf_ws = nullptr;
     bool flow_pending = false;
diff --git a/eppm_amd/csrc/ctx_compute.cpp b/eppm_amd/csrc/ctx_compute.cpp
--- a/eppm_amd/csrc/ctx_compute.cpp
+++ b/eppm_amd/csrc/ctx_compute.cpp
@@ -173,11 +173,11 @@
         b.cache_plane = (size_t)lw * lh;
         b.seed_plane = (size_t)lw * lh * 2;
         b.wl_units = pm_worklist_units(lw, lh, c->prm.seg_len);
-        b.p[0] = mk_problem(planes(c, L, false), c->cost1, c->nnf1, c->nnf_tmp, c->rng, 0, c->spec1, EPPM_SWEEP_CACHE ? c->scand1 : nullptr, sweep_list_on(c->opt_sweep_spec) ? c->wl1 : nullptr, c->seed1);
-        b.p[1] = mk_problem(planes(c, L, true), c->cost2, c->nnf2, c->nnf_tmp2, c->rng, 1, c->spec2, EPPM_SWEEP_CACHE ? c->scand2 : nullptr, sweep_list_on(c->opt_sweep_spec) ? c->wl2 : nullptr, c->seed2);
-        if (!seeded) run_patchmatch(b, c->rng, c->lut_pm, c->prm, s, c->opt_sweep_spec);
+        b.p[0] = mk_problem(planes(c, L, false), c->cost1, c->nnf1, c->nnf_tmp, c->rng, 0, c->spec1, EPPM_SWEEP_CACHE ? c->scand1 : nullptr, sweep_list_on(c->opt_sweep_spec) ? c->wl1 : nullptr, c->seed1, c->restw1);
+        b.p[1] = mk_problem(planes(c, L, true), c->cost2, c->nnf2, c->nnf_tmp2, c->rng, 1, c->spec2, EPPM_SWEEP_CACHE ? c->scand2 : nullptr, sweep_list_on(c->opt_sweep_spec) ? c->wl2 : nullptr, c->seed2, c->restw2);
+        if (!seeded) run_patchmatch(b, c->rng, c->lut_pm, c->prm, s, c->opt_sweep_spec, c->opt_search_pre);
         else {
-            pm_start(b, c->rng, c->lut_pm, c->prm, s);
+            pm_start(b, c->rng, c->lut_pm, c->prm, s, c->opt_search_pre);
             PmSeed sd;
             sd.prior[0] = c->prior1; sd.nnf_init[0] = c->nnf_init1; sd.cost_init[0] = c->cost_init1;
             sd.prior[1] = c->prior2; sd.nnf_init[1] = c->nnf_init2; sd.cost_init[1] = c->cost_init2;
@@ -185,7 +185,7 @@
             stage_begin(c, c->ev, "temporal_select");
             launch_pm_cost_select(b, sd, c->lut_pm, c->prm.patch_r, s);
             stage_end(c, c->ev);
-            pm_iterate(b, c->rng, c->lut_pm, c->prm, s, c->opt_sweep_spec);
+            pm_iterate(b, c->rng, c->lut_pm, c->prm, s, c->opt_sweep_spec, c->opt_search_pre);
         }
     }
     stage_end_at(c, c->ev, pm_entry);
diff --git a/eppm_amd/csrc/eppm_internal.h b/eppm_amd/csrc/eppm_internal.h
--- a/eppm_amd/csrc/eppm_internal.h
+++ b/eppm_amd/csrc/eppm_internal.h
@@ -65,6 +65,7 @@
     int16_t* seed = nullptr;
     uint32_t* rng_work;
     uint32_t* rng_work_next;
+    float* restw = nullptr;
 };
 struct PmBatch {
     PmProblem p[2];
@@ -99,7 +100,14 @@
 void launch_pm_jump(const PmBatch& b, const float* lut, int R, int step, hipStream_t s);
 void launch_pm_neighbor(const PmBatch& b, const float* lut, int R, hipStream_t s);
 void launch_pm_random_search(const PmBatch& b, const PmRngDev& rng, const float* lut, int R, int search_range, int num_guess,
-                             hipStream_t s);
+                             hipStream_t s, bool pretest = false);
+void launch_pm_rest_weight(const PmBatch& b, const float* lut, int R, hipStream_t s);
+bool pm_search_pretest_ready(const PmBatch& b, const PmRngDev& rng, int R);
+struct PmPretestSums { float* n[2]; float* d[2]; };
+void launch_pm_pretest_probe(const PmBatch& b, const float* lut, int R, const PmPretestSums& out, hipStream_t s);
+EPPM_DECISION bool pm_search_pretest_form(int w, int h, int R, int problems, int npairs);
+EPPM_DECISION bool pm_search_pretest(int iteration, int w, int h, int R, int problems, int npairs);
+EPPM_DECISION void pm_search_pretest_knobs(int R, int* row0, int* rows, int* from, float* eps);
 EPPM_DECISION int pm_search_rows(int w, int h, int R, int problems, int npairs, bool table);
 struct SweepForm { int lpc; bool small, pre, tile; };
 EPPM_DECISION SweepForm pm_sweep_form(int w, int h, int R, int seg_len, int dir, int problems, int npairs);
diff --git a/eppm_amd/csrc/k_pm_search.hip b/eppm_amd/csrc/k_pm_search.hip
--- a/eppm_amd/csrc/k_pm_search.hip
+++ b/eppm_amd/csrc/k_pm_search.hip
@@ -35,11 +35,12 @@
     hipLaunchKernelGGL(k_pm_rand_table, dim3(rng.gx * rng.gy), dim3(64), 0, s, rng, work, tab, G);
 }
 
-template <int RT, int PK = 0, bool TAB = false, int ROWS = 4>
+template <int RT, int PK = 0, bool TAB = false, int ROWS = 4, bool PRE = false>
 __global__ __launch_bounds__(576) EPPM_SEARCH_OCC void k_pm_random_search(PmBatch B, PmRngDev rng, const float* __restrict__ lut, int R,
                                                           int search_range, int G)
 {
     static_assert(ROWS == 4 || (ROWS == 2 && TAB && RT != 0), "eighth-block workgroups read their numbers from the table");
+    static_assert(!PRE || (ROWS == 4 && TAB && RT != 0 && PK == 2), "the pre-test reads the parity planes; a wave per guess, no drawing wave");
     using LUT = typename SearchLut<RT>::type;
     constexpr int PIXW = 16 * ROWS, NSUB = kBlock / ROWS;
     constexpr int TW = (RT == 0) ? 1 : kBlock + 2 * RT, TH = (RT == 0) ? 1 : ROWS + 2 * RT;
@@ -49,6 +50,9 @@
     __shared__ float s_cost[8][64];
     __shared__ int s_guess[8][64];
     __shared__ uint32_t s_state[TAB ? 2 : 64 * 6];
+    __shared__ uint16_t s_surv[PRE ? 8 * 64 : 1];
+    __shared__ int s_nsurv;
+    (void)s_surv; (void)s_nsurv;
     const unsigned nprob = B.n * B.npairs, bq = blockIdx.x % nprob, brest = blockIdx.x / nprob;
     const int bxx = brest % rng.gx, byy = brest / rng.gx;
     const PmProblem pr = pm_problem(B, bq);
@@ -63,6 +67,7 @@
         for (int q = 0; q < rng.per_lane; q++) s_rand[base + q] = (int16_t)xorwow_next(st);
         if (quarter == 0) store_state(s_state + tid * 6, st);
     }
+    if (PRE && tid == 0) s_nsurv = 0;
     const Planes P = to_dev(pr.P);
     if (RT != 0) {
         const int x0 = bxx * kBlock - RT, y0 = tile_y * kBlock + quarter * ROWS - RT;
@@ -108,6 +113,37 @@
         evaluate = !(EPPM_SEARCH_SKIP_SAME && gx == bx && gy == by);
         s_guess[k][lane] = (gx & 0xffff) | (gy << 16);
     }
+#ifndef EPPM_TOL
+    if constexpr (PRE) {
+        bool survives = false;
+        if (inimg) {
+            s_cost[k][lane] = INFINITY;
+            if (evaluate) {
+                float cs, ws;
+                search_patch_centre_rows<RT>(P, L, s_src, TW, lane & 15, lane >> 4, gx, gy, pr.P, cs, ws);
+                survives = !(cs * (1.0f - EPPM_SEARCH_PRE_EPS) >= pr.cost[cidx] * (ws + pr.restw[cidx]));
+            }
+        }
+        const uint64_t m = __ballot(survives);
+        int base = 0;
+        if ((tid & 63) == 0 && m) base = atomicAdd(&s_nsurv, __popcll(m));
+        base = __builtin_amdgcn_readfirstlane(base);
+        if (survives) s_surv[base + __builtin_amdgcn_mbcnt_hi((uint32_t)(m >> 32), __builtin_amdgcn_mbcnt_lo((uint32_t)m, 0u))] = (uint16_t)tid;
+        __syncthreads();
+        const int ns = s_nsurv;
+        if (ns <= EPPM_SEARCH_PRE_COOP_MAX) {
+            constexpr int CL = 16;
+            for (int slot = tid / CL; slot < ns; slot += (int)blockDim.x / CL) {
+                const int e = s_surv[slot], sk = e >> 6, sl = e & 63, sg = s_guess[sk][sl];
+                const float cv = coop_patch_dist<RT, CL>(P, L, s_src, TW, sl & 15, sl >> 4, (int)(int16_t)(sg & 0xffff), sg >> 16, tid % CL);
+                if (tid % CL == 0) s_cost[sk][sl] = cv;
+            }
+        } else if (tid < ns) {
+            const int e = s_surv[tid], sk = e >> 6, sl = e & 63, sg = s_guess[sk][sl];
+            s_cost[sk][sl] = search_patch_dist<RT, PK>(P, L, R, s_src, TW, sl & 15, sl >> 4, 0, 0, (int)(int16_t)(sg & 0xffff), sg >> 16, pr.P);
+        }
+    } else
+#endif
     if (inimg) {
         float cv = INFINITY;
         if (evaluate) {
@@ -131,14 +167,104 @@
     }
 }
 
+#ifndef EPPM_TOL
+template <int RT>
+__global__ __launch_bounds__(256) void k_pm_rest_weight(PmBatch B, const float* __restrict__ lut, int R)
+{
+    using LUT = typename SearchLut<RT>::type;
+    constexpr int TW = kBlock + 2 * RT, S = RT + 1, I0 = pre_row0(S);
+    __shared__ float4 s_src[TW * TW];
+    __shared__ EPPM_LUT_ALIGN LUT L;
+    const int tid = threadIdx.y * kBlock + threadIdx.x;
+    load_patch_lut(L, lut, R, tid, 256);
+    const PmProblem pr = pm_problem(B, blockIdx.z);
+    const Planes P = to_dev(pr.P);
+    pm_stage_tile<RT>(s_src, P, blockIdx.x, blockIdx.y, tid);
+    __syncthreads();
+    const int x = blockIdx.x * kBlock + threadIdx.x, y = blockIdx.y * kBlock + threadIdx.y;
+    if (x >= P.w || y >= P.h) return;
+    const rgbf c1 = texel_rgb(s_src[(threadIdx.y + RT) * TW + threadIdx.x + RT]);
+    float u = 0.0f;
+    for (int ii = 0; ii < S; ii++) {
+        if (ii >= I0 && ii < I0 + EPPM_SEARCH_PRE_ROWS) continue;
+        const float4* __restrict__ srow = s_src + (threadIdx.y + 2 * ii) * TW + threadIdx.x;
+        for (int jj = 0; jj < S; jj++) u += rest_weight_term(c1, srow[2 * jj], L.gsp[ii * S + jj]);
+    }
+    pr.restw[y * B.cpitch + x] = u;
+}
+#endif
+void launch_pm_rest_weight(const PmBatch& b, const float* lut, int R, hipStream_t s)
+{
+#ifndef EPPM_TOL
+    const int w = b.p[0].P.w, h = b.p[0].P.h;
+    if (R == 9) hipLaunchKernelGGL(k_pm_rest_weight<9>, dim3((w + kBlock - 1) / kBlock, (h + kBlock - 1) / kBlock, b.n * b.npairs), dim3(kBlock, kBlock), 0, s, b, lut, R);
+#endif
+}
+
 int pm_search_rows(int w, int h, int R, int problems, int npairs, bool table)
 {
     const int quarter_wgs = ((w + kBlock - 1) / kBlock) * ((h + kBlock - 1) / kBlock) * 4 * problems * npairs;
     return (table && R == 9 && quarter_wgs < EPPM_SEARCH_HALF_BELOW_WGS) ? 2 : 4;
 }
 
+#ifndef EPPM_TOL
+template <int RT>
+__global__ __launch_bounds__(64) void k_pm_pretest_probe(PmBatch B, const float* __restrict__ lut, int R, PmPretestSums out)
+{
+    using LUT = typename SearchLut<RT>::type;
+    constexpr int TW = kBlock + 2 * RT, TH = 4 + 2 * RT;
+    __shared__ float4 s_src[TW * TH];
+    __shared__ EPPM_LUT_ALIGN LUT L;
+    const int tid = threadIdx.x;
+    load_patch_lut(L, lut, R, tid, 64);
+    const PmProblem pr = pm_problem(B, blockIdx.z);
+    const Planes P = to_dev(pr.P);
+    const int x0 = blockIdx.x * kBlock - RT, y0 = blockIdx.y * 4 - RT;
+    for (int t = tid; t < TW * TH; t += 64) {
+        const int sy = iclamp(y0 + t / TW, 0, P.h - 1), sx = iclamp(x0 + t % TW, 0, P.w - 1);
+        s_src[t] = P.pk1[(unsigned)(sy * P.pitch + sx)];
+    }
+    __syncthreads();
+    const int x = blockIdx.x * kBlock + (tid & 15), y = blockIdx.y * 4 + (tid >> 4);
+    if (x >= P.w || y >= P.h) return;
+    const int k = blockIdx.z % (unsigned)B.n, pair = blockIdx.z / (unsigned)B.n, nidx = y * B.npitch + x;
+    float cs, ws;
+    search_patch_centre_rows<RT>(P, L, s_src, TW, tid & 15, tid >> 4, pr.nnf[nidx * 2], pr.nnf[nidx * 2 + 1], pr.P, cs, ws);
+    pair_ptr(k ? out.n[1] : out.n[0], B.stride, pair)[y * B.cpitch + x] = cs;
+    pair_ptr(k ? out.d[1] : out.d[0], B.stride, pair)[y * B.cpitch + x] = ws;
+}
+#endif
+void launch_pm_pretest_probe(const PmBatch& b, const float* lut, int R, const PmPretestSums& out, hipStream_t s)
+{
+#ifndef EPPM_TOL
+    const int w = b.p[0].P.w, h = b.p[0].P.h;
+    if (R == 9) hipLaunchKernelGGL(k_pm_pretest_probe<9>, dim3((w + kBlock - 1) / kBlock, (h + 3) / 4, b.n * b.npairs), dim3(64), 0, s, b, lut, R, out);
+#endif
+}
+
+bool pm_search_pretest_form(int w, int h, int R, int problems, int npairs)
+{
+#ifdef EPPM_TOL
+    return false;
+#else
+    return R == 9 && pm_search_rows(w, h, R, problems, npairs, true) == 4;
+#endif
+}
+bool pm_search_pretest(int iteration, int w, int h, int R, int problems, int npairs)
+{
+    return EPPM_SEARCH_PRE_FROM >= 0 && iteration >= EPPM_SEARCH_PRE_FROM && pm_search_pretest_form(w, h, R, problems, npairs);
+}
+void pm_search_pretest_knobs(int R, int* row0, int* rows, int* from, float* eps)
+{
+    *row0 = pre_row0(R + 1); *rows = EPPM_SEARCH_PRE_ROWS; *from = EPPM_SEARCH_PRE_FROM; *eps = EPPM_SEARCH_PRE_EPS;
+}
+bool pm_search_pretest_ready(const PmBatch& b, const PmRngDev& rng, int R)
+{
+    return rng.rand_tab && pm_has_parity(b, R, EPPM_PARITY_SEARCH) && b.p[0].restw && (b.n < 2 || b.p[1].restw);
+}
+
 void launch_pm_random_search(const PmBatch& b, const PmRngDev& rng, const float* lut, int R, int search_range, int num_guess,
-                             hipStream_t s)
+                             hipStream_t s, bool pretest)
 {
     dim3 grid(rng.gx * rng.gy * 4 * b.n * b.npairs), block(64 * (num_guess + 1));
     const bool have_pc = b.p[0].P.pc2 && (b.n < 2 || b.p[1].P.pc2);
@@ -146,6 +272,12 @@
         dim3 blockt(64 * num_guess);
         const bool half = pm_search_rows(b.p[0].P.w, b.p[0].P.h, R, b.n, b.npairs, true) == 2;
         if (pm_has_parity(b, R, EPPM_PARITY_SEARCH)) {
+#ifndef EPPM_TOL
+            if (pretest && R == 9 && pm_search_pretest_ready(b, rng, R)) {
+                hipLaunchKernelGGL((k_pm_random_search<9, 2, true, 4, true>), grid, blockt, 0, s, b, rng, lut, R, search_range, num_guess);
+                return;
+            }
+#endif
             if (half)
                 hipLaunchKernelGGL((k_pm_random_search<9, 2, true, 2>), dim3(grid.x * 2), dim3(32 * num_guess), 0, s, b, rng, lut, R, search_range, num_guess);
             else if (R == 9) hipLaunchKernelGGL((k_pm_random_search<9, 2, true>), grid, blockt, 0, s, b, rng, lut, R, search_range, num_guess);
diff --git a/eppm_amd/csrc/launchers_ref_abi.cpp b/eppm_amd/csrc/launchers_ref_abi.cpp
--- a/eppm_amd/csrc/launchers_ref_abi.cpp
+++ b/eppm_amd/csrc/launchers_ref_abi.cpp
@@ -453,6 +453,81 @@
 }
 #endif
 
+#ifdef EPPM_TEST_HOOKS
+extern "C" int eppm_test_pm_search(eppm_pm_rng* r, float* d_cost, eppm_short2* d_nnf, const uint32_t* d_img1, const uint32_t* d_img2, int w, int h,
+                                   int ndir, int npairs, int pretest, float* d_restw, float* d_pre_n, float* d_pre_d)
+{
+    if (!r || !d_cost || !d_nnf || !d_img1 || !d_img2 || w != r->w || h != r->h || ndir < 1 || ndir > 2 || npairs < 1)
+        return set_err(EPPM_ERR_ARG, "eppm_test_pm_search: bad argument");
+    LAUNCHER_BEGIN_INT;
+    const int R = g_prm.patch_r;
+    if (r->G != g_prm.num_guess || (R != 9 && R != 17)) return set_err(EPPM_ERR_ARG, "eppm_test_pm_search: num_guess %d / patch_r %d", r->G, R);
+    const size_t n = (size_t)w * h;
+    const int pad = (R + 2) & ~1, ppitch = parity_pitch(w, pad);
+    size_t off = 0;
+    auto carve = [&](size_t bytes) { const size_t o = off; off = (off + bytes + 255) & ~(size_t)255; return o; };
+    size_t o_img[2], o_cen[2], o_pk[2], o_pc[2], o_pp[2], o_cost[2], o_nnf[2], o_rw[2], o_pn[2], o_pd[2];
+    for (int k = 0; k < 2; k++) { o_img[k] = carve(n * 4); o_cen[k] = carve(n); o_pk[k] = carve(n * 16); o_pc[k] = carve(n * 4); o_pp[k] = carve((size_t)2 * h * ppitch * 4); }
+    for (int k = 0; k < ndir; k++) { o_cost[k] = carve(n * 4); o_nnf[k] = carve(n * 4); o_rw[k] = carve(n * 4); o_pn[k] = carve(n * 4); o_pd[k] = carve(n * 4); }
+    const size_t stride = (off + 4095) & ~(size_t)4095;
+    void *slab = nullptr, *tab = nullptr;
+    CHK(get_scratch(ds, stride * npairs, &slab, 0));
+    CHK(get_scratch(ds, (size_t)r->gx * r->gy * 512 * r->G * sizeof(int16_t), &tab, 7));
+    char* S = (char*)slab;
+    for (int p = 0; p < npairs; p++) {
+        CHK(copy_d2d(S + p * stride + o_img[0], d_img1 + p * n, n * 4));
+        CHK(copy_d2d(S + p * stride + o_img[1], d_img2 + p * n, n * 4));
+        for (int k = 0; k < ndir; k++) {
+            CHK(copy_d2d(S + p * stride + o_cost[k], d_cost + (p * ndir + k) * n, n * 4));
+            CHK(copy_d2d(S + p * stride + o_nnf[k], (const char*)d_nnf + (p * ndir + k) * n * 4, n * 4));
+        }
+    }
+    const Batch bt{npairs, stride};
+    CensusBatch cb;
+    cb.n = 2;
+    for (int k = 0; k < 2; k++) {
+        CensusJob& J = cb.job[k];
+        J.census = (uint8_t*)(S + o_cen[k]); J.cpitch = w; J.texels = S + o_pk[k]; J.tpitch = w; J.img = (const uint32_t*)(S + o_img[k]); J.ipitch = w;
+        J.w = w; J.h = h; J.first_block = 0; J.packed = (uint32_t*)(S + o_pc[k]);
+    }
+    launch_census_batch(cb, g_stream, bt);
+    for (int k = 0; k < 2; k++) launch_parity_planes((uint32_t*)(S + o_pp[k]), ppitch, pad, (const uint32_t*)(S + o_pc[k]), w, w, h, g_stream, bt);
+    PmBatch b;
+    b.n = ndir; b.cpitch = w; b.npitch = w; b.npairs = npairs; b.stride = stride;
+    for (int k = 0; k < ndir; k++) {
+        PlanesH P;
+        P.pk1 = S + o_pk[k]; P.pk2 = S + o_pk[k ^ 1]; P.w = w; P.h = h; P.pitch = w;
+        P.pc1 = (const uint32_t*)(S + o_pc[k]); P.pc2 = (const uint32_t*)(S + o_pc[k ^ 1]);
+        P.pp1 = (const uint32_t*)(S + o_pp[k]); P.pp2 = (const uint32_t*)(S + o_pp[k ^ 1]); P.pp_pitch = ppitch; P.pp_pad = pad;
+        b.p[k] = mk_problem(P, (float*)(S + o_cost[k]), (int16_t*)(S + o_nnf[k]), nullptr, nullptr, 0, nullptr, nullptr, nullptr, nullptr, (float*)(S + o_rw[k]));
+    }
+    PmRngDev d = r->dev();
+    launch_pm_rand_table(d, r->work[0][r->cur[0]], (int16_t*)tab, r->G, g_stream);
+    d.rand_tab = (const int16_t*)tab;
+    if (pretest) {
+        if (!pm_search_pretest_ready(b, d, R)) return set_err(EPPM_ERR_ARG, "eppm_test_pm_search: no two-phase search at patch_r %d", R);
+        launch_pm_rest_weight(b, ds->lut_pm, R, g_stream);
+        if (d_pre_n && d_pre_d) {
+            PmPretestSums ps{};
+            for (int k = 0; k < ndir; k++) { ps.n[k] = (float*)(S + o_pn[k]); ps.d[k] = (float*)(S + o_pd[k]); }
+            launch_pm_pretest_probe(b, ds->lut_pm, R, ps, g_stream);
+        }
+    }
+    launch_pm_random_search(b, d, ds->lut_pm, R, g_prm.search_range, g_prm.num_guess, g_stream, pretest != 0);
+    for (int p = 0; p < npairs; p++)
+        for (int k = 0; k < ndir; k++) {
+            CHK(copy_d2d(d_cost + (p * ndir + k) * n, S + p * stride + o_cost[k], n * 4));
+            CHK(copy_d2d((char*)d_nnf + (p * ndir + k) * n * 4, S + p * stride + o_nnf[k], n * 4));
+            if (pretest && d_restw) CHK(copy_d2d(d_restw + (p * ndir + k) * n, S + p * stride + o_rw[k], n * 4));
+            if (pretest && d_pre_n && d_pre_d) {
+                CHK(copy_d2d(d_pre_n + (p * ndir + k) * n, S + p * stride + o_pn[k], n * 4));
+                CHK(copy_d2d(d_pre_d + (p * ndir + k) * n, S + p * stride + o_pd[k], n * 4));
+            }
+        }
+    return finish();
+}
+#endif
+
 extern "C" void baoCudaFlowSmoothing(eppm_float2* d_flow, eppm_uchar4* d_img, int w, int h, size_t img_pitch, size_t flow_pitch)
 {
     LAUNCHER_BEGIN;
diff --git a/eppm_amd/csrc/pm_device.cuh b/eppm_amd/csrc/pm_device.cuh
--- a/eppm_amd/csrc/pm_device.cuh
+++ b/eppm_amd/csrc/pm_device.cuh
@@ -72,6 +72,18 @@
 #endif
 #ifndef EPPM_SEARCH_PK17
 #define EPPM_SEARCH_PK17 1
+#endif
+#ifndef EPPM_SEARCH_PRE_ROWS
+#define EPPM_SEARCH_PRE_ROWS 4
+#endif
+#ifndef EPPM_SEARCH_PRE_FROM
+#define EPPM_SEARCH_PRE_FROM 2
+#endif
+#ifndef EPPM_SEARCH_PRE_COOP_MAX
+#define EPPM_SEARCH_PRE_COOP_MAX 96
+#endif
+#ifndef EPPM_SEARCH_PRE_EPS
+#define EPPM_SEARCH_PRE_EPS 0x1p-13f
 #endif
 
 namespace eppm {
@@ -103,6 +115,7 @@
     p.seed = pair_ptr_opt(p.seed, B.stride, pair);
     p.rng_work = pair_ptr_opt(p.rng_work, B.stride, pair);
     p.rng_work_next = pair_ptr_opt(p.rng_work_next, B.stride, pair);
+    p.restw = pair_ptr_opt(p.restw, B.stride, pair);
     return p;
 }
 
@@ -201,6 +214,48 @@
     return sum.result();
 }
 
+constexpr int pre_row0(int S) { return (S - EPPM_SEARCH_PRE_ROWS) / 2; }
+#ifndef EPPM_TOL
+__device__ __forceinline__ float rest_weight_term(const rgbf c1, const float4 q1, float gsp)
+{
+    float a2 = max_abs_diff(c1, texel_rgb(q1));
+    a2 *= a2;
+    return fast_exp(div_ad2(-a2)) * gsp;
+}
+template <int RT, class LUT>
+__device__ __forceinline__ void search_patch_centre_rows(const Planes& P, const LUT& L, const float4* __restrict__ s_src, int TW, int tx, int ty,
+                                                         int x2, int y2, const PlanesH& PH, float& cs, float& ws)
+{
+    constexpr int S = RT + 1, I0 = pre_row0(S);
+    static_assert(S % 4 == 2 && EPPM_SEARCH_PRE_ROWS >= 1 && EPPM_SEARCH_PRE_ROWS <= S, "rows of whole dwordx4 gathers + one dwordx2");
+    const int pitch16 = P.pitch << 4;
+    const rgbf c1 = texel_rgb(s_src[(ty + RT) * TW + tx + RT]);
+    const rgbf c2 = texel_rgb(texel_at(P.pk2, texel_off(pitch16, P.w, P.h, x2, y2)));
+    const __amdgpu_buffer_rsrc_t rs = __builtin_amdgcn_make_buffer_rsrc(const_cast<uint32_t*>(PH.pp2), 0, 2 * P.h * PH.pp_pitch * 4, 0x00020000);
+    const int xp = x2 - RT + PH.pp_pad;
+    const int rb = ((xp & 1) * P.h) * PH.pp_pitch + (xp >> 1);
+    cs = 0.0f; ws = 0.0f;
+#pragma unroll 2
+    for (int ii = I0; ii < I0 + EPPM_SEARCH_PRE_ROWS; ii++) {
+        const int ro = (rb + iclamp(y2 + 2 * ii - RT, 0, P.h - 1) * PH.pp_pitch) * 4;
+        const float4* __restrict__ srow = s_src + (ty + 2 * ii) * TW + tx;
+        uint32_t wq[S];
+#pragma unroll
+        for (int g = 0; g < S / 4; g++) {
+            const u32x4 v = __builtin_amdgcn_raw_buffer_load_b128(rs, ro + 16 * g, 0, 0);
+            wq[4 * g] = v.x; wq[4 * g + 1] = v.y; wq[4 * g + 2] = v.z; wq[4 * g + 3] = v.w;
+        }
+        { const u32x2 v = __builtin_amdgcn_raw_buffer_load_b64(rs, ro + 4 * (S - 2), 0, 0); wq[S - 2] = v.x; wq[S - 1] = v.y; }
+EPPM_PM_UNROLL(((S % 5 == 0) ? 5 : S))
+        for (int jj = 0; jj < S; jj++) {
+            float ct, wt;
+            patch_terms(srow[2 * jj], unpack_texel(wq[jj], 0u), c1, c2, L.gsp[ii * S + jj], L.tab(), ct, wt);
+            patch_accum(cs, ws, ct, wt);
+        }
+    }
+}
+#endif
+
 template <int RT>
 __device__ __forceinline__ void pm_stage_tile(float4* __restrict__ s_src, const Planes& P, int bx, int by, int tid)
 {
diff --git a/eppm_amd/csrc/pm_driver.cpp b/eppm_amd/csrc/pm_driver.cpp
--- a/eppm_amd/csrc/pm_driver.cpp
+++ b/eppm_amd/csrc/pm_driver.cpp
@@ -2,19 +2,20 @@
 
 using namespace eppm;
 
-PmProblem mk_problem(const PlanesH& P, float* cost, int16_t* nnf, int16_t* nnf_alt, eppm_pm_rng* rng, int k, float* spec, int32_t* scand, uint32_t* wl, int16_t* seed)
+PmProblem mk_problem(const PlanesH& P, float* cost, int16_t* nnf, int16_t* nnf_alt, eppm_pm_rng* rng, int k, float* spec, int32_t* scand, uint32_t* wl, int16_t* seed,
+                     float* restw)
 {
     PmProblem p;
-    p.P = P; p.cost = cost; p.nnf = nnf; p.nnf_alt = nnf_alt; p.spec = spec; p.scand = scand; p.wl = wl; p.seed = seed;
+    p.P = P; p.cost = cost; p.nnf = nnf; p.nnf_alt = nnf_alt; p.spec = spec; p.scand = scand; p.wl = wl; p.seed = seed; p.restw = restw;
     p.rng_work = rng ? rng->work[k][rng->cur[k]] : nullptr;
     p.rng_work_next = rng ? rng->work[k][rng->cur[k] ^ 1] : nullptr;
     return p;
 }
-void search(PmBatch& b, eppm_pm_rng* rng, const float* lut, const eppm_params& prm, hipStream_t s, int launch_no)
+void search(PmBatch& b, eppm_pm_rng* rng, const float* lut, const eppm_params& prm, hipStream_t s, int launch_no, bool pretest)
 {
     PmRngDev d = rng->dev();
     if (rng->rand_tab && launch_no >= 0) d.rand_tab = rng->rand_tab + (size_t)launch_no * rng->rand_stride;
-    launch_pm_random_search(b, d, lut, prm.patch_r, prm.search_range, prm.num_guess, s);
+    launch_pm_random_search(b, d, lut, prm.patch_r, prm.search_range, prm.num_guess, s, pretest);
     for (int k = 0; k < b.n; k++) {
         std::swap(b.p[k].rng_work, b.p[k].rng_work_next);
         rng->cur[k] ^= 1;
@@ -67,18 +68,28 @@
         for (int k = 0; k < b.n; k++) std::swap(b.p[k].nnf, b.p[k].nnf_alt);
     }
 }
-void run_patchmatch(PmBatch& b, eppm_pm_rng* rng, const float* lut, const eppm_params& prm, hipStream_t s, int spec_mode)
+static bool search_pretest(const PmBatch& b, const eppm_params& prm, int it, int pre_from)
 {
-    pm_start(b, rng, lut, prm, s);
-    pm_iterate(b, rng, lut, prm, s, spec_mode);
+    const int w = b.p[0].P.w, h = b.p[0].P.h;
+    if (pre_from < 0) return pm_search_pretest(it, w, h, prm.patch_r, b.n, b.npairs);
+    return it >= pre_from && pm_search_pretest_form(w, h, prm.patch_r, b.n, b.npairs);
 }
-void pm_start(PmBatch& b, eppm_pm_rng* rng, const float* lut, const eppm_params& prm, hipStream_t s)
+void run_patchmatch(PmBatch& b, eppm_pm_rng* rng, const float* lut, const eppm_params& prm, hipStream_t s, int spec_mode, int pre_from)
+{
+    pm_start(b, rng, lut, prm, s, pre_from);
+    pm_iterate(b, rng, lut, prm, s, spec_mode, pre_from);
+}
+void pm_start(PmBatch& b, eppm_pm_rng* rng, const float* lut, const eppm_params& prm, hipStream_t s, int pre_from)
 {
     b.sweep_seq = 0;
     launch_pm_init_field(b, rng->dev(), s);
     launch_pm_cost_field(b, lut, prm.patch_r, s);
+    PmRngDev d = rng->dev();
+    d.rand_tab = rng->rand_tab;
+    if (prm.num_iter > 0 && search_pretest(b, prm, prm.num_iter - 1, pre_from) && pm_search_pretest_ready(b, d, prm.patch_r))
+        launch_pm_rest_weight(b, lut, prm.patch_r, s);
 }
-void pm_iterate(PmBatch& b, eppm_pm_rng* rng, const float* lut, const eppm_params& prm, hipStream_t s, int spec_mode)
+void pm_iterate(PmBatch& b, eppm_pm_rng* rng, const float* lut, const eppm_params& prm, hipStream_t s, int spec_mode, int pre_from)
 {
     for (int it = 0; it < prm.num_iter; it++) {
         if (prm.propagation == 1) jump(b, lut, prm, s);
@@ -88,6 +99,6 @@
             if (sweeps_merged(it, pixels, problem_pixels, spec_mode) && launch_pm_sweeps_merged(b, lut, prm.patch_r, prm.seg_len, it, s)) {  }
             else for (int dir = 0; dir < 4; dir++) sweep(b, lut, prm, dir, s, sweep_speculative(it, pixels, spec_mode));
         }
-        search(b, rng, lut, prm, s, it);
+        search(b, rng, lut, prm, s, it, search_pretest(b, prm, it, pre_from));
     }
 }
diff --git a/eppm_amd/stages.py b/eppm_amd/stages.py
--- a/eppm_amd/stages.py
+++ b/eppm_amd/stages.py
@@ -200,6 +200,29 @@
     return c.get(), n.get()
 
 
+def pm_search_launch(rng, costs, nnfs, pairs, ndir=1, pretest=False, sums=False):
+    h, w = nnfs[0].shape
+    n = len(nnfs)
+    assert n == len(pairs) * ndir == len(costs)
+    c = Dev(np.concatenate([np.ascontiguousarray(x, np.float32) for x in costs]))
+    f = Dev(np.concatenate([np.ascontiguousarray(x, short2) for x in nnfs]))
+    i1, i2 = (Dev(np.concatenate([np.ascontiguousarray(p[k], uchar4) for p in pairs])) for k in range(2))
+    u = Dev(shape=(n * h, w), dtype=np.float32) if pretest else None
+    pn, pd = (Dev(shape=(n * h, w), dtype=np.float32) for _ in range(2)) if pretest and sums else (None, None)
+    check(lib().eppm_test_pm_search(rng.p, c.ptr, f.ptr, i1.ptr, i2.ptr, w, h, ndir, len(pairs), int(pretest), u.ptr if u else None,
+                                    pn.ptr if pn else None, pd.ptr if pd else None), "eppm_test_pm_search")
+    split = lambda a: [a[k * h:(k + 1) * h] for k in range(n)]
+    out = (split(c.get()), split(f.get()), split(u.get()) if u else None)
+    return out + (split(pn.get()), split(pd.get())) if pn else out
+
+
+def probe_search_pretest(iteration, w, h, patch_r=9, problems=2, npairs=1):
+    out = (C.c_int * 5)()
+    eps = C.c_float()
+    check(lib().eppm_probe_search_pretest(iteration, w, h, patch_r, problems, npairs, out, C.byref(eps)), "eppm_probe_search_pretest")
+    return bool(out[0]), out[1], out[2], out[3], eps.value, bool(out[4])
+
+
 def patchmatch(P):
     n, c = Dev(shape=(P.h, P.w), dtype=short2), Dev(shape=(P.h, P.w), dtype=np.float32)
     lib().baoCudaPatchMatch(n.ptr, c.ptr, *P.args(), P.w, P.h, _sz(P.i1.pitch), _sz(c.pitch), _sz(n.pitch), _sz(P.c1.pitch))
```

Result: faster. 242.5 Mflow-vectors/s (median of 6 runs) (+2.2%).
